# isarandi/metro-pose3d

Hardware: AMD Instinct MI355X
Metric: crops/sec (256x256, RN50 stride16) (higher is better)
Workload: dtype f16

## Files before the change

### include/metro_hip.h

```cpp
#ifndef METRO_HIP_H
#define METRO_HIP_H

#include <stddef.h>
#include <stdint.h>

#ifdef __cplusplus
extern "C" {
#endif

#define METRO_ABI_VERSION 8

typedef enum MetroStatus {
    METRO_OK = 0,
    METRO_ERR_INVALID_ARG = -1,
    METRO_ERR_UNSUPPORTED = -2,
    METRO_ERR_HIP = -3,
    METRO_ERR_STATE = -4,
    METRO_ERR_NONFINITE = -5
} MetroStatus;

typedef enum MetroPrecision { METRO_PREC_F16 = 0, METRO_PREC_F32 = 1, METRO_PREC_F64 = 2, METRO_PREC_F32M = 3 } MetroPrecision;

typedef enum MetroDType { METRO_F16 = 0, METRO_F32 = 1, METRO_F64 = 2 } MetroDType;

#define METRO_MAX_JOINTS 64

typedef struct MetroSpec {
    int32_t arch;
    int32_t stride;
    int32_t n_joints_head;
    int32_t depth;
    int32_t centered_stride;
    int32_t proc_side;
    float   box_size_mm;
    int32_t base_width;
    int32_t precision;
    int32_t n_joints_out;
    int32_t permutation[METRO_MAX_JOINTS];
} MetroSpec;

typedef struct MetroPlan MetroPlan;

typedef enum MetroParamKind {
    METRO_PARAM_CONV_W = 0,
    METRO_PARAM_BIAS = 1,
    METRO_PARAM_PRO_SCALE = 2,
    METRO_PARAM_PRO_SHIFT = 3
} MetroParamKind;

typedef struct MetroParamInfo {
    char    name[96];
    char    conv_var[160];
    char    bn_var[160];
    int32_t kind;
    int32_t dtype;
    int32_t c_out, kh, kw, c_in;
    int32_t kw_pad, c_in_pad;
    int64_t offset;
    int64_t bytes;
} MetroParamInfo;

#define METRO_FUSED_CONV1_IN_FRONT 1
#define METRO_FUSED_PROJECTION_SHORTCUT 2
#define METRO_FUSED_OUT_ON_CHIP 4
#define METRO_FUSED_REBUILT_SHORTCUT 8
#define METRO_FUSED_COMPACT_SHORTCUT 16

typedef struct MetroLayerInfo {
    char    name[96];
    int32_t kind;
    int32_t h_in, w_in, c_in, h_out, w_out, c_out, kh, kw, stride, dilation, pad_top, pad_left;
    int32_t has_prologue, relu, has_residual, res_stride, res_offset;
    int32_t out_dtype;
    int64_t out_offset;
    int64_t out_bytes_per_image;
    double  flops_per_image;
    int64_t out2_offset;
    int32_t out2_channels;
    int32_t fused_flags;
    int64_t algo_act_bytes_per_image;
    int64_t algo_param_bytes;
    int64_t out_sub_offset;
    int32_t out_sub_side, out_sub_off;
} MetroLayerInfo;

int  metro_plan_create(const MetroSpec* spec, int32_t max_batch, MetroPlan** out_plan);
int  metro_plan_destroy(MetroPlan* plan);
int64_t metro_plan_workspace_bytes(const MetroPlan* plan);
int64_t metro_plan_param_bytes(const MetroPlan* plan);
int32_t metro_plan_num_params(const MetroPlan* plan);
int  metro_plan_param_info(const MetroPlan* plan, int32_t index, MetroParamInfo* out);
int32_t metro_plan_num_layers(const MetroPlan* plan);
int  metro_plan_layer_info(const MetroPlan* plan, int32_t index, MetroLayerInfo* out);
double metro_plan_flops_per_image(const MetroPlan* plan);
int  metro_plan_layer_kernel(const MetroPlan* plan, int32_t index, int32_t n, char* buf, int32_t buf_len);
int  metro_kernel_notes(int32_t mode);
const char* metro_last_kernel_id(void);
int  metro_plan_bind_params(MetroPlan* plan, const void* d_param_blob);

int  metro_forward(MetroPlan* plan, const float* d_images_nhwc, int32_t n, float* d_poses_out,
                   void* d_workspace, void* stream);
int  metro_plan_set_graph_max_batch(MetroPlan* plan, int32_t max_batch_for_graphs);
int  metro_forward_status(const MetroPlan* plan, const void* d_workspace, int32_t n, void* stream, int32_t* n_nonfinite_out);
int64_t metro_plan_status_offset(const MetroPlan* plan);
int  metro_forward_upto(MetroPlan* plan, const float* d_images_nhwc, int32_t n,
                        float* d_poses_out, void* d_workspace, void* stream,
                        int32_t last_layer);

int  metro_forward_timed(MetroPlan* plan, const float* d_images_nhwc, int32_t n,
                         float* d_poses_out, void* d_workspace, void* stream,
                         float* ms_out );


typedef struct MetroConvDesc {
    int32_t n, h_in, w_in, c_in;
    int32_t in_pix_stride;
    int32_t h_out, w_out, c_out;
    int32_t kh, kw, stride, dilation;
    int32_t pad_top, pad_left;
    int32_t has_prologue;
    int32_t relu;
    int32_t has_residual;
    int32_t res_h, res_w;
    int32_t res_stride, res_offset;
    int32_t out_dtype;
    int32_t in_dtype;
} MetroConvDesc;

int  metro_conv_f16(const MetroConvDesc* d, const void* d_in, const void* d_w, const float* d_bias,
                    const void* d_pro_scale, const void* d_pro_shift, const void* d_residual,
                    void* d_out, void* stream);
int  metro_conv_f16_pair(const MetroConvDesc* d, const void* d_in, const void* d_w, const float* d_bias,
                         const void* d_pro_scale, const void* d_pro_shift, void* d_out, int32_t split,
                         void* d_out2, void* stream);
int  metro_conv_f16_next(const MetroConvDesc* d, const void* d_in, const void* d_w, const float* d_bias,
                         const void* d_residual, void* d_out, const void* d_w2, const float* d_bias2,
                         const void* d_scale2, const void* d_shift2, void* d_out2, int32_t c2, void* stream);
int  metro_conv_f16_conv1_conv2(const MetroConvDesc* d, const void* d_x, const void* d_w1, const float* d_bias1, const void* d_pro_scale,
                                const void* d_pro_shift, const void* d_w2, const float* d_bias2, void* d_out, void* stream);
int  metro_conv_f16_next_proj(const MetroConvDesc* d, const void* d_in, const void* d_w, const float* d_bias, const void* d_x,
                              const void* d_w_sc, const float* d_bias_sc, const void* d_pro_scale, const void* d_pro_shift, void* d_out,
                              const void* d_w2, const float* d_bias2, const void* d_scale2, const void* d_shift2, void* d_out2,
                              int32_t c2, void* stream);
int  metro_conv_f16_next_rebuild(const MetroConvDesc* d, const void* d_in, const void* d_w, const float* d_bias, const void* d_x,
                                 const void* d_w_sc, const float* d_bias_sc, const void* d_pro_scale, const void* d_pro_shift,
                                 const void* d_t2_prev, const void* d_w3_prev, const float* d_bias3_prev, void* d_out, void* d_out_sub,
                                 int32_t sub_off, const void* d_w2, const float* d_bias2, const void* d_scale2, const void* d_shift2,
                                 void* d_out2, int32_t c2, void* stream);
int  metro_conv_b1_form(int32_t classic);
int  metro_conv_f16_gemm4w(const MetroConvDesc* d, const void* d_in, const void* d_w, const float* d_bias,
                           const void* d_pro_scale, const void* d_pro_shift, const void* d_residual, void* d_out,
                           int32_t split, void* d_out2, void* stream);
int  metro_stem_pool_f16(const void* d_prepped, const void* d_w, const float* d_bias, void* d_out, int32_t n,
                         int32_t side, void* stream);
int  metro_stem_pool_f32in(const float* d_images, const void* d_w, const float* d_bias, void* d_out, int32_t n,
                           int32_t side, void* stream);
int  metro_stem_pool_u8in(const uint8_t* d_images, const void* d_w, const float* d_bias, void* d_out, int32_t n,
                          int32_t side, void* stream);
int  metro_conv_f64acc(const MetroConvDesc* d, const void* d_in, const double* d_w,
                       const double* d_bias, const double* d_pro_scale,
                       const double* d_pro_shift, const void* d_residual, void* d_out,
                       void* stream);

int  metro_conv_f32m(const MetroConvDesc* d, const void* d_in, const float* d_w, const float* d_bias, const float* d_pro_scale,
                     const float* d_pro_shift, const void* d_residual, void* d_out, void* stream);

int  metro_prep_input_f16(const float* d_images, int32_t n, int32_t side, void* d_out, void* stream);
int  metro_images_u8_to_f32(const uint8_t* d_in, int64_t count, float* d_out, void* stream);

int  metro_warp_crop_u8(const uint8_t* d_image, int32_t h, int32_t w, int32_t row_stride,
                        const float* d_homographies, int32_t n, int32_t side, float* d_out, void* stream);

#define METRO_MAX_FRAMES 64
#define METRO_WARP_HOMOGRAPHY 0
#define METRO_WARP_DISTORTED 1
typedef struct MetroFrame {
    const uint8_t* data;
    int32_t h, w, row_stride;
    int32_t reserved;
} MetroFrame;
typedef struct MetroCropWarp {
    int32_t frame;
    int32_t mode;
    double partial[9];
    float homography[9];
    float intrinsics[6];
    float distortion[5];
} MetroCropWarp;
int  metro_warp_crops_frames_u8(const MetroFrame* frames, int32_t n_frames, const MetroCropWarp* d_crops, int32_t n,
                                int32_t side, float* d_out, void* stream);
int  metro_warp_crops_frames_u8_to_u8(const MetroFrame* frames, int32_t n_frames, const MetroCropWarp* d_crops, int32_t n,
                                      int32_t side, uint8_t* d_out, void* stream);

#define METRO_PIX_RGB  0
#define METRO_PIX_BGR  1
#define METRO_PIX_NV12 2
#define METRO_PIX_I420 3
#define METRO_YUV_BT601 0
#define METRO_YUV_BT709 1
typedef struct MetroFramePlanes {
    const uint8_t* plane[3];
    int32_t h, w;
    int32_t stride[2];
    int32_t format, matrix;
} MetroFramePlanes;
int  metro_warp_crops_frames_planes(const MetroFramePlanes* frames, int32_t n_frames, const MetroCropWarp* d_crops,
                                    int32_t n, int32_t side, float* d_out, void* stream);
int  metro_warp_crops_frames_planes_to_u8(const MetroFramePlanes* frames, int32_t n_frames, const MetroCropWarp* d_crops,
                                          int32_t n, int32_t side, uint8_t* d_out, void* stream);

int  metro_maxpool3x3s2_zeropad(const void* d_in, void* d_out, int32_t n, int32_t h_in,
                                int32_t w_in, int32_t c, int32_t dtype, void* stream);

int64_t metro_softargmax_scratch_bytes(int32_t n, int32_t side, int32_t n_joints_head);
int  metro_softargmax(const void* d_logits, int32_t n, const MetroSpec* spec, int32_t precise,
                      void* d_partials, float* d_poses_out, void* stream);

int64_t metro_head_f16_scratch_bytes(int32_t n, int32_t side, int32_t n_joints_head);
int  metro_head_f16(const void* d_x, const void* d_w, const float* d_bias, const void* d_pro_scale, const void* d_pro_shift,
                    int32_t n, int32_t c_in, const MetroSpec* spec, void* d_partials, float* d_logits_out, float* d_poses_out,
                    void* stream);

int  metro_eval_metrics(const float* d_pred, const float* d_true, const uint8_t* d_valid, int32_t n,
                        int32_t n_joints, float threshold_mm, float* d_dist, float* d_dist_aligned,
                        double* d_sums, void* stream);

int  metro_softargmax01(const void* d_logits, int32_t n, const MetroSpec* spec, int32_t precise, void* d_scratch,
                        float* d_coords01_out, void* stream);
int  metro_backproject_bone_lengths(const float* d_coords01, const float* d_inv_intrinsics, const double* d_bone_lengths,
                                    int32_t per_pose_lengths, const int32_t* d_edges, int32_t n_edges, int32_t n,
                                    const MetroSpec* spec, int32_t root_relative, int32_t permute,
                                    float* d_coords3d_out, float* d_z_offset_out, void* stream);
int  metro_backproject_root_depth(const float* d_coords01, const float* d_inv_intrinsics, const float* d_root_z,
                                  int32_t n, const MetroSpec* spec, int32_t root_relative, int32_t permute,
                                  float* d_coords3d_out, void* stream);
int  metro_heatmap_to_25d(const float* d_coords01, int32_t n, const MetroSpec* spec, float* d_out, void* stream);
int  metro_to_orig_cam(const float* d_coords, const float* d_rot, const int32_t* d_mirror, float* d_out, int32_t n,
                       int32_t n_joints, void* stream);

int  metro_forward_coords01(MetroPlan* plan, const float* d_images_nhwc, int32_t n, float* d_poses_out,
                            float* d_coords01_out, void* d_workspace, void* stream);
int  metro_forward_u8(MetroPlan* plan, const uint8_t* d_images_nhwc, int32_t n, float* d_poses_out,
                      float* d_coords01_out, void* d_workspace, void* stream);
typedef struct MetroPlacement {
    int32_t keypoint_mode;
    int32_t reserved;
    float inv_intrinsics[9];
    float rot_to_orig_cam[9];
    float rot_to_world[9];
    float cam_loc[3];
    float homography[9];
    float intrinsics[6];
    float distortion[5];
} MetroPlacement;
#define METRO_SCALE_METRO 0
#define METRO_SCALE_BONE_LENGTHS 1
#define METRO_SCALE_TRUE_ROOT_DEPTH 2
#define METRO_COORDS_CROP 0
#define METRO_COORDS_CAMERA 1
#define METRO_COORDS_WORLD 2
int  metro_place_poses(const float* d_coords01, const float* d_poses, const MetroPlacement* d_records, int32_t n,
                       const MetroSpec* spec, int32_t scale_recovery, const double* d_bone_lengths, int32_t per_pose_lengths,
                       const float* d_root_depth, const int32_t* d_edges, int32_t n_edges, const int32_t* d_mirror,
                       int32_t coords, float* d_poses_out, float* d_keypoints_out, float* d_z_offset_out, void* stream);

typedef struct MetroViewBase {
    int32_t frame;
    int32_t mode;
    int32_t has_camera;
    int32_t reserved;
    double old_matrix[9];
    double orig_r[9];
    double virt_k[9];
    double virt_r[9];
    double partial[9];
    float homography[9];
    float inv_intrinsics[9];
    float rot_to_orig_cam[9];
    float rot_to_world[9];
    float cam_loc[3];
    float intrinsics[6];
    float distortion[5];
} MetroViewBase;
#define METRO_MAX_VIEWS 32
typedef struct MetroView {
    double cos_roll, sin_roll, zoom;
    int32_t flip;
    int32_t reserved;
} MetroView;
int  metro_expand_views(const MetroViewBase* d_bases, int32_t n, const MetroView* views, int32_t n_views, int32_t side,
                        MetroCropWarp* d_crops_out, MetroPlacement* d_placements_out, void* stream);
typedef struct MetroFrameCamera {
    float intrinsics[9];
    float r[9];
    float r_inv[9];
    float t[3];
    float distortion[5];
    int32_t has_distortion;
    double world_up[3];
    double old_matrix[9];
} MetroFrameCamera;
// ... 79 lines not shown
```

### metro_pose3d_amd/_lib.py

```python
from __future__ import annotations

import ctypes as C
import os

HERE = os.path.dirname(os.path.abspath(__file__))
LIB_PATH = os.environ.get('METRO_HIP_LIB') or os.path.join(HERE, 'libmetro_hip.so')

METRO_MAX_JOINTS = 64
ABI_VERSION = 8
METRO_PREC_F16, METRO_PREC_F32, METRO_PREC_F64, METRO_PREC_F32M = 0, 1, 2, 3
METRO_F16, METRO_F32, METRO_F64 = 0, 1, 2
PARAM_CONV_W, PARAM_BIAS, PARAM_PRO_SCALE, PARAM_PRO_SHIFT = 0, 1, 2, 3
LAYER_PREP, LAYER_CONV, LAYER_POOL, LAYER_SOFTARGMAX = 0, 1, 2, 3
FUSED_CONV1_IN_FRONT, FUSED_PROJECTION_SHORTCUT = 1, 2
FUSED_OUT_ON_CHIP, FUSED_REBUILT_SHORTCUT, FUSED_COMPACT_SHORTCUT = 4, 8, 16


class MetroSpec(C.Structure):
    _fields_ = [('arch', C.c_int32), ('stride', C.c_int32), ('n_joints_head', C.c_int32),
                ('depth', C.c_int32), ('centered_stride', C.c_int32), ('proc_side', C.c_int32),
                ('box_size_mm', C.c_float), ('base_width', C.c_int32), ('precision', C.c_int32),
                ('n_joints_out', C.c_int32), ('permutation', C.c_int32 * METRO_MAX_JOINTS)]


class MetroParamInfo(C.Structure):
    _fields_ = [('name', C.c_char * 96), ('conv_var', C.c_char * 160), ('bn_var', C.c_char * 160),
                ('kind', C.c_int32), ('dtype', C.c_int32),
                ('c_out', C.c_int32), ('kh', C.c_int32), ('kw', C.c_int32), ('c_in', C.c_int32),
                ('kw_pad', C.c_int32), ('c_in_pad', C.c_int32),
                ('offset', C.c_int64), ('bytes', C.c_int64)]


class MetroLayerInfo(C.Structure):
    _fields_ = [('name', C.c_char * 96), ('kind', C.c_int32),
                ('h_in', C.c_int32), ('w_in', C.c_int32), ('c_in', C.c_int32),
                ('h_out', C.c_int32), ('w_out', C.c_int32), ('c_out', C.c_int32),
                ('kh', C.c_int32), ('kw', C.c_int32), ('stride', C.c_int32),
                ('dilation', C.c_int32), ('pad_top', C.c_int32), ('pad_left', C.c_int32),
                ('has_prologue', C.c_int32), ('relu', C.c_int32), ('has_residual', C.c_int32),
                ('res_stride', C.c_int32), ('res_offset', C.c_int32), ('out_dtype', C.c_int32),
                ('out_offset', C.c_int64), ('out_bytes_per_image', C.c_int64),
                ('flops_per_image', C.c_double),
                ('out2_offset', C.c_int64), ('out2_channels', C.c_int32), ('fused_flags', C.c_int32),
                ('algo_act_bytes_per_image', C.c_int64), ('algo_param_bytes', C.c_int64),
                ('out_sub_offset', C.c_int64), ('out_sub_side', C.c_int32), ('out_sub_off', C.c_int32)]


class MetroConvDesc(C.Structure):
    _fields_ = [('n', C.c_int32), ('h_in', C.c_int32), ('w_in', C.c_int32), ('c_in', C.c_int32),
                ('in_pix_stride', C.c_int32),
                ('h_out', C.c_int32), ('w_out', C.c_int32), ('c_out', C.c_int32),
                ('kh', C.c_int32), ('kw', C.c_int32), ('stride', C.c_int32), ('dilation', C.c_int32),
                ('pad_top', C.c_int32), ('pad_left', C.c_int32),
                ('has_prologue', C.c_int32), ('relu', C.c_int32), ('has_residual', C.c_int32),
                ('res_h', C.c_int32), ('res_w', C.c_int32),
                ('res_stride', C.c_int32), ('res_offset', C.c_int32), ('out_dtype', C.c_int32),
                ('in_dtype', C.c_int32)]


METRO_MAX_FRAMES = 64
METRO_WARP_HOMOGRAPHY, METRO_WARP_DISTORTED = 0, 1


class MetroFrame(C.Structure):
    _fields_ = [('data', C.c_void_p), ('h', C.c_int32), ('w', C.c_int32), ('row_stride', C.c_int32),
                ('reserved', C.c_int32)]


METRO_PIX_RGB, METRO_PIX_BGR, METRO_PIX_NV12, METRO_PIX_I420 = 0, 1, 2, 3
METRO_YUV_BT601, METRO_YUV_BT709 = 0, 1


class MetroFramePlanes(C.Structure):
    _fields_ = [('plane', C.c_void_p * 3), ('h', C.c_int32), ('w', C.c_int32), ('stride', C.c_int32 * 2),
                ('format', C.c_int32), ('matrix', C.c_int32)]


class MetroCropWarp(C.Structure):
    _fields_ = [('frame', C.c_int32), ('mode', C.c_int32), ('partial', C.c_double * 9), ('homography', C.c_float * 9),
                ('intrinsics', C.c_float * 6), ('distortion', C.c_float * 5)]


METRO_SCALE_METRO, METRO_SCALE_BONE_LENGTHS, METRO_SCALE_TRUE_ROOT_DEPTH = 0, 1, 2
METRO_COORDS_CROP, METRO_COORDS_CAMERA, METRO_COORDS_WORLD = 0, 1, 2


class MetroPlacement(C.Structure):
    _fields_ = [('keypoint_mode', C.c_int32), ('reserved', C.c_int32), ('inv_intrinsics', C.c_float * 9),
                ('rot_to_orig_cam', C.c_float * 9), ('rot_to_world', C.c_float * 9), ('cam_loc', C.c_float * 3),
                ('homography', C.c_float * 9), ('intrinsics', C.c_float * 6), ('distortion', C.c_float * 5)]


METRO_MAX_VIEWS = 32
METRO_TRI_UNIFORM, METRO_TRI_COVARIANCE = 0, 1
METRO_MATCH_MAX_BOXES = 128
METRO_SMOOTH_FILTER, METRO_SMOOTH_RTS = 0, 1
METRO_SMOOTH_ISOTROPIC, METRO_SMOOTH_COVARIANCE = 0, 1
METRO_ASSOC_MAX = 128


class MetroViewBase(C.Structure):
    _fields_ = [('frame', C.c_int32), ('mode', C.c_int32), ('has_camera', C.c_int32), ('reserved', C.c_int32),
                ('old_matrix', C.c_double * 9), ('orig_r', C.c_double * 9), ('virt_k', C.c_double * 9),
                ('virt_r', C.c_double * 9), ('partial', C.c_double * 9), ('homography', C.c_float * 9),
                ('inv_intrinsics', C.c_float * 9), ('rot_to_orig_cam', C.c_float * 9), ('rot_to_world', C.c_float * 9),
                ('cam_loc', C.c_float * 3), ('intrinsics', C.c_float * 6), ('distortion', C.c_float * 5)]


class MetroFrameCamera(C.Structure):
    _fields_ = [('intrinsics', C.c_float * 9), ('r', C.c_float * 9), ('r_inv', C.c_float * 9), ('t', C.c_float * 3),
                ('distortion', C.c_float * 5), ('has_distortion', C.c_int32), ('world_up', C.c_double * 3),
                ('old_matrix', C.c_double * 9)]


class MetroView(C.Structure):
    _fields_ = [('cos_roll', C.c_double), ('sin_roll', C.c_double), ('zoom', C.c_double), ('flip', C.c_int32),
                ('reserved', C.c_int32)]


_P = C.c_void_p
SIGNATURES = {
    'metro_plan_create': (C.c_int, [C.POINTER(MetroSpec), C.c_int32, C.POINTER(_P)]),
    'metro_plan_destroy': (C.c_int, [_P]),
    'metro_plan_workspace_bytes': (C.c_int64, [_P]),
    'metro_plan_param_bytes': (C.c_int64, [_P]),
    'metro_plan_num_params': (C.c_int32, [_P]),
    'metro_plan_param_info': (C.c_int, [_P, C.c_int32, C.POINTER(MetroParamInfo)]),
    'metro_plan_num_layers': (C.c_int32, [_P]),
    'metro_plan_layer_info': (C.c_int, [_P, C.c_int32, C.POINTER(MetroLayerInfo)]),
    'metro_plan_flops_per_image': (C.c_double, [_P]),
    'metro_plan_bind_params': (C.c_int, [_P, _P]),
    'metro_plan_layer_kernel': (C.c_int, [_P, C.c_int32, C.c_int32, C.c_char_p, C.c_int32]),
    'metro_kernel_notes': (C.c_int, [C.c_int32]),
    'metro_last_kernel_id': (C.c_char_p, []),
    'metro_plan_set_graph_max_batch': (C.c_int, [_P, C.c_int32]),
    'metro_forward': (C.c_int, [_P, _P, C.c_int32, _P, _P, _P]),
    'metro_forward_coords01': (C.c_int, [_P, _P, C.c_int32, _P, _P, _P, _P]),
    'metro_forward_u8': (C.c_int, [_P, _P, C.c_int32, _P, _P, _P, _P]),
    'metro_forward_status': (C.c_int, [_P, _P, C.c_int32, _P, C.POINTER(C.c_int32)]),
    'metro_plan_status_offset': (C.c_int64, [_P]),
    'metro_forward_upto': (C.c_int, [_P, _P, C.c_int32, _P, _P, _P, C.c_int32]),
    'metro_forward_timed': (C.c_int, [_P, _P, C.c_int32, _P, _P, _P, C.POINTER(C.c_float)]),
    'metro_conv_f16': (C.c_int, [C.POINTER(MetroConvDesc), _P, _P, _P, _P, _P, _P, _P, _P]),
    'metro_conv_f32m': (C.c_int, [C.POINTER(MetroConvDesc), _P, _P, _P, _P, _P, _P, _P, _P]),
    'metro_conv_f64acc': (C.c_int, [C.POINTER(MetroConvDesc), _P, _P, _P, _P, _P, _P, _P, _P]),
    'metro_conv_f16_pair': (C.c_int, [C.POINTER(MetroConvDesc), _P, _P, _P, _P, _P, _P, C.c_int32, _P, _P]),
    'metro_conv_b1_form': (C.c_int, [C.c_int32]),
    'metro_conv_f16_gemm4w': (C.c_int, [C.POINTER(MetroConvDesc), _P, _P, _P, _P, _P, _P, _P, C.c_int32, _P, _P]),
    'metro_conv_f16_conv1_conv2': (C.c_int, [C.POINTER(MetroConvDesc), _P, _P, _P, _P, _P, _P, _P, _P, _P]),
    'metro_conv_f16_next_proj': (C.c_int, [C.POINTER(MetroConvDesc)] + [_P] * 14 + [C.c_int32, _P]),
    'metro_conv_f16_next_rebuild': (C.c_int, [C.POINTER(MetroConvDesc)] + [_P] * 13 + [C.c_int32] + [_P] * 5 + [C.c_int32, _P]),
    'metro_conv_f16_next': (C.c_int, [C.POINTER(MetroConvDesc), _P, _P, _P, _P, _P, _P, _P, _P, _P, _P, C.c_int32, _P]),
    'metro_stem_pool_f16': (C.c_int, [_P, _P, _P, _P, C.c_int32, C.c_int32, _P]),
    'metro_stem_pool_f32in': (C.c_int, [_P, _P, _P, _P, C.c_int32, C.c_int32, _P]),
    'metro_stem_pool_u8in': (C.c_int, [_P, _P, _P, _P, C.c_int32, C.c_int32, _P]),
    'metro_prep_input_f16': (C.c_int, [_P, C.c_int32, C.c_int32, _P, _P]),
    'metro_images_u8_to_f32': (C.c_int, [_P, C.c_int64, _P, _P]),
    'metro_warp_crop_u8': (C.c_int, [_P, C.c_int32, C.c_int32, C.c_int32, _P, C.c_int32, C.c_int32, _P, _P]),
    'metro_warp_crops_frames_u8': (C.c_int, [C.POINTER(MetroFrame), C.c_int32, _P, C.c_int32, C.c_int32, _P, _P]),
    'metro_warp_crops_frames_planes': (C.c_int, [C.POINTER(MetroFramePlanes), C.c_int32, _P, C.c_int32, C.c_int32, _P,
                                                 _P]),
    'metro_warp_crops_frames_u8_to_u8': (C.c_int, [C.POINTER(MetroFrame), C.c_int32, _P, C.c_int32, C.c_int32, _P, _P]),
    'metro_warp_crops_frames_planes_to_u8': (C.c_int, [C.POINTER(MetroFramePlanes), C.c_int32, _P, C.c_int32, C.c_int32, _P,
                                                       _P]),
    'metro_eval_metrics': (C.c_int, [_P, _P, _P, C.c_int32, C.c_int32, C.c_float, _P, _P, _P, _P]),
    'metro_maxpool3x3s2_zeropad': (C.c_int, [_P, _P, C.c_int32, C.c_int32, C.c_int32, C.c_int32,
                                             C.c_int32, _P]),
    'metro_softargmax_scratch_bytes': (C.c_int64, [C.c_int32, C.c_int32, C.c_int32]),
    'metro_softargmax01': (C.c_int, [_P, C.c_int32, C.POINTER(MetroSpec), C.c_int32, _P, _P, _P]),
    'metro_backproject_bone_lengths': (C.c_int, [_P, _P, _P, C.c_int32, _P, C.c_int32, C.c_int32, C.POINTER(MetroSpec),
                                                 C.c_int32, C.c_int32, _P, _P, _P]),
    'metro_backproject_root_depth': (C.c_int, [_P, _P, _P, C.c_int32, C.POINTER(MetroSpec), C.c_int32, C.c_int32, _P, _P]),
    'metro_to_orig_cam': (C.c_int, [_P, _P, _P, _P, C.c_int32, C.c_int32, _P]),
    'metro_place_poses': (C.c_int, [_P, _P, _P, C.c_int32, C.POINTER(MetroSpec), C.c_int32, _P, C.c_int32, _P, _P, C.c_int32,
                                    _P, C.c_int32, _P, _P, _P, _P]),
    'metro_expand_views': (C.c_int, [_P, C.c_int32, C.POINTER(MetroView), C.c_int32, C.c_int32, _P, _P, _P]),
    'metro_look_at_boxes': (C.c_int, [_P, _P, C.c_int32, C.c_int32, _P, C.c_int32, C.c_int32, _P, _P, _P]),
    'metro_merge_views': (C.c_int, [_P, _P, _P, _P, _P, C.c_int32, C.c_int32, C.c_int32, _P, _P, _P, _P, _P]),
    'metro_heatmap_to_25d': (C.c_int, [_P, C.c_int32, C.POINTER(MetroSpec), _P, _P]),
    'metro_head_f16_scratch_bytes': (C.c_int64, [C.c_int32, C.c_int32, C.c_int32]),
    'metro_head_f16': (C.c_int, [_P, _P, _P, _P, _P, C.c_int32, C.c_int32, C.POINTER(MetroSpec), _P, _P, _P, _P]),
    'metro_softargmax': (C.c_int, [_P, C.c_int32, C.POINTER(MetroSpec), C.c_int32, _P, _P, _P]),
    'metro_moments_scratch_bytes': (C.c_int64, [C.POINTER(MetroSpec), C.c_int32]),
    'metro_forward_moments': (C.c_int, [_P, _P, C.c_int32, C.c_int32, _P, _P, _P, _P, _P, _P, _P]),
    'metro_head_f16_moments': (C.c_int, [_P, _P, _P, _P, _P, C.c_int32, C.c_int32, C.POINTER(MetroSpec)] + [_P] * 8),
    'metro_softargmax01_moments': (C.c_int, [_P, C.c_int32, C.POINTER(MetroSpec), C.c_int32, _P, _P, _P, _P, _P, _P]),
    'metro_place_covariances': (C.c_int, [_P, _P, _P, C.c_int32, C.c_int32, C.POINTER(MetroSpec), _P, C.c_int32, _P, _P, _P]),
    'metro_triangulate_joints': (C.c_int, [_P, _P, _P, C.c_int32, _P, C.c_int32, _P, C.c_int32, C.POINTER(MetroSpec), _P, C.c_int32,
                                           C.c_double, _P, _P, _P, _P]),
    'metro_view_affinity': (C.c_int, [_P, _P, _P, C.POINTER(MetroSpec), _P, _P, C.c_int32, C.c_int32, C.c_int32, C.c_double, C.c_double,
                                      C.c_int32, _P, _P, _P]),
    'metro_triangulate_joints_cov': (C.c_int, [_P, _P, _P, C.c_int32, _P, C.c_int32, _P, C.c_int32, C.POINTER(MetroSpec), _P, C.c_int32,
                                               C.c_double, _P, _P, _P, _P, _P]),
    'metro_view_affinity_steps': (C.c_int, [_P, _P, _P, C.POINTER(MetroSpec), _P, _P, _P, C.c_int32, C.c_int32, C.c_int32, C.c_double,
                                            C.c_double, C.c_int32, _P, _P, _P]),
    'metro_person_steps': (C.c_int, [_P, C.c_int32, _P, _P, C.c_int32, C.c_int32, _P, C.c_int32, _P, C.c_int32, _P, _P, _P, _P, _P]),
    'metro_cluster_views': (C.c_int, [_P, C.c_int32, C.c_int32, C.c_float, _P, _P, _P, _P, _P]),
    'metro_smooth_tracks_workspace_bytes': (C.c_size_t, [C.c_int32, C.c_int32]),
    'metro_smooth_tracks': (C.c_int, [_P, _P, _P, C.c_int32, _P, C.c_int32, _P, C.c_int32, C.POINTER(MetroSpec), C.c_int32, C.c_int32,
                                      C.c_double, C.c_double, C.c_double, C.c_double, C.c_double, _P, _P, _P, _P, _P, _P, _P]),
    'metro_associate_tracks_workspace_bytes': (C.c_size_t, [C.c_int32, C.c_int32]),
    'metro_associate_tracks': (C.c_int, [_P, _P, _P, C.c_int32, _P, C.c_int32, _P, C.c_int32, C.POINTER(MetroSpec), C.c_int32,
                                         C.c_double, C.c_double, C.c_double, C.c_double, C.c_double, C.c_float, C.c_double, C.c_int32,
                                         C.c_double, _P, C.c_int32] + [_P] * 11),
    'metro_last_error': (C.c_char_p, []),
    'metro_abi_version': (C.c_int32, []),
}

EXPERIMENTAL_LIB_PATH = os.path.join(HERE, 'libmetro_experimental.so')
EXPERIMENTAL_SIGNATURES = {
    'metro_conv_f16_gemm8p': (C.c_int, [C.POINTER(MetroConvDesc), _P, _P, _P, _P, _P, _P, _P, C.c_int32, _P, _P]),
    'metro_conv_f16_gemm4d': (C.c_int, [C.POINTER(MetroConvDesc), _P, _P, _P, _P, _P, _P, _P, C.c_int32, _P, _P]),
    'metro_conv_f16_gemm4d_geo': (C.c_int, [C.POINTER(MetroConvDesc), _P, _P, _P, _P, _P, _P, _P, C.c_int32, _P, C.c_int32, _P]),
}

_lib = None
_xlib = None


class MetroError(RuntimeError):
    pass


class NonFiniteError(MetroError):
    """metro_forward_status: activations overflowed the arithmetic mode (fp16 storage tops out at 65 504)."""


def load() -> C.CDLL:
    global _lib
    if _lib is not None:
        return _lib
    if not os.path.exists(LIB_PATH):
        raise MetroError(
            f'{LIB_PATH} is missing: build it with `python -m metro_pose3d_amd.build` '
            '(hipcc --offload-arch=gfx950). There is no CPU fallback for this path.')
    import torch
    lib = C.CDLL(LIB_PATH)
    for name, (res, args) in SIGNATURES.items():
        fn = getattr(lib, name)
        fn.restype = res
        fn.argtypes = args
    if lib.metro_abi_version() != ABI_VERSION:
        raise MetroError(f'ABI version mismatch: library {lib.metro_abi_version()}, bindings {ABI_VERSION}')
    _lib = lib
    return lib


def load_experimental() -> C.CDLL:
    global _xlib
    if _xlib is not None:
        return _xlib
    load()
    if not os.path.exists(EXPERIMENTAL_LIB_PATH):
        raise MetroError(f'{EXPERIMENTAL_LIB_PATH} is missing: build it with `python -m metro_pose3d_amd.build`')
    lib = C.CDLL(EXPERIMENTAL_LIB_PATH)
    for name, (res, args) in EXPERIMENTAL_SIGNATURES.items():
        fn = getattr(lib, name)
        fn.restype = res
        fn.argtypes = args
    _xlib = lib
    return lib


def check(status: int, what: str = '') -> None:
    if status == 0:
        return
    msg = load().metro_last_error().decode(errors='replace')
    if status == -1:
        raise ValueError(f'{what}: {msg}')
    if status == -5:
        raise NonFiniteError(f'{what}: {msg}')
    raise MetroError(f'{what}: status {status}: {msg}')
```

### metro_pose3d_amd/csrc/conv_igemm_f16_dma.hip

```cpp
#include <cstdlib>
#include <type_traits>

#include "metro_common.h"
#include "gfx950_prims.h"

namespace metro {

template <int WAVES_M_, int WAVES_N_, int WM_, int WN_, int STAGES_, int BK_ = 64>
struct DmaCfg {
    static constexpr int WAVES_M = WAVES_M_, WAVES_N = WAVES_N_, WM = WM_, WN = WN_, STAGES = STAGES_;
    static constexpr int BK = BK_;
    static constexpr int CPR = BK / 8;
    static constexpr int RPI = 64 / CPR;
    static constexpr int NW = WAVES_M * WAVES_N;
    static constexpr int NT = 64 * NW;
    static constexpr int TM = WAVES_M * WM * 32;
    static constexpr int TN = WAVES_N * WN * 32;
    static constexpr int WI = TM / (RPI * NW);
    static constexpr int XI = TN / (RPI * NW);
    static constexpr int LPS = WI + XI;
    static constexpr int ROW_BYTES = BK * 2;
    static constexpr int STAGE_BYTES = (TM + TN) * ROW_BYTES;
    static constexpr int RING_BYTES = STAGES * STAGE_BYTES;
    static constexpr int OUT_ROW_BYTES = TM * 2 + 16;
    static constexpr int OUT_BYTES = TN * OUT_ROW_BYTES;
    static constexpr int MAIN_BYTES = RING_BYTES > OUT_BYTES ? RING_BYTES : OUT_BYTES;
    static constexpr int PRO_BYTES = 2 * 2048 * 2;
    static_assert(TM % (RPI * NW) == 0 && TN % (RPI * NW) == 0, "tile/loader mismatch");
    static_assert(BK == 64 || BK == 32, "BK must be 32 or 64");
    static_assert(STAGES >= 1 && STAGES <= 6, "ring depth 1..6");
};

struct Fuse2Args {
    const half_t* w2; const float* bias2; const half_t* scale2; const half_t* shift2; half_t* out2; int c2;
};

template <class Cfg, bool PROLOGUE, bool FASTK, bool FUSE2>
__device__ __forceinline__ void conv_dma_body(
    const ConvArgs& a, const half_t* __restrict__ in, const half_t* __restrict__ w,
    const float* __restrict__ bias, const half_t* __restrict__ pro_scale,
    const half_t* __restrict__ pro_shift, const half_t* __restrict__ residual,
    void* __restrict__ out, int out_f32, int tiles_m, void* __restrict__ out2, const Fuse2Args& f2) {
    extern __shared__ __attribute__((aligned(16))) char smem[];
    constexpr int BK = Cfg::BK, STAGES = Cfg::STAGES, NW = Cfg::NW;
    constexpr int CPR = Cfg::CPR, RPI = Cfg::RPI;
    constexpr int SLICES = BK / 16;
    constexpr int F2_W_OFF = Cfg::MAIN_BYTES + (PROLOGUE ? Cfg::PRO_BYTES : 0);
    constexpr int F2_W_BYTES = 64 * Cfg::TM * 2;
    constexpr int F2_P_OFF = F2_W_OFF + F2_W_BYTES;

    const int tid = threadIdx.x;
    const int lane = tid & 63;
    const int wave = __builtin_amdgcn_readfirstlane(tid >> 6);
    const int wave_m = wave / Cfg::WAVES_N;
    const int wave_n = wave % Cfg::WAVES_N;

    const int nblk = gridDim.x;
    int lid;
    {
        const int b = blockIdx.x;
        const int q = nblk >> 3, r = nblk & 7;
        const int xcd = b & 7, idx = b >> 3;
        lid = (xcd < r ? xcd * (q + 1) : r * (q + 1) + (xcd - r) * q) + idx;
    }
    const int tile_n = lid / tiles_m;
    const int tile_m = lid % tiles_m;
    const int m0 = tile_n * Cfg::TN;
    const int n0 = tile_m * Cfg::TM;

    const int taps = a.kh * a.kw;
    const int k_total = taps * a.c_in;
    const int kc_steps = (a.c_in + BK - 1) / BK;
    const int nk = taps * kc_steps;
    const int hw_out = a.h_out * a.w_out;
    const half_t* zero = reinterpret_cast<const half_t*>(g_zero_page);
    const unsigned smem_base = lds_offset_of(smem);

    half_t* pro_lds = reinterpret_cast<half_t*>(smem + Cfg::MAIN_BYTES);

    const int lrow = lane / CPR;
    const int lch = lane % CPR;
    const half_t* wsrc[Cfg::WI];
    int wkoff[Cfg::WI], winc[Cfg::WI];
    bool wvalid[Cfg::WI];
#pragma unroll
    for (int i = 0; i < Cfg::WI; ++i) {
        const int row = (i * NW + wave) * RPI + lrow;
        const int co = n0 + row;
        wvalid[i] = co < a.c_out;
        wkoff[i] = (lch ^ swz<BK>(row)) * 8;
        const half_t* base = w + (size_t)(wvalid[i] ? co : 0) * k_total;
        wsrc[i] = FASTK ? (wvalid[i] ? base + wkoff[i] : zero) : base;
        winc[i] = wvalid[i] ? BK : 0;
    }
    int xh[Cfg::XI], xw[Cfg::XI], xn[Cfg::XI], xkoff[Cfg::XI], xinc[Cfg::XI];
    const half_t* xptr[Cfg::XI];
    bool xvalid[Cfg::XI];
#pragma unroll
    for (int i = 0; i < Cfg::XI; ++i) {
        const int row = (i * NW + wave) * RPI + lrow;
        const int m = m0 + row;
        xvalid[i] = m < a.m_total;
        const int mm = xvalid[i] ? m : 0;
        const int img = mm / hw_out;
        const int rem = mm - img * hw_out;
        const int ho = rem / a.w_out;
        const int wo = rem - ho * a.w_out;
        xh[i] = ho * a.stride - a.pad_top;
        xw[i] = wo * a.stride - a.pad_left;
        xn[i] = img * a.h_in * a.w_in;
        xkoff[i] = (lch ^ swz<BK>(row)) * 8;
        xptr[i] = zero;
        xinc[i] = 0;
    }

    int is_tap = 0, is_c0 = 0, is_r = 0, is_s = 0;
    auto x_new_tap = [&]() {
#pragma unroll
        for (int i = 0; i < Cfg::XI; ++i) {
            const int hi = xh[i] + is_r * a.dil;
            const int wi = xw[i] + is_s * a.dil;
            const bool ok = xvalid[i] && (unsigned)hi < (unsigned)a.h_in && (unsigned)wi < (unsigned)a.w_in;
            xptr[i] = ok ? in + (size_t)(xn[i] + hi * a.w_in + wi) * a.in_pix_stride + xkoff[i] : zero;
            xinc[i] = ok ? BK : 0;
        }
    };
    if (FASTK) x_new_tap();
    unsigned is_wl = 0, is_xl = 0;
    int is_kbase = 0;
    auto issue_begin = [&](int buf) {
        is_wl = __builtin_amdgcn_readfirstlane(smem_base + buf * Cfg::STAGE_BYTES + wave * RPI * Cfg::ROW_BYTES);
        is_xl = is_wl + Cfg::TM * Cfg::ROW_BYTES;
        is_kbase = is_tap * a.c_in + is_c0;
    };
    auto issue_part = [&](int part) {
#pragma unroll
        for (int i = 0; i < Cfg::WI; ++i) {
            if ((i % SLICES) != part) continue;
            if (FASTK) {
                dma16(wsrc[i], is_wl + i * NW * RPI * Cfg::ROW_BYTES);
                wsrc[i] += winc[i];
            } else {
                const int c = is_c0 + wkoff[i];
                const half_t* src = (wvalid[i] && c < a.c_in) ? wsrc[i] + is_kbase + wkoff[i] : zero;
                dma16(src, is_wl + i * NW * RPI * Cfg::ROW_BYTES);
            }
        }
#pragma unroll
        for (int i = 0; i < Cfg::XI; ++i) {
            if (((i + Cfg::WI) % SLICES) != part) continue;
            if (FASTK) {
                dma16(xptr[i], is_xl + i * NW * RPI * Cfg::ROW_BYTES);
                xptr[i] += xinc[i];
            } else {
                const int hi = xh[i] + is_r * a.dil;
                const int wi = xw[i] + is_s * a.dil;
                const int c = is_c0 + xkoff[i];
                const bool ok = xvalid[i] && c < a.c_in && (unsigned)hi < (unsigned)a.h_in &&
                                (unsigned)wi < (unsigned)a.w_in;
                const half_t* src = ok ? in + (size_t)(xn[i] + hi * a.w_in + wi) * a.in_pix_stride + c : zero;
                dma16(src, is_xl + i * NW * RPI * Cfg::ROW_BYTES);
            }
        }
    };
    auto issue_end = [&]() {
        is_c0 += BK;
        if (is_c0 >= a.c_in) {
            is_c0 = 0;
            ++is_tap;
            if (++is_s == a.kw) { is_s = 0; ++is_r; }
            if (FASTK && is_tap < taps) x_new_tap();
        }
    };
    auto issue_step = [&](int buf) {
        issue_begin(buf);
#pragma unroll
        for (int p = 0; p < SLICES; ++p) issue_part(p);
        issue_end();
    };

    floatx16 acc[Cfg::WM][Cfg::WN];
#pragma unroll
    for (int i = 0; i < Cfg::WM; ++i)
#pragma unroll
        for (int j = 0; j < Cfg::WN; ++j)
#pragma unroll
            for (int e = 0; e < 16; ++e) acc[i][j][e] = 0.f;

    const int frag_row = lane & 31;
    const int frag_half = lane >> 5;

    auto compute_step = [&](int buf, int c0, auto with_issue) {
        const char* wl = smem + buf * Cfg::STAGE_BYTES;
        const char* xl = wl + Cfg::TM * Cfg::ROW_BYTES;
#pragma unroll
        for (int kk = 0; kk < BK / 16; ++kk) {
            half8_t af[Cfg::WM], bf[Cfg::WN];
            const int chunk = kk * 2 + frag_half;
#pragma unroll
            for (int i = 0; i < Cfg::WM; ++i) {
                const int row = (wave_m * Cfg::WM + i) * 32 + frag_row;
                af[i] = *reinterpret_cast<const half8_t*>(wl + row * Cfg::ROW_BYTES + ((chunk ^ swz<BK>(row)) << 4));
            }
#pragma unroll
            for (int j = 0; j < Cfg::WN; ++j) {
                const int row = (wave_n * Cfg::WN + j) * 32 + frag_row;
                bf[j] = *reinterpret_cast<const half8_t*>(xl + row * Cfg::ROW_BYTES + ((chunk ^ swz<BK>(row)) << 4));
            }
            if (PROLOGUE) {
                const half8_t sc = *reinterpret_cast<const half8_t*>(pro_lds + c0 + chunk * 8);
                const half8_t sh = *reinterpret_cast<const half8_t*>(pro_lds + 2048 + c0 + chunk * 8);
                const half8_t z = {};
#pragma unroll
                for (int j = 0; j < Cfg::WN; ++j) bf[j] = __builtin_elementwise_max(bf[j] * sc + sh, z);
            }
#ifdef METRO_SETPRIO
            __builtin_amdgcn_s_setprio(1);
#endif
#pragma unroll
            for (int i = 0; i < Cfg::WM; ++i)
#pragma unroll
                for (int j = 0; j < Cfg::WN; ++j)
                    acc[i][j] = __builtin_amdgcn_mfma_f32_32x32x16_f16(af[i], bf[j], acc[i][j], 0, 0, 0);
#ifdef METRO_SETPRIO
            __builtin_amdgcn_s_setprio(0);
#endif
            if constexpr (decltype(with_issue)::value) issue_part(kk);
        }
    };
    using Yes = std::integral_constant<bool, true>;
    using No = std::integral_constant<bool, false>;

    constexpr int CPRO = Cfg::TM / 8;
    constexpr int EPI_ITERS = Cfg::TN * CPRO / Cfg::NT;
    static_assert(Cfg::TN * CPRO % Cfg::NT == 0, "epilogue loop must divide evenly");
    const bool res_same = a.res_stride == 1 && a.res_offset == 0 && a.res_h == a.h_out && a.res_w == a.w_out;
    const bool has_res = residual != nullptr && !out_f32;
    uint4 rres[EPI_ITERS];
#pragma unroll
    for (int it = 0; it < EPI_ITERS; ++it) rres[it] = make_uint4(0, 0, 0, 0);
    auto prefetch_residual = [&]() {
#pragma unroll
        for (int it = 0; it < EPI_ITERS; ++it) {
            const int idx = tid + it * Cfg::NT;
            const int prow = idx / CPRO;
            const int ch = idx - prow * CPRO;
            const int m = m0 + prow;
            const int co = n0 + ch * 8;
            const bool ok = m < a.m_total && co + 8 <= a.c_out;
            size_t rp = ok ? (size_t)m : 0;
            if (!res_same && ok) {
                const int img = m / hw_out;
                const int rem = m - img * hw_out;
                const int ho = rem / a.w_out;
                const int wo = rem - ho * a.w_out;
                rp = (size_t)(img * a.res_h + ho * a.res_stride + a.res_offset) * a.res_w +
                     (wo * a.res_stride + a.res_offset);
            }
            rres[it] = *reinterpret_cast<const uint4*>(residual + rp * a.c_out + (ok ? co : 0));
        }
    };

    constexpr bool PRO_DMA = PROLOGUE && !FUSE2;
    if constexpr (PRO_DMA) {
#pragma unroll
        for (int i = 0; i < (8 + NW - 1) / NW; ++i) {
            const int id = wave * ((8 + NW - 1) / NW) + i;
            const int piece = id & 3;
            if (id < 8 && piece * 512 < a.c_in) {
                const int idx = piece * 512 + lane * 8;
                const half_t* src = idx < a.c_in ? ((id >> 2) ? pro_shift : pro_scale) + idx : zero;
                dma16(src, __builtin_amdgcn_readfirstlane(smem_base + Cfg::MAIN_BYTES + (id >> 2) * 4096 + piece * 1024));
            }
        }
    }
    if constexpr (STAGES > 1) {
#pragma unroll
        for (int s = 0; s < STAGES - 1; ++s)
            if (s < nk) issue_step(s);
    } else {
        issue_step(0);
    }
    if constexpr (FUSE2) {
        static_assert(BK == 64 && (F2_W_BYTES / 1024) % NW == 0, "FUSE2 layout");
#pragma unroll
        for (int i = 0; i < F2_W_BYTES / 1024 / NW; ++i) {
            const int vrow = (i * NW + wave) * 8 + (lane >> 3);
            const int kc = vrow >> 6, r = vrow & 63;
            const half_t* src = f2.w2 + (size_t)r * Cfg::TM + kc * 64 + (((lane & 7) ^ swz<64>(r)) * 8);
            dma16(src, __builtin_amdgcn_readfirstlane(smem_base + F2_W_OFF + (i * NW + wave) * 1024));
        }
        half_t* p2 = reinterpret_cast<half_t*>(smem + F2_P_OFF);
        for (int c = tid * 8; c < Cfg::TM; c += Cfg::NT * 8) {
            *reinterpret_cast<uint4*>(p2 + c) = *reinterpret_cast<const uint4*>(f2.scale2 + c);
            *reinterpret_cast<uint4*>(p2 + Cfg::TM + c) = *reinterpret_cast<const uint4*>(f2.shift2 + c);
        }
    }
    if (PROLOGUE && !PRO_DMA) {
        const int cpad = kc_steps * BK;
        for (int c = tid * 8; c < cpad; c += Cfg::NT * 8) {
            uint4 sv = make_uint4(0, 0, 0, 0), bv = make_uint4(0, 0, 0, 0);
            if (c < a.c_in) {
                sv = *reinterpret_cast<const uint4*>(pro_scale + c);
                bv = *reinterpret_cast<const uint4*>(pro_shift + c);
            }
            *reinterpret_cast<uint4*>(pro_lds + c) = sv;
            *reinterpret_cast<uint4*>(pro_lds + 2048 + c) = bv;
        }
    }

    if (PROLOGUE && !PRO_DMA) __syncthreads();
    if constexpr (STAGES == 1) {
        int cc0 = 0;
        for (int k = 0; k < nk; ++k) {
            if (k > 0) {
                wait_vm_and_barrier<0>();
                issue_step(0);
            }
            if (has_res && k == nk - 1) {
                prefetch_residual();
                wait_vm_and_barrier<EPI_ITERS>();
            } else {
                wait_vm_and_barrier<0>();
            }
            compute_step(0, cc0, No{});
            cc0 += BK;
            if (cc0 >= a.c_in) cc0 = 0;
        }
    } else {
        int cbuf = 0, ibuf = STAGES - 1, cc0 = 0;
        auto advance = [&]() {
            cbuf = cbuf + 1 == STAGES ? 0 : cbuf + 1;
            ibuf = ibuf + 1 == STAGES ? 0 : ibuf + 1;
            cc0 += BK;
            if (cc0 >= a.c_in) cc0 = 0;
        };
        const int n_main = nk - (STAGES - 1);
        for (int k = 0; k < n_main; ++k) {
            wait_vm_and_barrier<(STAGES - 2) * Cfg::LPS>();
            issue_begin(ibuf);
            compute_step(cbuf, cc0, Yes{});
            issue_end();
            advance();
        }
        if (has_res) prefetch_residual();
        for (int k = n_main < 0 ? 0 : n_main; k < nk; ++k) {
            int ahead = nk - 1 - k;
            if (ahead > STAGES - 2) ahead = STAGES - 2;
            if (has_res) {
                switch (ahead) {
                    case 4: wait_vm_and_barrier<(STAGES >= 6 ? 4 : 0) * Cfg::LPS + EPI_ITERS>(); break;
                    case 3: wait_vm_and_barrier<(STAGES >= 5 ? 3 : 0) * Cfg::LPS + EPI_ITERS>(); break;
                    case 2: wait_vm_and_barrier<(STAGES >= 4 ? 2 : 0) * Cfg::LPS + EPI_ITERS>(); break;
                    case 1: wait_vm_and_barrier<(STAGES >= 3 ? 1 : 0) * Cfg::LPS + EPI_ITERS>(); break;
                    default: wait_vm_and_barrier<EPI_ITERS>(); break;
                }
            } else {
                switch (ahead) {
                    case 4: wait_vm_and_barrier<(STAGES >= 6 ? 4 : 0) * Cfg::LPS>(); break;
                    case 3: wait_vm_and_barrier<(STAGES >= 5 ? 3 : 0) * Cfg::LPS>(); break;
                    case 2: wait_vm_and_barrier<(STAGES >= 4 ? 2 : 0) * Cfg::LPS>(); break;
                    case 1: wait_vm_and_barrier<(STAGES >= 3 ? 1 : 0) * Cfg::LPS>(); break;
                    default: wait_vm_and_barrier<0>(); break;
                }
            }
            compute_step(cbuf, cc0, No{});
            advance();
        }
    }

    const bool second = a.split > 0 && n0 >= a.split;
    const int o_c = a.split > 0 ? (second ? a.c_out2 : a.split) : a.c_out;
    const int o_n0 = second ? n0 - a.split : n0;
    const int o_relu = second ? a.relu2 : a.relu;
    void* o_ptr = second ? out2 : out;
    if (out_f32) {
#pragma unroll
        for (int j = 0; j < Cfg::WN; ++j) {
            const int m = m0 + (wave_n * Cfg::WN + j) * 32 + frag_row;
            if (m >= a.m_total) continue;
#pragma unroll
            for (int i = 0; i < Cfg::WM; ++i) {
#pragma unroll
                for (int q = 0; q < 4; ++q) {
                    const int co = n0 + (wave_m * Cfg::WM + i) * 32 + 8 * q + 4 * frag_half;
                    if (co >= a.c_out) continue;
                    const floatx4 bv = *reinterpret_cast<const floatx4*>(bias + co);
                    floatx4 v;
#pragma unroll
                    for (int e = 0; e < 4; ++e) v[e] = acc[i][j][4 * q + e] + bv[e];
                    if (a.relu) {
#pragma unroll
                        for (int e = 0; e < 4; ++e) v[e] = fmaxf(v[e], 0.f);
                    }
                    *reinterpret_cast<floatx4*>(reinterpret_cast<float*>(out) + (size_t)m * a.c_out + co) = v;
                }
            }
        }
        return;
    }

    __syncthreads();
#pragma unroll
    for (int i = 0; i < Cfg::WM; ++i) {
#pragma unroll
        for (int q = 0; q < 4; ++q) {
            const int col = (wave_m * Cfg::WM + i) * 32 + 8 * q + 4 * frag_half;
            const int co = n0 + col;
            floatx4 bv = {0.f, 0.f, 0.f, 0.f};
            if (co < a.c_out) bv = *reinterpret_cast<const floatx4*>(bias + co);
#pragma unroll
            for (int j = 0; j < Cfg::WN; ++j) {
                const int prow = (wave_n * Cfg::WN + j) * 32 + frag_row;
                half4_t hv;
#pragma unroll
                for (int e = 0; e < 4; ++e) {
                    float v = acc[i][j][4 * q + e] + bv[e];
                    if (o_relu) v = fmaxf(v, 0.f);
                    hv[e] = (half_t)v;
                }
                *reinterpret_cast<half4_t*>(smem + prow * Cfg::OUT_ROW_BYTES + col * 2) = hv;
            }
        }
    }
    constexpr int T2M = 2, T2N = Cfg::TN / 32;
    constexpr int F2_KSTEPS = FUSE2 ? Cfg::TM / 16 : 1;
    __syncthreads();
    half_t* outh = reinterpret_cast<half_t*>(o_ptr);
    constexpr int EPI_G = EPI_ITERS % 8 == 0 ? 8 : EPI_ITERS % 4 == 0 ? 4 : EPI_ITERS % 2 == 0 ? 2 : 1;
    const bool interior = m0 + Cfg::TN <= a.m_total && o_n0 + Cfg::TM <= o_c;
    if (interior) {
#pragma unroll
        for (int it0 = 0; it0 < EPI_ITERS; it0 += EPI_G) {
            uint4 vv[EPI_G];
#pragma unroll
            for (int u = 0; u < EPI_G; ++u) {
                const int idx = tid + (it0 + u) * Cfg::NT;
                const int prow = idx / CPRO;
                vv[u] = *reinterpret_cast<const uint4*>(smem + prow * Cfg::OUT_ROW_BYTES + (idx - prow * CPRO) * 16);
            }
            __builtin_amdgcn_sched_barrier(0);
#pragma unroll
            for (int u = 0; u < EPI_G; ++u) {
                const int idx = tid + (it0 + u) * Cfg::NT;
                const int prow = idx / CPRO;
                const int ch = idx - prow * CPRO;
                uint4 v = vv[u];
                if (residual != nullptr) {
                    half2_t* x = reinterpret_cast<half2_t*>(&v);
                    const half2_t* r = reinterpret_cast<const half2_t*>(&rres[it0 + u]);
#pragma unroll
                    for (int e = 0; e < 4; ++e) x[e] = x[e] + r[e];
                }
                store_out16<2>(outh + (size_t)(m0 + prow) * o_c + o_n0 + ch * 8, v);
                if constexpr (FUSE2) *reinterpret_cast<uint4*>(smem + prow * Cfg::OUT_ROW_BYTES + ch * 16) = v;
            }
        }
    } else
#pragma unroll
    for (int it = 0; it < EPI_ITERS; ++it) {
        const int idx = tid + it * Cfg::NT;
        const int prow = idx / CPRO;
        const int ch = idx - prow * CPRO;
        const int m = m0 + prow;
        const int co = o_n0 + ch * 8;
        if (m >= a.m_total || co >= o_c) continue;
        uint4 v = *reinterpret_cast<const uint4*>(smem + prow * Cfg::OUT_ROW_BYTES + ch * 16);
        if (co + 8 <= o_c) {
            if (residual != nullptr) {
                half2_t* x = reinterpret_cast<half2_t*>(&v);
                const half2_t* r = reinterpret_cast<const half2_t*>(&rres[it]);
#pragma unroll
                for (int e = 0; e < 4; ++e) x[e] = x[e] + r[e];
            }
            store_out16<2>(outh + (size_t)m * o_c + co, v);
            if constexpr (FUSE2) *reinterpret_cast<uint4*>(smem + prow * Cfg::OUT_ROW_BYTES + ch * 16) = v;
        } else {
            const half8_t x = *reinterpret_cast<const half8_t*>(&v);
#pragma unroll
            for (int e = 0; e < 8; ++e)
                if (co + e < o_c) outh[(size_t)m * o_c + co + e] = x[e];
        }
    }
    if constexpr (FUSE2) {
        __syncthreads();
        if (wave < T2M * T2N) {
            const int i2 = wave / T2N, j2 = wave % T2N;
            floatx16 acc2;
#pragma unroll
            for (int e = 0; e < 16; ++e) acc2[e] = 0.f;
            const half_t* p2 = reinterpret_cast<const half_t*>(smem + F2_P_OFF);
            const int prow2 = j2 * 32 + frag_row;
            const int arow = i2 * 32 + frag_row;
            const char* w2l = smem + F2_W_OFF + arow * 128;
#pragma unroll
            for (int ks = 0; ks < F2_KSTEPS; ++ks) {
                const int k0 = ks * 16 + frag_half * 8;
                const half8_t af = *reinterpret_cast<const half8_t*>(
                    w2l + (ks >> 2) * 8192 + ((((ks & 3) * 2 + frag_half) ^ swz<64>(arow)) << 4));
                half8_t bf = *reinterpret_cast<const half8_t*>(smem + prow2 * Cfg::OUT_ROW_BYTES + k0 * 2);
                const half8_t sc = *reinterpret_cast<const half8_t*>(p2 + k0);
                const half8_t sh = *reinterpret_cast<const half8_t*>(p2 + Cfg::TM + k0);
                const half8_t z = {};
                bf = __builtin_elementwise_max(bf * sc + sh, z);
                acc2 = __builtin_amdgcn_mfma_f32_32x32x16_f16(af, bf, acc2, 0, 0, 0);
            }
            const int m = m0 + prow2;
            if (m < a.m_total) {
#pragma unroll
                for (int q = 0; q < 4; ++q) {
                    const int co = i2 * 32 + 8 * q + 4 * frag_half;
                    const floatx4 bv = *reinterpret_cast<const floatx4*>(f2.bias2 + co);
                    half4_t hv;
#pragma unroll
                    for (int e = 0; e < 4; ++e) hv[e] = (half_t)fmaxf(acc2[4 * q + e] + bv[e], 0.f);
                    *reinterpret_cast<half4_t*>(f2.out2 + (size_t)m * f2.c2 + co) = hv;
                }
            }
        }
    }
}

template <class Cfg, bool PROLOGUE, bool FASTK>
__global__ __launch_bounds__(Cfg::NT) void conv_igemm_f16_dma_kernel(
    ConvArgs a, const half_t* __restrict__ in, const half_t* __restrict__ w,
    const float* __restrict__ bias, const half_t* __restrict__ pro_scale,
    const half_t* __restrict__ pro_shift, const half_t* __restrict__ residual,
    void* __restrict__ out, int out_f32, int tiles_m, void* __restrict__ out2) {
    conv_dma_body<Cfg, PROLOGUE, FASTK, false>(a, in, w, bias, pro_scale, pro_shift, residual, out, out_f32, tiles_m,
                                               out2, Fuse2Args{});
}

template <class Cfg>
__global__ __launch_bounds__(Cfg::NT) void conv_igemm_f16_fuse2_kernel(
    ConvArgs a, const half_t* __restrict__ in, const half_t* __restrict__ w, const float* __restrict__ bias,
    const half_t* __restrict__ residual, void* __restrict__ out, Fuse2Args f2) {
    conv_dma_body<Cfg, false, true, true>(a, in, w, bias, nullptr, nullptr, residual, out, 0, 1, nullptr, f2);
}

template <class Cfg, bool PROLOGUE, bool FASTK>
static int launch_dma_cfg2(const ConvArgs& a, const half_t* in, const half_t* w, const float* bias,
                           const half_t* ps, const half_t* pb, const half_t* res, void* out, int out_f32, void* out2,
                           hipStream_t stream) {
    static_assert(256 % Cfg::TM == 0, "a pair splits on a 256-row boundary (conv_form_supported): whole cout tiles");
    if (note_kernel("conv_igemm_f16_dma<%dx%d,bk%d,s%d%s%s>%s%s%s", Cfg::TM, Cfg::TN, Cfg::BK, Cfg::STAGES, PROLOGUE ? ",pro" : "",
                    FASTK ? "" : ",ktail", res ? "+res" : "", a.split > 0 ? "+pair" : "", out_f32 ? "+f32out" : ""))
        return METRO_OK;
    auto kern = conv_igemm_f16_dma_kernel<Cfg, PROLOGUE, FASTK>;
    constexpr int lds = Cfg::MAIN_BYTES + (PROLOGUE ? Cfg::PRO_BYTES : 0);
    static PerDeviceInt attr_done;
    if (const int st = ensure_dyn_lds(reinterpret_cast<const void*>(kern), lds, attr_done, "conv_igemm_f16_dma")) return st;
    const int tiles_m = (a.c_out + Cfg::TM - 1) / Cfg::TM;
    const int tiles_n = (a.m_total + Cfg::TN - 1) / Cfg::TN;
    hipLaunchKernelGGL(kern, dim3(tiles_m * tiles_n), dim3(Cfg::NT), lds, stream, a, in, w, bias, ps, pb,
                       res, out, out_f32, tiles_m, out2);
    return launch_status("conv_igemm_f16_dma");
}

template <class Cfg, bool PROLOGUE>
static int launch_dma_cfg(const ConvArgs& a, const half_t* in, const half_t* w, const float* bias,
                          const half_t* ps, const half_t* pb, const half_t* res, void* out, int out_f32, void* out2,
                          hipStream_t stream) {
    if (a.c_in % Cfg::BK == 0)
        return launch_dma_cfg2<Cfg, PROLOGUE, true>(a, in, w, bias, ps, pb, res, out, out_f32, out2, stream);
    return launch_dma_cfg2<Cfg, PROLOGUE, false>(a, in, w, bias, ps, pb, res, out, out_f32, out2, stream);
}

using Dma128x256s3 = DmaCfg<2, 4, 2, 2, 3>;
using Dma128x128s4 = DmaCfg<2, 4, 2, 1, 4>;
using Dma128x128s2 = DmaCfg<2, 4, 2, 1, 2>;
using Dma128x128s1 = DmaCfg<2, 4, 2, 1, 1>;
using Dma256x256s4k32 = DmaCfg<2, 4, 4, 2, 4, 32>;
using Dma128x256s3k32 = DmaCfg<2, 4, 2, 2, 3, 32>;
using Dma64x128s3 = DmaCfg<1, 4, 2, 1, 3>;
using Dma64x128s1 = DmaCfg<1, 4, 2, 1, 1>;
using Dma64x128s3k32 = DmaCfg<1, 4, 2, 1, 3, 32>;

using DmaFuse256x64 = DmaCfg<4, 2, 2, 1, 1>;

bool conv_f16_fuse2_supported(const MetroConvDesc& d, int c2) {
    static const int enabled = tuning_knob("METRO_FUSE2", 1);
    return enabled && d.c_out == DmaFuse256x64::TM && c2 == 64 && d.kh == 1 && d.kw == 1 && d.c_in == 64 &&
           d.in_pix_stride == 64 && d.stride == 1 && d.pad_top == 0 && d.pad_left == 0 && !d.has_prologue &&
           d.out_dtype == METRO_F16 && d.in_dtype == METRO_F16 && d.h_in == d.h_out && d.w_in == d.w_out;
}

static int launch_fuse2(const ConvArgs& a, const half_t* in, const half_t* w, const float* bias, const half_t* res,
                        void* out, const ConvFuse2& f, hipStream_t stream) {
    using Cfg = DmaFuse256x64;
    if (note_kernel("conv_igemm_f16_fuse2<256x64>%s", res ? "+res" : "")) return METRO_OK;
    auto kern = conv_igemm_f16_fuse2_kernel<Cfg>;
    constexpr int lds = Cfg::MAIN_BYTES + 64 * Cfg::TM * 2 + 2 * Cfg::TM * 2;
    static PerDeviceInt attr_done;
    if (const int st = ensure_dyn_lds(reinterpret_cast<const void*>(kern), lds, attr_done, "conv_igemm_f16_fuse2")) return st;
    const int tiles_n = (a.m_total + Cfg::TN - 1) / Cfg::TN;
    hipLaunchKernelGGL(kern, dim3(tiles_n), dim3(Cfg::NT), lds, stream, a, in, w, bias, res, out,
                       Fuse2Args{static_cast<const half_t*>(f.w2), f.bias2, static_cast<const half_t*>(f.scale2),
                                 static_cast<const half_t*>(f.shift2), static_cast<half_t*>(f.out2), f.c2});
    return launch_status("conv_igemm_f16_dma<fuse2>");
}

bool conv_f16_dma_supported(const MetroConvDesc& d) {
    return d.in_pix_stride % 4 == 0 && d.c_in % 8 == 0 && d.c_in <= 2048 && d.c_out % 4 == 0 &&
           (!d.has_residual || d.c_out % 8 == 0) && (d.in_pix_stride % 8 == 0 || !d.has_prologue);
}

bool conv_form_supported(const MetroConvDesc& d, const ConvFused& f) {
    const ConvSplit& s = f.pair;
    const ConvRebuild& rb = f.rb;
    switch (f.form) {
        case ConvForm::Plain:
            return true;
        case ConvForm::Pair:
            return d.kh == 1 && d.kw == 1 && d.stride == 1 && d.has_prologue && !d.has_residual && !d.relu && d.in_dtype == METRO_F16 &&
                   d.out_dtype == METRO_F16 && d.c_in % 64 == 0 && s.split > 0 && s.c_out2 > 0 && s.split + s.c_out2 == d.c_out &&
                   s.split % 256 == 0 && s.c_out2 % 8 == 0;
        case ConvForm::Next:
            return conv_f16_fuse2_supported(d, f.next.c2) || conv_pw64_supported(d, f);
        case ConvForm::NextProj:
            return conv_pw64_supported(d, f) && (rb.out_mode == 0 || rb.out_mode == 1);
        case ConvForm::NextRebuild:
            return conv_pw64_supported(d, f) &&
                   (rb.out_mode == 0 || (rb.out_mode == 2 && rb.out_sub != nullptr && (rb.sub_off == 0 || rb.sub_off == 1) && rb.h_sub > 0 &&
                                         rb.w_sub > 0));
    }
    return false;
}

int launch_conv_f16_dma(const MetroConvDesc& d, const void* in_, const void* w_, const float* bias,
                        const void* ps_, const void* pb_, const void* res_, void* out, hipStream_t stream, const ConvFused& f) {
    ConvArgs a = make_conv_args(d);
    void* out2 = nullptr;
    switch (f.form) {
        case ConvForm::NextProj:
        case ConvForm::NextRebuild:
            return launch_conv_pw64(d, in_, w_, bias, nullptr, nullptr, nullptr, out, stream, f);
        case ConvForm::Next:
            if (conv_pw64_supported(d, f)) return launch_conv_pw64(d, in_, w_, bias, ps_, pb_, res_, out, stream, f);
            return launch_fuse2(a, static_cast<const half_t*>(in_), static_cast<const half_t*>(w_), bias,
                                d.has_residual ? static_cast<const half_t*>(res_) : nullptr, out, f.next, stream);
        case ConvForm::Pair:
            if (conv_pw64_supported(d, f)) return launch_conv_pw64(d, in_, w_, bias, ps_, pb_, res_, out, stream, f);
            if (conv_gemm4w_supported(d, &f.pair)) return launch_conv_gemm4w(d, in_, w_, bias, ps_, pb_, res_, out, stream, &f.pair);
            a.split = f.pair.split; a.c_out2 = f.pair.c_out2; a.relu2 = f.pair.relu2;
            out2 = f.pair.out2;
            break;
        case ConvForm::Plain:
            if (conv_pws_supported(d)) return launch_conv_pws(d, in_, w_, bias, res_, out, stream);
            if (conv_pw64_supported(d, f)) return launch_conv_pw64(d, in_, w_, bias, ps_, pb_, res_, out, stream, f);
            if (conv_gemm4w_supported(d, nullptr)) return launch_conv_gemm4w(d, in_, w_, bias, ps_, pb_, res_, out, stream, nullptr);
            break;
    }
    const half_t* in = static_cast<const half_t*>(in_);
    const half_t* w = static_cast<const half_t*>(w_);
    const half_t* ps = static_cast<const half_t*>(ps_);
    const half_t* pb = static_cast<const half_t*>(pb_);
    const half_t* res = d.has_residual ? static_cast<const half_t*>(res_) : nullptr;
    const int out_f32 = d.out_dtype == METRO_F32;
    const bool pro = d.has_prologue != 0;
    const int tiles128 = (d.c_out + 127) / 128;
    static const int nk_s1 = tuning_knob("METRO_NK_S1", 2);
    static const int nk_s2 = tuning_knob("METRO_NK_S2", 8);
#define METRO_DMA(CFG)                                                                               \
    return pro ? launch_dma_cfg<CFG, true>(a, in, w, bias, ps, pb, res, out, out_f32, out2, stream)  \
               : launch_dma_cfg<CFG, false>(a, in, w, bias, ps, pb, res, out, out_f32, out2, stream)
    if (d.c_in <= 32 && !pro) {
        return launch_dma_cfg<Dma64x128s3k32, false>(a, in, w, bias, ps, pb, res, out, out_f32, out2, stream);
    }
    const int nk = d.kh * d.kw * ((d.c_in + 63) / 64);
    static const int head64 = tuning_knob("METRO_DMA_HEAD64", 1);
    const bool narrow = d.c_out <= 64 || (head64 && d.c_out < 256 && d.c_out % 128 != 0 && (d.c_out % 128) <= 64 &&
                                          d.c_out / 128 <= 1);
    if (narrow) {
        if (nk <= nk_s1) { METRO_DMA(Dma64x128s1); }
        METRO_DMA(Dma64x128s3);
    }
    if (nk <= nk_s1) { METRO_DMA(Dma128x128s1); }
    static const int k32 = tuning_knob("METRO_DMA_K32", 8);
    {
        const long b256 = (long)tiles128 * ((a.m_total + 255) / 256);
        if (k32 && nk <= k32 && b256 >= 512) { METRO_DMA(Dma128x256s3k32); }
    }
    if (nk <= nk_s2) { METRO_DMA(Dma128x128s2); }
    const long blocks256 = (long)tiles128 * ((a.m_total + 255) / 256);
    static const int big = tuning_knob("METRO_DMA_BIG", 2);
    if (big && d.c_out % 256 == 0 && blocks256 / 2 >= 256) { METRO_DMA(Dma256x256s4k32); }
    if (blocks256 >= 256) { METRO_DMA(Dma128x256s3); }
    static const int half_tiles = tuning_knob("METRO_DMA_HALF_TILES", 1);
    const long blocks128 = (long)tiles128 * ((a.m_total + 127) / 128);
    if (half_tiles && d.c_out % 64 == 0 && blocks128 >= 64 && blocks128 < 224 && a.split == 0) { METRO_DMA(Dma64x128s3); }
    METRO_DMA(Dma128x128s4);
#undef METRO_DMA
}

int launch_conv_f16(const MetroConvDesc& d, const void* in, const void* w, const float* bias, const void* ps,
                    const void* pb, const void* res, void* out, hipStream_t stream) {
    if (conv3x3_c64_supported(d)) return launch_conv3x3_c64(d, in, w, bias, out, stream);
    if (conv3x3_slab_supported(d)) return launch_conv3x3_slab(d, in, w, bias, out, stream);
    if (conv_f16_dma_supported(d)) return launch_conv_f16_dma(d, in, w, bias, ps, pb, res, out, stream);
    set_error("conv_f16: unsupported layer (c_in %d must be a multiple of 8 and <= 2048, in_pix_stride %d of 4 (8 with a "
              "prologue), c_out %d of 4 (8 with a residual))", d.c_in, d.in_pix_stride, d.c_out);
    return METRO_ERR_UNSUPPORTED;
}

}
```

### metro_pose3d_amd/csrc/entries.cpp

```cpp
#include <cmath>
#include <cstring>

#include "metro_common.h"

namespace metro {

static thread_local char g_err[512] = "";

void set_error(const char* fmt, ...) {
    va_list ap;
    va_start(ap, fmt);
    vsnprintf(g_err, sizeof(g_err), fmt, ap);
    va_end(ap);
}
const char* get_error() { return g_err; }

static thread_local KernelNotes g_notes = {0, ""};
KernelNotes& kernel_notes() { return g_notes; }
bool note_kernel(const char* fmt, ...) {
    if (g_notes.mode == 0) return false;
    const size_t cap = sizeof(g_notes.ids) - 5;
    const size_t used = strlen(g_notes.ids);
    if (used >= 4 && strcmp(g_notes.ids + used - 4, " ...") == 0) return g_notes.mode == 2;
    char one[512];
    va_list ap;
    va_start(ap, fmt);
    vsnprintf(one, sizeof(one), fmt, ap);
    va_end(ap);
    const size_t need = strlen(one) + (used ? 3 : 0);
    if (used + need > cap) { memcpy(g_notes.ids + used, " ...", 5); return g_notes.mode == 2; }
    if (used) memcpy(g_notes.ids + used, " & ", 3);
    memcpy(g_notes.ids + used + (used ? 3 : 0), one, strlen(one) + 1);
    return g_notes.mode == 2;
}

int validate_conv_desc(const MetroConvDesc* d) {
    METRO_CHECK_ARG(d != nullptr, "conv desc is NULL");
    METRO_CHECK_ARG(d->n > 0 && d->h_in > 0 && d->w_in > 0 && d->c_in > 0 && d->h_out > 0 &&
                        d->w_out > 0 && d->c_out > 0,
                    "conv desc: non-positive dimension");
    METRO_CHECK_ARG(d->kh > 0 && d->kw > 0 && d->stride > 0 && d->dilation > 0, "conv desc: bad kernel geometry");
    METRO_CHECK_ARG(d->in_pix_stride > 0, "conv desc: in_pix_stride must be positive");
    METRO_CHECK_ARG((long)d->n * d->h_out * d->w_out < (1L << 31), "conv desc: too many output pixels");
    METRO_CHECK_ARG((long)d->n * d->h_in * d->w_in < (1L << 31), "conv desc: too many input pixels");
    if (d->has_prologue) {
        METRO_CHECK_ARG(d->kh == 1 && d->kw == 1, "conv desc: prologue requires a 1x1 kernel");
        const long last_h = (long)(d->h_out - 1) * d->stride - d->pad_top;
        const long last_w = (long)(d->w_out - 1) * d->stride - d->pad_left;
        METRO_CHECK_ARG(d->pad_top <= 0 && d->pad_left <= 0 && last_h < d->h_in && last_w < d->w_in,
                        "conv desc: prologue requires every tap to be in bounds (no padding)");
    }
    if (d->has_residual) {
        METRO_CHECK_ARG(d->res_stride > 0 && d->res_offset >= 0, "conv desc: bad residual gather");
        METRO_CHECK_ARG((d->h_out - 1) * d->res_stride + d->res_offset < d->res_h &&
                            (d->w_out - 1) * d->res_stride + d->res_offset < d->res_w,
                        "conv desc: residual gather out of bounds");
    }
    return METRO_OK;
}

}

using namespace metro;

extern "C" {

int metro_kernel_notes(int32_t mode) {
    METRO_CHECK_ARG(mode >= 0 && mode <= 2, "metro_kernel_notes: mode must be 0 (off), 1 (record) or 2 (dry run)");
    KernelNotes& kn = kernel_notes();
    kn.mode = mode; kn.ids[0] = 0;
    return METRO_OK;
}
const char* metro_last_kernel_id(void) { return kernel_notes().ids; }

int metro_conv_f16(const MetroConvDesc* d, const void* d_in, const void* d_w, const float* d_bias,
                   const void* d_pro_scale, const void* d_pro_shift, const void* d_residual,
                   void* d_out, void* stream) {
    int st = validate_conv_desc(d);
    if (st) return st;
    METRO_CHECK_ARG(d->c_in % 8 == 0 && d->in_pix_stride % 4 == 0, "conv_f16: c_in must be a multiple of 8 (got %d) and in_pix_stride of 4", d->c_in);
    METRO_CHECK_ARG(d->c_in <= 2048, "conv_f16: c_in must be <= 2048 (got %d)", d->c_in);
    METRO_CHECK_ARG(d->c_out % 4 == 0, "conv_f16: c_out must be a multiple of 4 (got %d)", d->c_out);
    METRO_CHECK_ARG(d->out_dtype == METRO_F16 || d->out_dtype == METRO_F32, "conv_f16: out_dtype must be F16 or F32");
    METRO_CHECK_ARG(d->in_dtype == METRO_F16, "conv_f16: in_dtype must be F16");
    METRO_CHECK_ARG(!(d->has_residual && d->out_dtype == METRO_F32), "conv_f16: a residual needs F16 output (F32 output has no residual epilogue)");
    METRO_CHECK_ARG(d_in && d_w && d_bias && d_out, "conv_f16: NULL tensor pointer");
    METRO_CHECK_ARG(!d->has_prologue || (d_pro_scale && d_pro_shift), "conv_f16: prologue tensors missing");
    METRO_CHECK_ARG(!d->has_residual || d_residual, "conv_f16: residual tensor missing");
    return launch_conv_f16(*d, d_in, d_w, d_bias, d_pro_scale, d_pro_shift, d_residual, d_out,
                           static_cast<hipStream_t>(stream));
}

int metro_conv_f16_pair(const MetroConvDesc* d, const void* d_in, const void* d_w, const float* d_bias,
                        const void* d_pro_scale, const void* d_pro_shift, void* d_out, int32_t split,
                        void* d_out2, void* stream) {
    int st = validate_conv_desc(d);
    if (st) return st;
    METRO_CHECK_ARG(d_in && d_w && d_bias && d_out && d_out2 && d_pro_scale && d_pro_shift, "conv_f16_pair: NULL tensor pointer");
    ConvFused f;
    f.form = ConvForm::Pair;
    f.pair = {split, d->c_out - split, 1, d_out2};
    METRO_CHECK_ARG(conv_form_supported(*d, f), "conv_f16_pair: fp16 1x1 stride-1 convolution with prologue, without residual / ReLU on the "
                    "first output, c_in %% 64; split %d of c_out %d (split %% 256, rest %% 8)", split, d->c_out);
    return launch_conv_f16_dma(*d, d_in, d_w, d_bias, d_pro_scale, d_pro_shift, nullptr, d_out, static_cast<hipStream_t>(stream), f);
}

int metro_conv_f16_next(const MetroConvDesc* d, const void* d_in, const void* d_w, const float* d_bias,
                        const void* d_residual, void* d_out, const void* d_w2, const float* d_bias2,
                        const void* d_scale2, const void* d_shift2, void* d_out2, int32_t c2, void* stream) {
    int st = validate_conv_desc(d);
    if (st) return st;
    METRO_CHECK_ARG(d_in && d_w && d_bias && d_out && d_w2 && d_bias2 && d_scale2 && d_shift2 && d_out2,
                    "conv_f16_next: NULL tensor pointer");
    METRO_CHECK_ARG(!d->has_residual || d_residual, "conv_f16_next: residual tensor missing");
    ConvFused f;
    f.form = ConvForm::Next;
    f.next = {d_w2, d_bias2, d_scale2, d_shift2, d_out2, c2};
    METRO_CHECK_ARG(conv_form_supported(*d, f),
                    "conv_f16_next: built for 1x1 stride-1 64 -> 256 with c2 = 64 (block1) and 128 -> 512 with c2 = 128 (block2), fp16");
    return launch_conv_f16_dma(*d, d_in, d_w, d_bias, nullptr, nullptr, d_residual, d_out, static_cast<hipStream_t>(stream), f);
}

int metro_conv_f16_conv1_conv2(const MetroConvDesc* d, const void* d_x, const void* d_w1, const float* d_bias1, const void* d_pro_scale,
                               const void* d_pro_shift, const void* d_w2, const float* d_bias2, void* d_out, void* stream) {
    int st = validate_conv_desc(d);
    if (st) return st;
    METRO_CHECK_ARG(d_x && d_w1 && d_bias1 && d_pro_scale && d_pro_shift && d_w2 && d_bias2 && d_out, "conv_f16_conv1_conv2: NULL tensor pointer");
    METRO_CHECK_ARG(conv3x3_c64_supported(*d), "conv_f16_conv1_conv2: built for 3x3 stride-1 SAME 64 -> 64 on maps of <= 64 columns that tile into "
                    "128-pixel row pairs (block1 of the 256-pixel nets)");
    ConvPre1 p1;
    p1.w1 = d_w1; p1.bias1 = d_bias1; p1.pro_scale = d_pro_scale; p1.pro_shift = d_pro_shift;
    return launch_conv3x3_c64(*d, d_x, d_w2, d_bias2, d_out, static_cast<hipStream_t>(stream), &p1);
}

int metro_conv_f16_next_proj(const MetroConvDesc* d, const void* d_in, const void* d_w, const float* d_bias, const void* d_x,
                             const void* d_w_sc, const float* d_bias_sc, const void* d_pro_scale, const void* d_pro_shift, void* d_out,
                             const void* d_w2, const float* d_bias2, const void* d_scale2, const void* d_shift2, void* d_out2,
                             int32_t c2, void* stream) {
    int st = validate_conv_desc(d);
    if (st) return st;
    METRO_CHECK_ARG(d_in && d_w && d_bias && d_x && d_w_sc && d_bias_sc && d_pro_scale && d_pro_shift && d_w2 && d_bias2 &&
                        d_scale2 && d_shift2 && d_out2, "conv_f16_next_proj: NULL tensor pointer");
    ConvFused f;
    f.form = ConvForm::NextProj;
    f.next = {d_w2, d_bias2, d_scale2, d_shift2, d_out2, c2};
    f.psc = {d_x, d_w_sc, d_bias_sc, d_pro_scale, d_pro_shift};
    f.rb.out_mode = d_out == nullptr ? 1 : 0;
    METRO_CHECK_ARG(conv_form_supported(*d, f), "conv_f16_next_proj: built for 1x1 stride-1 64 -> 256 without prologue / residual, "
                    "c2 = 64 (block1/unit_1), fp16");
    return launch_conv_f16_dma(*d, d_in, d_w, d_bias, nullptr, nullptr, nullptr, d_out, static_cast<hipStream_t>(stream), f);
}

int metro_conv_f16_next_rebuild(const MetroConvDesc* d, const void* d_in, const void* d_w, const float* d_bias, const void* d_x,
                                const void* d_w_sc, const float* d_bias_sc, const void* d_pro_scale, const void* d_pro_shift,
                                const void* d_t2_prev, const void* d_w3_prev, const float* d_bias3_prev, void* d_out, void* d_out_sub,
                                int32_t sub_off, const void* d_w2, const float* d_bias2, const void* d_scale2, const void* d_shift2,
                                void* d_out2, int32_t c2, void* stream) {
    int st = validate_conv_desc(d);
    if (st) return st;
    METRO_CHECK_ARG(d_in && d_w && d_bias && d_x && d_w_sc && d_bias_sc && d_pro_scale && d_pro_shift && d_t2_prev && d_w3_prev && d_bias3_prev &&
                        d_w2 && d_bias2 && d_scale2 && d_shift2 && d_out2, "conv_f16_next_rebuild: NULL tensor pointer");
    METRO_CHECK_ARG((d_out != nullptr) != (d_out_sub != nullptr), "conv_f16_next_rebuild: exactly one of d_out (the whole sum) and d_out_sub (its "
                    "sub-sampled compact copy) must be given");
    METRO_CHECK_ARG(sub_off == 0 || sub_off == 1, "conv_f16_next_rebuild: sub_off %d must be 0 or 1", sub_off);
    ConvFused f;
    f.form = ConvForm::NextRebuild;
    f.next = {d_w2, d_bias2, d_scale2, d_shift2, d_out2, c2};
    f.psc = {d_x, d_w_sc, d_bias_sc, d_pro_scale, d_pro_shift};
    ConvRebuild& rb = f.rb;
    rb.t2_prev = d_t2_prev; rb.w3_prev = d_w3_prev; rb.bias3_prev = d_bias3_prev;
    if (d_out_sub != nullptr) {
        rb.out_mode = 2; rb.out_sub = d_out_sub; rb.sub_off = sub_off;
        rb.h_sub = (d->h_out - sub_off + 1) / 2; rb.w_sub = (d->w_out - sub_off + 1) / 2;
    }
    METRO_CHECK_ARG(conv_form_supported(*d, f), "conv_f16_next_rebuild: built for 1x1 stride-1 64 -> 256 without prologue / residual on maps "
                    "whose width is a power of two >= 16 and whose pixel count is a multiple of 64, c2 = 64 (block1/unit_2), fp16");
    return launch_conv_f16_dma(*d, d_in, d_w, d_bias, nullptr, nullptr, nullptr, d_out, static_cast<hipStream_t>(stream), f);
}

int metro_conv_b1_form(int32_t classic) {
    METRO_CHECK_ARG(classic == 0 || classic == 1, "metro_conv_b1_form: 0 (default dispatch) or 1 (classic single-role kernel)");
    conv_b1_set_form(classic);
    return METRO_OK;
}

int metro_conv_f16_gemm4w(const MetroConvDesc* d, const void* d_in, const void* d_w, const float* d_bias,
                          const void* d_pro_scale, const void* d_pro_shift, const void* d_residual, void* d_out,
                          int32_t split, void* d_out2, void* stream) {
    int st = validate_conv_desc(d);
    if (st) return st;
    METRO_CHECK_ARG(d_in && d_w && d_bias && d_out, "conv_f16_gemm4w: NULL tensor pointer");
    METRO_CHECK_ARG(!d->has_prologue || (d_pro_scale && d_pro_shift), "conv_f16_gemm4w: prologue tensors missing");
    METRO_CHECK_ARG(!d->has_residual || d_residual, "conv_f16_gemm4w: residual tensor missing");
    METRO_CHECK_ARG(split >= 0 && split < d->c_out && (split == 0 || d_out2), "conv_f16_gemm4w: bad split %d / missing second output", split);
    ConvSplit sp;
    sp.split = split; sp.c_out2 = d->c_out - split; sp.relu2 = 1; sp.out2 = d_out2;
    return launch_conv_gemm4w(*d, d_in, d_w, d_bias, d_pro_scale, d_pro_shift, d_residual, d_out,
                              static_cast<hipStream_t>(stream), split > 0 ? &sp : nullptr);
}

int metro_stem_pool_f16(const void* d_prepped, const void* d_w, const float* d_bias, void* d_out, int32_t n,
                        int32_t side, void* stream) {
    METRO_CHECK_ARG(d_prepped && d_w && d_bias && d_out, "stem_pool_f16: NULL tensor pointer");
    METRO_CHECK_ARG(n > 0, "stem_pool_f16: n = %d", n);
    METRO_CHECK_ARG(stem_pool_f16_supported(side, 64), "stem_pool_f16: side %d must be a multiple of 32 (and METRO_STEM_POOL != 0)", side);
    return launch_stem_pool_f16(d_prepped, d_w, d_bias, d_out, n, side, static_cast<hipStream_t>(stream));
}

int metro_stem_pool_f32in(const float* d_images, const void* d_w, const float* d_bias, void* d_out, int32_t n,
                          int32_t side, void* stream) {
    METRO_CHECK_ARG(d_images && d_w && d_bias && d_out, "stem_pool_f32in: NULL tensor pointer");
    METRO_CHECK_ARG(n > 0, "stem_pool_f32in: n = %d", n);
    METRO_CHECK_ARG(stem_pool_f32in_supported(side, 64), "stem_pool_f32in: side %d must be a multiple of 32 (and METRO_STEM_POOL / METRO_STEM_RAW != 0)", side);
    return launch_stem_pool_f32in(d_images, d_w, d_bias, d_out, n, side, static_cast<hipStream_t>(stream));
}

int metro_stem_pool_u8in(const uint8_t* d_images, const void* d_w, const float* d_bias, void* d_out, int32_t n,
                         int32_t side, void* stream) {
    METRO_CHECK_ARG(d_images && d_w && d_bias && d_out, "stem_pool_u8in: NULL tensor pointer");
    METRO_CHECK_ARG(n > 0, "stem_pool_u8in: n = %d", n);
    METRO_CHECK_ARG(stem_pool_f32in_supported(side, 64), "stem_pool_u8in: side %d must be a multiple of 32 (and METRO_STEM_POOL / METRO_STEM_RAW != 0)", side);
    return launch_stem_pool_u8in(d_images, d_w, d_bias, d_out, n, side, static_cast<hipStream_t>(stream));
}

int metro_images_u8_to_f32(const uint8_t* d_in, int64_t count, float* d_out, void* stream) {
    METRO_CHECK_ARG(d_in && d_out, "images_u8_to_f32: NULL pointer");
    METRO_CHECK_ARG(count > 0, "images_u8_to_f32: count = %lld", (long long)count);
    return launch_images_u8_to_f32(d_in, (long)count, d_out, static_cast<hipStream_t>(stream));
}

int metro_conv_f64acc(const MetroConvDesc* d, const void* d_in, const double* d_w, const double* d_bias,
                      const double* d_pro_scale, const double* d_pro_shift, const void* d_residual,
                      void* d_out, void* stream) {
    int st = validate_conv_desc(d);
    if (st) return st;
    METRO_CHECK_ARG((d->in_dtype == METRO_F32 || d->in_dtype == METRO_F64) && (d->out_dtype == METRO_F32 || d->out_dtype == METRO_F64) &&
                        !(d->in_dtype == METRO_F64 && d->out_dtype == METRO_F32),
                    "conv_f64acc: in/out dtypes must be F32/F32, F32/F64 or F64/F64");
    METRO_CHECK_ARG(d_in && d_w && d_bias && d_out, "conv_f64acc: NULL tensor pointer");
    METRO_CHECK_ARG(!d->has_prologue || (d_pro_scale && d_pro_shift), "conv_f64acc: prologue tensors missing");
    METRO_CHECK_ARG(!d->has_residual || d_residual, "conv_f64acc: residual tensor missing");
    return launch_conv_f64acc(*d, d_in, d_w, d_bias, d_pro_scale, d_pro_shift, d_residual, d_out,
                              static_cast<hipStream_t>(stream));
}

int metro_conv_f32m(const MetroConvDesc* d, const void* d_in, const float* d_w, const float* d_bias, const float* d_pro_scale,
                    const float* d_pro_shift, const void* d_residual, void* d_out, void* stream) {
    int st = validate_conv_desc(d);
    if (st) return st;
    METRO_CHECK_ARG(d->in_dtype == METRO_F32 && d->out_dtype == METRO_F32, "conv_f32m: in/out dtypes must be F32");
    METRO_CHECK_ARG(d_in && d_w && d_bias && d_out, "conv_f32m: NULL tensor pointer");
    METRO_CHECK_ARG(!d->has_prologue || (d_pro_scale && d_pro_shift), "conv_f32m: prologue tensors missing");
    METRO_CHECK_ARG(!d->has_residual || d_residual, "conv_f32m: residual tensor missing");
    return launch_conv_f32m(*d, d_in, d_w, d_bias, d_pro_scale, d_pro_shift, d_residual, d_out, static_cast<hipStream_t>(stream));
}

int metro_prep_input_f16(const float* d_images, int32_t n, int32_t side, void* d_out, void* stream) {
    METRO_CHECK_ARG(d_images && d_out && n > 0 && side > 0, "prep_input_f16: bad argument");
    return launch_prep_input_f16(d_images, n, side, d_out, static_cast<hipStream_t>(stream));
}

int metro_warp_crop_u8(const uint8_t* d_image, int32_t h, int32_t w, int32_t row_stride, const float* d_homographies,
                       int32_t n, int32_t side, float* d_out, void* stream) {
    METRO_CHECK_ARG(d_image && d_homographies && d_out, "warp_crop_u8: NULL pointer");
    METRO_CHECK_ARG(h > 0 && w > 0 && n > 0 && side > 0 && row_stride >= 3 * w, "warp_crop_u8: bad geometry (h %d w %d stride %d n %d side %d)", h, w, row_stride, n, side);
    METRO_CHECK_ARG(h <= 32767 && w <= 32767, "warp_crop_u8: frames larger than 32767 pixels a side are outside cv2.remap's short coordinates (h %d w %d)", h, w);
    return launch_warp_crop_u8(d_image, h, w, row_stride, d_homographies, d_out, n, side, static_cast<hipStream_t>(stream));
}

}

template <typename OutT>
static int warp_crops_frames_entry(const char* who, const MetroFrame* frames, int32_t n_frames, const MetroCropWarp* d_crops, int32_t n,
                                   int32_t side, OutT* d_out, void* stream) {
    METRO_CHECK_ARG(frames && d_crops && d_out, "%s: NULL pointer", who);
    METRO_CHECK_ARG(n_frames > 0 && n_frames <= METRO_MAX_FRAMES, "%s: %d frames (1 to %d per launch)", who,
                    n_frames, METRO_MAX_FRAMES);
    METRO_CHECK_ARG(n > 0 && side > 0, "%s: bad geometry (n %d side %d)", who, n, side);
    metro::FrameTable table = {};
    for (int i = 0; i < n_frames; ++i) {
        const MetroFrame& f = frames[i];
        METRO_CHECK_ARG(f.data, "%s: frame %d: NULL data pointer", who, i);
        METRO_CHECK_ARG(f.h <= 32767 && f.w <= 32767, "%s: frame %d: frames larger than 32767 pixels a side "
                        "are outside cv2.remap's short coordinates (h %d w %d)", who, i, f.h, f.w);
        METRO_CHECK_ARG(f.h > 0 && f.w > 0 && f.row_stride >= 3 * f.w,
                        "%s: frame %d: bad geometry (h %d w %d stride %d)", who, i, f.h, f.w, f.row_stride);
        table.f[i] = f;
    }
    return launch_warp_crops_frames_u8(table, n_frames, d_crops, n, side, d_out, static_cast<hipStream_t>(stream));
}

template <typename OutT>
static int warp_crops_frames_planes_entry(const char* who, const MetroFramePlanes* frames, int32_t n_frames, const MetroCropWarp* d_crops,
                                          int32_t n, int32_t side, OutT* d_out, void* stream) {
    METRO_CHECK_ARG(frames && d_crops && d_out, "%s: NULL pointer", who);
    METRO_CHECK_ARG(n_frames > 0 && n_frames <= METRO_MAX_FRAMES, "%s: %d frames (1 to %d per launch)", who,
                    n_frames, METRO_MAX_FRAMES);
    METRO_CHECK_ARG(n > 0 && side > 0, "%s: bad geometry (n %d side %d)", who, n, side);
    metro::FramePlanesTable table = {};
    for (int i = 0; i < n_frames; ++i) {
        const MetroFramePlanes& f = frames[i];
        METRO_CHECK_ARG(f.format >= METRO_PIX_RGB && f.format <= METRO_PIX_I420,
                        "%s: frame %d: unknown pixel format %d", who, i, f.format);
        METRO_CHECK_ARG(f.matrix == METRO_YUV_BT601 || f.matrix == METRO_YUV_BT709,
                        "%s: frame %d: unknown colour matrix %d", who, i, f.matrix);
        const bool yuv = f.format == METRO_PIX_NV12 || f.format == METRO_PIX_I420;
        const int n_planes = f.format == METRO_PIX_I420 ? 3 : f.format == METRO_PIX_NV12 ? 2 : 1;
        for (int k = 0; k < n_planes; ++k)
            METRO_CHECK_ARG(f.plane[k], "%s: frame %d: NULL plane %d", who, i, k);
        METRO_CHECK_ARG(f.h > 0 && f.w > 0 && f.h <= 32767 && f.w <= 32767, "%s: frame %d: h %d w %d "
                        "outside [1, 32767] (cv2.remap's short coordinates)", who, i, f.h, f.w);
        METRO_CHECK_ARG(!yuv || (f.h % 2 == 0 && f.w % 2 == 0),
                        "%s: frame %d: 4:2:0 frames need an even h and w (h %d w %d)", who, i, f.h, f.w);
        const int min_stride0 = yuv ? f.w : 3 * f.w;
        METRO_CHECK_ARG(f.stride[0] >= min_stride0, "%s: frame %d: stride[0] %d < %d", who, i, f.stride[0],
                        min_stride0);
        if (yuv) {
            const int min_stride1 = f.format == METRO_PIX_NV12 ? f.w : f.w / 2;
            METRO_CHECK_ARG(f.stride[1] >= min_stride1, "%s: frame %d: stride[1] %d < %d", who, i,
                            f.stride[1], min_stride1);
        }
        table.f[i] = f;
    }
    return launch_warp_crops_frames_planes(table, n_frames, d_crops, n, side, d_out, static_cast<hipStream_t>(stream));
}

extern "C" {

int metro_warp_crops_frames_u8(const MetroFrame* frames, int32_t n_frames, const MetroCropWarp* d_crops, int32_t n,
                               int32_t side, float* d_out, void* stream) {
// ... 446 lines not shown
```

### metro_pose3d_amd/csrc/executor.cpp

```cpp
#include <vector>

#include "plan.h"

using namespace metro;

namespace {

int launch_layer(const MetroPlan* p, const char* d_params, int li, const float* images, int n, float* poses, char* ws, hipStream_t stream, bool dump,
                 float* coords01 = nullptr, bool images_u8 = false, const MomentsOut& mo = MomentsOut{}) {
    const Layer& L = p->layers[li];
    auto slot_ptr = [&](int slot) -> void* {
        if (slot == S_IMAGES) return const_cast<float*>(images);
        if (slot < 0) return nullptr;
        return ws + p->slot_offset[slot];
    };
    auto prm = [&](int idx) -> const void* { return idx < 0 ? nullptr : d_params + p->params[idx].offset; };
    switch (L.kind) {
        case LK_PREP:
            if (images_u8)
                return launch_prep_input_u8_f16(reinterpret_cast<const unsigned char*>(images), n, p->spec.proc_side, slot_ptr(L.out_slot), stream);
            return launch_prep_input_f16(images, n, p->spec.proc_side, slot_ptr(L.out_slot), stream);
        case LK_POOL:
            return launch_maxpool(slot_ptr(L.in_slot), slot_ptr(L.out_slot), n, L.cd.h_in, L.cd.w_in, L.cd.c_in, p->act_dtype, stream);
        case LK_CONV: {
            MetroConvDesc cd = L.cd;
            cd.n = n;
            auto fprm = [&](int idx) { return static_cast<const float*>(prm(idx)); };
            void* in = slot_ptr(L.in_slot);
            void* out = slot_ptr(L.out_slot);
            const void* w = prm(L.main.w);
            const float* bias = fprm(L.main.bias);
            ConvFused f;
            switch (L.form) {
                case LayerForm::Head: {
                    float* logits_dump = dump ? static_cast<float*>(out) : nullptr;
                    return launch_head_f16(in, w, bias, prm(L.main.scale), prm(L.main.shift), n, L.cd.c_in, L.cd.c_out, p->spec.n_joints_head,
                                           p->spec.depth, L.cd.h_in, static_cast<float*>(slot_ptr(S_PART)), logits_dump, stream,
                                           static_cast<float*>(mo.scratch));
                }
                case LayerForm::StemPoolF32In:
                    if (images_u8)
                        return launch_stem_pool_u8in(reinterpret_cast<const unsigned char*>(images), w, bias, out, n, p->spec.proc_side, stream);
                    return launch_stem_pool_f32in(images, w, bias, out, n, p->spec.proc_side, stream);
                case LayerForm::StemPool:
                    return launch_stem_pool_f16(in, w, bias, out, n, p->spec.proc_side, stream);
                case LayerForm::Conv1Conv2: {
                    ConvPre1 p1;
                    p1.w1 = prm(L.conv1.w); p1.bias1 = fprm(L.conv1.bias);
                    p1.pro_scale = prm(L.conv1.scale); p1.pro_shift = prm(L.conv1.shift);
                    p1.t1_dump = dump ? slot_ptr(S_T1) : nullptr;
                    return launch_conv3x3_c64(cd, in, w, bias, out, stream, &p1);
                }
                case LayerForm::Plain:
                    if (p->fast)
                        return launch_conv_f16(cd, in, w, bias, prm(L.main.scale), prm(L.main.shift), slot_ptr(L.res_slot), out, stream);
                    if (p->spec.precision == METRO_PREC_F32M)
                        return launch_conv_f32m(cd, in, static_cast<const float*>(w), bias, fprm(L.main.scale), fprm(L.main.shift),
                                                slot_ptr(L.res_slot), out, stream);
                    return launch_conv_f64acc(cd, in, static_cast<const double*>(w), static_cast<const double*>(prm(L.main.bias)),
                                              static_cast<const double*>(prm(L.main.scale)), static_cast<const double*>(prm(L.main.shift)),
                                              slot_ptr(L.res_slot), out, stream);
                case LayerForm::Pair:
                    f.form = ConvForm::Pair;
                    f.pair = {L.cd.c_out - L.c2, L.c2, 1, slot_ptr(L.out2_slot)};
                    return launch_conv_f16_dma(cd, in, w, bias, prm(L.main.scale), prm(L.main.shift), nullptr, out, stream, f);
                case LayerForm::Next:
                case LayerForm::NextProj:
                case LayerForm::NextRebuild:
                    f.form = conv_form(L.form);
                    f.next = {prm(L.next.w), fprm(L.next.bias), prm(L.next.scale), prm(L.next.shift), slot_ptr(L.out2_slot), L.c2};
                    if (f.form != ConvForm::Next)
                        f.psc = {slot_ptr(L.psc_slot), prm(L.psc.w), fprm(L.psc.bias), prm(L.psc.scale), prm(L.psc.shift)};
                    if (f.form == ConvForm::NextRebuild) {
                        f.rb.t2_prev = slot_ptr(L.reb_slot); f.rb.w3_prev = prm(L.reb.w); f.rb.bias3_prev = fprm(L.reb.bias);
                    }
                    f.rb.out_mode = dump ? 0 : L.out_mode;
                    f.rb.classic = dump ? 1 : 0;
                    if (f.rb.out_mode == 2) { f.rb.out_sub = slot_ptr(L.sub_slot); f.rb.sub_off = L.sub_off; f.rb.h_sub = f.rb.w_sub = L.sub_side; }
                    return launch_conv_f16_dma(cd, in, w, bias, nullptr, nullptr, slot_ptr(L.res_slot), out, stream, f);
            }
            break;
        }
        case LK_SOFTARGMAX: {
            if (poses == nullptr) { set_error("metro_forward: poses_out is NULL"); return METRO_ERR_INVALID_ARG; }
            const SoftArgmaxArgs a = make_softargmax_args(p->spec, n);
            if (L.form == LayerForm::Head)
                return launch_softargmax_finalize(static_cast<const float*>(slot_ptr(S_PART)), a,
                                                  head_f16_records(n, L.head_c_in, a.depth * a.n_joints_head, a.side), poses, stream, coords01,
                                                  static_cast<int32_t*>(slot_ptr(S_STATUS)), mo);
            return launch_softargmax(slot_ptr(L.in_slot), a, p->spec.precision == METRO_PREC_F32M ? 1 : p->spec.precision, slot_ptr(S_PART), poses, stream,
                                     coords01, static_cast<int32_t*>(slot_ptr(S_STATUS)), mo);
        }
    }
    set_error("internal: layer %d has unknown kind %d", li, L.kind);
    return METRO_ERR_STATE;
}

int run_layers(MetroPlan* p, const float* images, int n, float* poses, void* ws_, hipStream_t stream,
               int last_layer, float* ms_out, float* coords01 = nullptr, bool images_u8 = false, const MomentsOut& mo = MomentsOut{}) {
    METRO_CHECK_ARG(p != nullptr, "plan is NULL");
    METRO_CHECK_ARG(n > 0 && n <= p->max_batch, "batch %d outside [1, %d]", n, p->max_batch);
    METRO_CHECK_ARG(images != nullptr && ws_ != nullptr, "NULL images/workspace pointer");
    if (p->d_params == nullptr) { set_error("metro_forward: parameters not bound (metro_plan_bind_params)"); return METRO_ERR_STATE; }
    char* ws = static_cast<char*>(ws_);
    const int nl = (int)p->layers.size();
    if (last_layer < 0 || last_layer >= nl) last_layer = nl - 1;

    std::vector<hipEvent_t> ev;
    if (ms_out) {
        ev.resize(2 * (last_layer + 1));
        for (auto& e : ev) METRO_HIP_CHECK(hipEventCreate(&e));
    }
    int st = METRO_OK;
    for (int li = 0; li <= last_layer && st == METRO_OK; ++li) {
        if (ms_out) METRO_HIP_CHECK(hipEventRecord(ev[2 * li], stream));
        st = launch_layer(p, p->d_params, li, images, n, poses, ws, stream, li == last_layer && li + 1 < nl, coords01, images_u8, mo);
        if (ms_out) METRO_HIP_CHECK(hipEventRecord(ev[2 * li + 1], stream));
    }
    if (ms_out) {
        if (st == METRO_OK) {
            METRO_HIP_CHECK(hipEventSynchronize(ev.back()));
            for (int li = 0; li <= last_layer; ++li) {
                float ms = 0.f;
                METRO_HIP_CHECK(hipEventElapsedTime(&ms, ev[2 * li], ev[2 * li + 1]));
                ms_out[li] += ms;
            }
        }
        for (auto& e : ev) (void)hipEventDestroy(e);
    }
    return st;
}

}

extern "C" {

int metro_plan_layer_kernel(const MetroPlan* plan, int32_t index, int32_t n, char* buf, int32_t buf_len) {
    METRO_CHECK_ARG(plan && buf && buf_len > 1 && index >= 0 && index < (int)plan->layers.size(), "metro_plan_layer_kernel: bad argument");
    METRO_CHECK_ARG(n > 0 && n <= plan->max_batch, "metro_plan_layer_kernel: batch %d outside [1, %d]", n, plan->max_batch);
    KernelNotes& kn = kernel_notes();
    const KernelNotes saved = kn;
    kn.mode = 2; kn.ids[0] = 0;
    static const char fake = 0;
    float dummy_poses = 0.f;
    const int st = launch_layer(plan, &fake, index, reinterpret_cast<const float*>(&fake), n, &dummy_poses,
                                const_cast<char*>(&fake), nullptr, false);
    snprintf(buf, (size_t)buf_len, "%s", kn.ids);
    kn = saved;
    return st;
}

int metro_plan_bind_params(MetroPlan* plan, const void* d_param_blob) {
    METRO_CHECK_ARG(plan && d_param_blob, "metro_plan_bind_params: NULL argument");
    METRO_CHECK_ARG(((uintptr_t)d_param_blob & 255) == 0, "parameter blob must be 256-byte aligned");
    plan->d_params = static_cast<const char*>(d_param_blob);
    for (GraphEntry& g : plan->graphs)
        if (g.exec) (void)hipGraphExecDestroy(g.exec);
    plan->graphs.clear();
    return METRO_OK;
}

int metro_plan_set_graph_max_batch(MetroPlan* plan, int32_t max_batch_for_graphs) {
    METRO_CHECK_ARG(plan != nullptr && max_batch_for_graphs >= 0, "metro_plan_set_graph_max_batch: bad argument");
    plan->graph_max_batch = max_batch_for_graphs;
    return METRO_OK;
}

static int forward_impl(MetroPlan* plan, const float* d_images_nhwc, int32_t n, float* d_poses_out, float* d_coords01,
                        void* d_workspace, void* stream_) {
    hipStream_t stream = static_cast<hipStream_t>(stream_);
    if (plan == nullptr || n > plan->graph_max_batch || n < 1)
        return run_layers(plan, d_images_nhwc, n, d_poses_out, d_workspace, stream, -1, nullptr, d_coords01);
    GraphEntry* hit = nullptr;
    for (GraphEntry& g : plan->graphs)
        if (g.n == n && g.images == d_images_nhwc && g.poses == d_poses_out && g.coords01 == d_coords01 && g.ws == d_workspace)
            hit = &g;
    if (hit == nullptr) {
        if (plan->graphs.size() >= 16) {
            if (plan->graphs.front().exec) (void)hipGraphExecDestroy(plan->graphs.front().exec);
            plan->graphs.erase(plan->graphs.begin());
        }
        plan->graphs.push_back(GraphEntry{n, d_images_nhwc, d_poses_out, d_coords01, d_workspace, stream, nullptr, 0});
        hit = &plan->graphs.back();
    }
    if (hit->exec == nullptr) {
        if (hit->eager_runs == 0) {
            hit->eager_runs = 1;
            return run_layers(plan, d_images_nhwc, n, d_poses_out, d_workspace, stream, -1, nullptr, d_coords01);
        }
        hipGraph_t graph = nullptr;
        if (plan->cap_stream == nullptr) METRO_HIP_CHECK(hipStreamCreateWithFlags(&plan->cap_stream, hipStreamNonBlocking));
        METRO_HIP_CHECK(hipStreamBeginCapture(plan->cap_stream, hipStreamCaptureModeThreadLocal));
        const int st = run_layers(plan, d_images_nhwc, n, d_poses_out, d_workspace, plan->cap_stream, -1, nullptr, d_coords01);
        const hipError_t e = hipStreamEndCapture(plan->cap_stream, &graph);
        if (st != METRO_OK) { if (graph) (void)hipGraphDestroy(graph); return st; }
        if (e != hipSuccess) { set_error("hipStreamEndCapture: %s", hipGetErrorString(e)); return METRO_ERR_HIP; }
        const hipError_t ei = hipGraphInstantiate(&hit->exec, graph, nullptr, nullptr, 0);
        (void)hipGraphDestroy(graph);
        if (ei != hipSuccess) { hit->exec = nullptr; set_error("hipGraphInstantiate: %s", hipGetErrorString(ei)); return METRO_ERR_HIP; }
    }
    METRO_HIP_CHECK(hipGraphLaunch(hit->exec, stream));
    return METRO_OK;
}

int metro_forward(MetroPlan* plan, const float* d_images_nhwc, int32_t n, float* d_poses_out,
                  void* d_workspace, void* stream) {
    return forward_impl(plan, d_images_nhwc, n, d_poses_out, nullptr, d_workspace, stream);
}

int metro_forward_coords01(MetroPlan* plan, const float* d_images_nhwc, int32_t n, float* d_poses_out,
                           float* d_coords01_out, void* d_workspace, void* stream) {
    METRO_CHECK_ARG(d_coords01_out != nullptr && d_poses_out != nullptr, "metro_forward_coords01: NULL poses / coords01 pointer");
    return forward_impl(plan, d_images_nhwc, n, d_poses_out, d_coords01_out, d_workspace, stream);
}

int metro_forward_u8(MetroPlan* plan, const uint8_t* d_images_nhwc, int32_t n, float* d_poses_out, float* d_coords01_out,
                     void* d_workspace, void* stream) {
    METRO_CHECK_ARG(plan != nullptr, "metro_forward_u8: plan is NULL");
    METRO_CHECK_ARG(plan->spec.precision == METRO_PREC_F16,
                    "metro_forward_u8: uint8 crops run on f16 plans only; for this precision expand them with metro_images_u8_to_f32 "
                    "and call metro_forward");
    METRO_CHECK_ARG(d_poses_out != nullptr, "metro_forward_u8: NULL poses pointer");
    METRO_CHECK_ARG(((uintptr_t)d_images_nhwc & 15) == 0, "metro_forward_u8: uint8 crops must start at a 16-byte aligned address (got %p)",
                    (const void*)d_images_nhwc);
    return run_layers(plan, reinterpret_cast<const float*>(d_images_nhwc), n, d_poses_out, d_workspace, static_cast<hipStream_t>(stream), -1,
                      nullptr, d_coords01_out, true);
}

int64_t metro_moments_scratch_bytes(const MetroSpec* spec, int32_t n) {
    if (spec == nullptr || n <= 0 || spec->stride <= 0 || spec->proc_side / spec->stride < 2 || spec->n_joints_head <= 0) return -1;
    return moments_scratch_bytes(n, spec->proc_side / spec->stride, spec->n_joints_head);
}

int metro_forward_moments(MetroPlan* plan, const void* d_images_nhwc, int32_t images_u8, int32_t n, float* d_poses_out,
                          float* d_coords01_out, float* d_cov01_out, float* d_peak_out, void* d_moments_scratch,
                          void* d_workspace, void* stream) {
    METRO_CHECK_ARG(plan != nullptr, "metro_forward_moments: plan is NULL");
    METRO_CHECK_ARG(d_poses_out != nullptr, "metro_forward_moments: NULL poses pointer");
    METRO_CHECK_ARG(images_u8 == 0 || images_u8 == 1, "metro_forward_moments: images_u8 must be 0 or 1 (got %d)", images_u8);
    METRO_CHECK_ARG(!images_u8 || plan->spec.precision == METRO_PREC_F16,
                    "metro_forward_moments: uint8 crops run on f16 plans only; for this precision expand them with "
                    "metro_images_u8_to_f32");
    METRO_CHECK_ARG(!images_u8 || ((uintptr_t)d_images_nhwc & 15) == 0,
                    "metro_forward_moments: uint8 crops must start at a 16-byte aligned address (got %p)", d_images_nhwc);
    METRO_CHECK_ARG((d_cov01_out != nullptr) == (d_peak_out != nullptr) && (d_cov01_out != nullptr) == (d_moments_scratch != nullptr),
                    "metro_forward_moments: cov01_out, peak_out and the moments scratch go together (all three or none)");
    METRO_CHECK_ARG(((uintptr_t)d_moments_scratch & 15) == 0, "metro_forward_moments: the moments scratch must be 16-byte aligned");
    MomentsOut mo;
    mo.scratch = d_moments_scratch; mo.cov01 = d_cov01_out; mo.peak = d_peak_out;
    return run_layers(plan, static_cast<const float*>(d_images_nhwc), n, d_poses_out, d_workspace, static_cast<hipStream_t>(stream), -1,
                      nullptr, d_coords01_out, images_u8 != 0, mo);
}

int metro_forward_status(const MetroPlan* plan, const void* d_workspace, int32_t n, void* stream_, int32_t* n_nonfinite_out) {
    METRO_CHECK_ARG(plan && d_workspace && n_nonfinite_out, "metro_forward_status: NULL argument");
    METRO_CHECK_ARG(n > 0 && n <= plan->max_batch, "metro_forward_status: batch %d outside [1, %d]", n, plan->max_batch);
    hipStream_t stream = static_cast<hipStream_t>(stream_);
    std::vector<int32_t> host((size_t)n);
    METRO_HIP_CHECK(hipMemcpyAsync(host.data(), static_cast<const char*>(d_workspace) + plan->slot_offset[S_STATUS], (size_t)n * 4,
                                   hipMemcpyDeviceToHost, stream));
    METRO_HIP_CHECK(hipStreamSynchronize(stream));
    int32_t bad = 0;
    for (int32_t v : host) bad += v != 0;
    *n_nonfinite_out = bad;
    if (bad) {
        set_error("%d of %d crops reached the soft-argmax with non-finite statistics%s", bad, n,
                  plan->spec.precision == METRO_PREC_F16 ? " (fp16 storage overflows at 65504: run this model with precision f32m or f64)" : "");
        return METRO_ERR_NONFINITE;
    }
    return METRO_OK;
}


int metro_forward_upto(MetroPlan* plan, const float* d_images_nhwc, int32_t n, float* d_poses_out,
                       void* d_workspace, void* stream, int32_t last_layer) {
    return run_layers(plan, d_images_nhwc, n, d_poses_out, d_workspace, static_cast<hipStream_t>(stream), last_layer, nullptr);
}

int metro_forward_timed(MetroPlan* plan, const float* d_images_nhwc, int32_t n, float* d_poses_out,
                        void* d_workspace, void* stream, float* ms_out) {
    METRO_CHECK_ARG(ms_out != nullptr, "metro_forward_timed: ms_out is NULL");
    return run_layers(plan, d_images_nhwc, n, d_poses_out, d_workspace, static_cast<hipStream_t>(stream), -1, ms_out);
}

}
```

### metro_pose3d_amd/csrc/metro_common.h

```cpp
#pragma once
#include <hip/hip_runtime.h>
#include <cstdarg>
#include <cstdint>
#include <cstdio>
#include <cstdlib>

#include "../../include/metro_hip.h"

namespace metro {

void set_error(const char* fmt, ...);
const char* get_error();

#define METRO_CHECK_ARG(cond, ...)                  \
    do {                                            \
        if (!(cond)) {                              \
            ::metro::set_error(__VA_ARGS__);        \
            return METRO_ERR_INVALID_ARG;           \
        }                                           \
    } while (0)

#define METRO_HIP_CHECK(expr)                                                              \
    do {                                                                                   \
        hipError_t _e = (expr);                                                            \
// ... 74 lines not shown
    }
}

constexpr int METRO_MAX_DEVICES = 64;
struct PerDeviceInt { int v[METRO_MAX_DEVICES]; };

inline int current_device_slot(int* slot) {
    int dev = 0;
    const hipError_t e = hipGetDevice(&dev);
    if (e != hipSuccess || dev < 0 || dev >= METRO_MAX_DEVICES) {
        set_error("hipGetDevice: %s (device %d; at most %d devices per process)", hipGetErrorString(e), dev, METRO_MAX_DEVICES);
        return METRO_ERR_HIP;
    }
    *slot = dev;
    return METRO_OK;
}

inline int ensure_dyn_lds(const void* kern, int bytes, PerDeviceInt& done, const char* what) {
    int slot = 0;
    const int st = current_device_slot(&slot);
    if (st) return st;
    if (done.v[slot]) return METRO_OK;
    const hipError_t e = hipFuncSetAttribute(kern, hipFuncAttributeMaxDynamicSharedMemorySize, bytes);
    if (e != hipSuccess) {
        set_error("hipFuncSetAttribute(%s, %d B of LDS, device %d): %s", what, bytes, slot, hipGetErrorString(e));
        return METRO_ERR_HIP;
    }
    done.v[slot] = 1;
    return METRO_OK;
}

inline int ensure_dyn_lds_and_grid_cap(const void* kern, int threads, int bytes, PerDeviceInt& cap, const char* what,
                                       int max_blocks_per_cu, int* grid_cap) {
    int slot = 0;
    int st = current_device_slot(&slot);
    if (st) return st;
    if (cap.v[slot] == 0) {
        const hipError_t e = hipFuncSetAttribute(kern, hipFuncAttributeMaxDynamicSharedMemorySize, bytes);
        if (e != hipSuccess) {
            set_error("hipFuncSetAttribute(%s, %d B of LDS, device %d): %s", what, bytes, slot, hipGetErrorString(e));
            return METRO_ERR_HIP;
        }
        int cus = 0, occ = 0;
        METRO_HIP_CHECK(hipDeviceGetAttribute(&cus, hipDeviceAttributeMultiprocessorCount, slot));
        if (const int lim = tuning_knob("METRO_CU_LIMIT", 0); lim > 0 && lim < cus) cus = lim;
        METRO_HIP_CHECK(hipOccupancyMaxActiveBlocksPerMultiprocessor(&occ, kern, threads, bytes));
        if (occ < 1) occ = 1;
        if (max_blocks_per_cu > 0 && occ > max_blocks_per_cu) occ = max_blocks_per_cu;
        cap.v[slot] = cus * occ;
    }
    *grid_cap = cap.v[slot];
    return METRO_OK;
}

inline int launch_status(const char* what) {
    if (kernel_notes().mode == 2) {
        set_error("internal: %s was launched during a dry run (note_kernel must come first)", what);
        return METRO_ERR_STATE;
    }
    hipError_t e = hipGetLastError();
    if (e != hipSuccess) {
        set_error("launch of %s failed: %s", what, hipGetErrorString(e));
        return METRO_ERR_HIP;
    }
    return METRO_OK;
}

struct ConvSplit {
    int split = 0;
    int c_out2 = 0;
    int relu2 = 0;
    void* out2 = nullptr;
};

struct ConvFuse2 {
    const void* w2 = nullptr;
    const float* bias2 = nullptr;
    const void* scale2 = nullptr;
    const void* shift2 = nullptr;
    void* out2 = nullptr;
    int c2 = 0;
};

struct ConvPre1 {
    const void* w1 = nullptr;
    const float* bias1 = nullptr;
    const void* pro_scale = nullptr;
    const void* pro_shift = nullptr;
    void* t1_dump = nullptr;
};

struct ConvProjSc {
    const void* x = nullptr;
    const void* w_sc = nullptr;
    const float* bias_sc = nullptr;
    const void* pro_scale = nullptr;
    const void* pro_shift = nullptr;
};

struct ConvRebuild {
    const void* t2_prev = nullptr;
    const void* w3_prev = nullptr;
    const float* bias3_prev = nullptr;
    int out_mode = 0;
    void* out_sub = nullptr;
    int sub_off = 0, h_sub = 0, w_sub = 0;
    int classic = 0;
};

enum class ConvForm { Plain, Pair, Next, NextProj, NextRebuild };

struct ConvFused {
    ConvForm form = ConvForm::Plain;
    ConvSplit pair;
    ConvFuse2 next;
    ConvProjSc psc;
    ConvRebuild rb;
};

struct ConvArgs {
    int split, c_out2, relu2;
    int n, h_in, w_in, c_in, in_pix_stride;
    int h_out, w_out, c_out;
    int kh, kw, stride, dil, pad_top, pad_left;
    int res_h, res_w, res_stride, res_offset;
    int m_total;
    int relu;
};

inline ConvArgs make_conv_args(const MetroConvDesc& d) {
    ConvArgs a;
    a.split = 0; a.c_out2 = 0; a.relu2 = 0;
    a.n = d.n; a.h_in = d.h_in; a.w_in = d.w_in; a.c_in = d.c_in; a.in_pix_stride = d.in_pix_stride;
    a.h_out = d.h_out; a.w_out = d.w_out; a.c_out = d.c_out;
    a.kh = d.kh; a.kw = d.kw; a.stride = d.stride; a.dil = d.dilation;
    a.pad_top = d.pad_top; a.pad_left = d.pad_left;
    a.res_h = d.res_h; a.res_w = d.res_w; a.res_stride = d.res_stride; a.res_offset = d.res_offset;
    a.m_total = d.n * d.h_out * d.w_out;
    a.relu = d.relu;
    return a;
}

int validate_conv_desc(const MetroConvDesc* d);

int launch_conv_f16(const MetroConvDesc& d, const void* in, const void* w, const float* bias,
                    const void* pro_scale, const void* pro_shift, const void* residual, void* out,
                    hipStream_t stream);
bool conv_f16_dma_supported(const MetroConvDesc& d);
int launch_conv_f16_dma(const MetroConvDesc& d, const void* in, const void* w, const float* bias,
                        const void* pro_scale, const void* pro_shift, const void* residual, void* out,
                        hipStream_t stream, const ConvFused& f = ConvFused{});
bool conv_form_supported(const MetroConvDesc& d, const ConvFused& f);
bool conv_f16_fuse2_supported(const MetroConvDesc& d, int c2);
bool conv_gemm4w_shape_ok(const MetroConvDesc& d, const ConvSplit* split);
bool conv_gemm4w_supported(const MetroConvDesc& d, const ConvSplit* split);
int launch_conv_gemm4w(const MetroConvDesc& d, const void* in, const void* w, const float* bias, const void* pro_scale,
                       const void* pro_shift, const void* residual, void* out, hipStream_t stream, const ConvSplit* split);
bool conv_pw64_supported(const MetroConvDesc& d, const ConvFused& f);
int launch_conv_pw64(const MetroConvDesc& d, const void* in, const void* w, const float* bias, const void* pro_scale,
                     const void* pro_shift, const void* residual, void* out, hipStream_t stream, const ConvFused& f);
bool conv_b1_chain_preferred();
void conv_b1_set_form(int classic);
bool classic_forms_forced();
bool conv_pws_supported(const MetroConvDesc& d);
int launch_conv_pws(const MetroConvDesc& d, const void* in, const void* w, const float* bias, const void* res, void* out, hipStream_t stream);
int launch_conv_b1_chain(const MetroConvDesc& d, const void* in, const void* w, const float* bias, void* out, hipStream_t stream,
                         const ConvFused& f);
bool stem_pool_f16_supported(int side, int base_width);
int launch_stem_pool_f16(const void* prepped, const void* w, const float* bias, void* out, int n, int side,
                         hipStream_t stream);
bool stem_pool_f32in_supported(int side, int base_width);
int launch_stem_pool_f32in(const float* images, const void* w, const float* bias, void* out, int n, int side,
                           hipStream_t stream);
int launch_stem_pool_u8in(const unsigned char* images, const void* w, const float* bias, void* out, int n, int side,
                          hipStream_t stream);
bool conv3x3_c64_supported(const MetroConvDesc& d);
int launch_conv3x3_c64(const MetroConvDesc& d, const void* in, const void* w, const float* bias, void* out, hipStream_t stream,
                       const ConvPre1* pre1 = nullptr);
bool conv3x3_slab_supported(const MetroConvDesc& d);
int launch_conv3x3_slab(const MetroConvDesc& d, const void* in, const void* w, const float* bias, void* out,
                        hipStream_t stream);
int launch_conv_f64acc(const MetroConvDesc& d, const void* in, const double* w, const double* bias,
                       const double* pro_scale, const double* pro_shift, const void* residual,
                       void* out, hipStream_t stream);
int launch_conv_f32m(const MetroConvDesc& d, const void* in, const float* w, const float* bias, const float* pro_scale,
                     const float* pro_shift, const void* residual, void* out, hipStream_t stream);
int launch_prep_input_f16(const float* images, int n, int side, void* out, hipStream_t stream);
int launch_prep_input_u8_f16(const unsigned char* images, int n, int side, void* out, hipStream_t stream);
int launch_images_u8_to_f32(const unsigned char* in, long count, float* out, hipStream_t stream);
struct FrameTable { MetroFrame f[METRO_MAX_FRAMES]; };
template <typename OutT>
int launch_warp_crops_frames_u8(const FrameTable& frames, int n_frames, const MetroCropWarp* crops, int n, int side,
                                OutT* out, hipStream_t stream);
struct FramePlanesTable { MetroFramePlanes f[METRO_MAX_FRAMES]; };
template <typename OutT>
int launch_warp_crops_frames_planes(const FramePlanesTable& frames, int n_frames, const MetroCropWarp* crops, int n,
                                    int side, OutT* out, hipStream_t stream);
template <typename OutT>
int launch_warp_crop_u8(const unsigned char* img, int h, int w, int row_stride, const float* homs, OutT* out,
                        int n, int side, hipStream_t stream);
int launch_eval_metrics(const float* pred, const float* truth, const unsigned char* valid, int n, int nj,
                        float threshold, float* dist, float* dist_pa, double* sums, hipStream_t stream);
int launch_maxpool(const void* in, void* out, int n, int h_in, int w_in, int c, int dtype,
                   hipStream_t stream);

struct SoftArgmaxArgs {
    int n, side, depth, n_joints_head, n_joints_out;
    int lrc, half_off;
    float box_size_mm;
    int proc_side;
    int perm[METRO_MAX_JOINTS];
};
struct MomentsOut {
    void* scratch = nullptr;
    float* cov01 = nullptr;
    float* peak = nullptr;
};
int64_t moments_scratch_bytes(int n, int side, int n_joints_head);
int softargmax_slabs(int n, int side);
int64_t softargmax_scratch_bytes(int n, int side, int n_joints_head);
int launch_softargmax(const void* logits, const SoftArgmaxArgs& a, int precise, void* partials,
                      float* poses_out, hipStream_t stream, float* coords01_out = nullptr, int32_t* status = nullptr,
                      const MomentsOut& mo = MomentsOut{});
int launch_softargmax_finalize(const float* partials, const SoftArgmaxArgs& a, int slabs, float* poses_out,
                               hipStream_t stream, float* coords01_out = nullptr, int32_t* status = nullptr,
                               const MomentsOut& mo = MomentsOut{});
bool head_f16_supported(int c_in, int c_head, int n_joints, int depth, int side);
int head_f16_slabs(int side);
int head_f16_records(int n, int c_in, int c_head, int side);
int launch_head_f16(const void* x, const void* w, const float* bias, const void* pro_scale, const void* pro_shift,
                    int n, int c_in, int c_head, int n_joints, int depth, int side, float* partials, float* logits_out,
                    hipStream_t stream, float* moments = nullptr);
int launch_backproject(const float* coords01, const float* inv_k, const double* targets, int per_pose_targets,
                       const float* root_z, const int* edges, int n, int nj, int ne, const MetroSpec& spec,
                       int root_relative, int permute, float* out, float* z_out, hipStream_t stream);
int launch_heatmap_to_25d(const float* coords01, float* out, int n, const MetroSpec& spec, hipStream_t stream);
int launch_to_orig_cam(const float* x, const float* rot, const int* mirror, float* out, int n, int nj, hipStream_t stream);
int launch_place_poses(const float* coords01, const float* poses, const MetroPlacement* rec, int n, const MetroSpec& spec,
                       int scale, const double* targets, int per_pose_targets, const float* root_z, const int* edges, int ne,
                       const int* mirror, int coords, float* out, float* keypoints, float* z_out, hipStream_t stream);
SoftArgmaxArgs make_softargmax_args(const MetroSpec& spec, int n);
int launch_expand_views(const MetroViewBase* bases, int n, const MetroView* views, int n_views, int side, MetroCropWarp* crops,
                        MetroPlacement* places, hipStream_t stream);
int launch_merge_views(const float* poses, const float* keypoints, const float* z, const MetroPlacement* rec, const int* mirror,
                       int n, int n_views, int nj, float* poses_out, float* keypoints_out, float* z_out, float* spread_out,
                       hipStream_t stream);
int launch_place_covariances(const float* cov01, const float* peak, const MetroPlacement* rec, int n, int n_views,
                             const MetroSpec& spec, const int* mirror, int coords, float* cov_out, float* peak_out,
                             hipStream_t stream);
int launch_triangulate_joints(const float* coords01, const float* cov01, const MetroPlacement* rec, int m, const int* rows,
                              int n_rows, const int* starts, int n_persons, const MetroSpec& spec, const int* mirror, int weights,
                              double min_det, float* points, int* n_rays, float* residual, float* cov, hipStream_t stream);
int launch_view_affinity(const float* coords01, const float* cov01, const MetroPlacement* rec, const MetroSpec& spec,
                         const int* mirror, const int* frame_index, const int* step_index, int n, int n_views, int weights,
                         double min_sin2, double clip_mm, int min_pairs, float* cost, int* n_pairs, hipStream_t stream);
int launch_cluster_views(const float* cost, int n, int n_views, float max_cost, int* person_index, int* n_persons, int* rows,
                         int* starts, hipStream_t stream);
int launch_person_steps(const int* rows, int n_rows, const int* starts, const int* n_persons, int n, int n_views, const int* box_step,
                        int n_boxes, const double* step_times, int n_steps, int* person_step, double* person_times, int* step_rows,
                        int* step_starts, hipStream_t stream);
size_t smooth_tracks_workspace_bytes(int n_rows, int n_out);
int launch_smooth_tracks(const float* poses, const float* cov, const double* times, int n, const int* rows, int n_rows,
                         const int* starts, int n_tracks, int n_out, int mode, int measurement, double q, double r_floor,
                         double cov_scale, double v0, double gate, double* state, void* workspace, float* poses_out,
                         float* velocity_out, float* cov_out, unsigned char* used_out, hipStream_t stream);
size_t associate_tracks_workspace_bytes(int n_tracks, int n_out);
int launch_associate_tracks(const float* poses, const float* cov, const double* times, int n, const int* step_rows, int n_step_rows,
                            const int* step_starts, int n_steps, int n_out, int measurement, double q, double r_floor,
                            double cov_scale, double v0, double gate, float max_cost_mm, double clip_mm, int min_joints,
                            double max_age_s, double* state, int n_tracks, int* ids, int* next_id, void* workspace, int* track_index,
                            int* track_id, float* cost_out, int* rows_out, int* starts_out, int* n_new, int* n_dropped,
                            hipStream_t stream);
int launch_look_at_boxes(const double* boxes, const int32_t* frame_index, int n, int n_frames, const MetroFrameCamera* cameras,
                         int n_cameras, int side, MetroViewBase* out, int32_t* status, hipStream_t stream);

}
```

### metro_pose3d_amd/csrc/plan.h

```cpp
#pragma once
#include <cstring>
#include <vector>

#include "metro_common.h"

namespace metro {

enum LayerKind { LK_PREP = 0, LK_CONV = 1, LK_POOL = 2, LK_SOFTARGMAX = 3 };
enum Slot { S_IMAGES = -2, S_NONE = -1, S_PREP = 0, S_STEM, S_X0, S_X1, S_T1, S_T2, S_T2B, S_SC, S_LOGITS, S_PART, S_STATUS, S_COUNT };

inline int dtype_bytes(int dtype) { return dtype == METRO_F16 ? 2 : dtype == METRO_F32 ? 4 : 8; }

struct ConvParams { int w = -1, bias = -1, scale = -1, shift = -1; };

enum class LayerForm { Plain, Pair, Next, NextProj, NextRebuild, Conv1Conv2, StemPool, StemPoolF32In, Head };
inline ConvForm conv_form(LayerForm f) { return static_cast<ConvForm>(f); }
static_assert((int)LayerForm::Plain == (int)ConvForm::Plain && (int)LayerForm::Pair == (int)ConvForm::Pair &&
              (int)LayerForm::Next == (int)ConvForm::Next && (int)LayerForm::NextProj == (int)ConvForm::NextProj &&
              (int)LayerForm::NextRebuild == (int)ConvForm::NextRebuild, "LayerForm starts with ConvForm's values");

struct Layer {
    Layer() { memset(&info, 0, sizeof(info)); }
    MetroLayerInfo info;
    int kind = LK_CONV;
    LayerForm form = LayerForm::Plain;
    MetroConvDesc cd{};
    int in_slot = S_NONE, out_slot = S_NONE, res_slot = S_NONE;
    ConvParams main;
    ConvParams conv1;
    ConvParams next;
    ConvParams psc;
    ConvParams reb;
    int c2 = 0, out2_slot = S_NONE;
    int psc_slot = S_NONE, reb_slot = S_NONE;
    int out_mode = 0, sub_slot = S_NONE, sub_off = 0, sub_side = 0;
    int head_c_in = 0;
};

struct GraphEntry {
    int n;
    const void* images;
    const void* poses;
    const void* coords01;
    const void* ws;
    hipStream_t stream;
    hipGraphExec_t exec;
    int eager_runs;
};

}

struct MetroPlan {
    std::vector<metro::GraphEntry> graphs;
    hipStream_t cap_stream = nullptr;
    int graph_max_batch = 0;
    MetroSpec spec;
    int max_batch;
    bool fast;
    int act_dtype;
    int act_bytes;
    std::vector<MetroParamInfo> params;
    std::vector<metro::Layer> layers;
    int64_t slot_bytes_per_image[metro::S_COUNT] = {}, slot_offset[metro::S_COUNT] = {};
    int64_t workspace_bytes = 0, param_bytes = 0;
    const char* d_params = nullptr;
    double flops_per_image = 0.0;
};
```

### metro_pose3d_amd/csrc/planner.cpp

```cpp
#include <algorithm>
#include <cmath>
#include <string>

#include "plan.h"

using namespace metro;

namespace {

int64_t align_up(int64_t v, int64_t a) { return (v + a - 1) / a * a; }

int tf_same_pad_beg(int in, int k_eff, int s) {
    const int out = (in + s - 1) / s;
    return std::max((out - 1) * s + k_eff - in, 0) / 2;
}

int stem_side(int proc_side) { return (proc_side + 6 - 7) / 2 + 1; }
int pool_side(int s2) { return (s2 + 2 - 3) / 2 + 1; }

struct UnitGeom {
    int block, unit, n_units;
    int c_in, width, c_out;
    int side_in, side_out, stride, rate;
    bool centered, project;
// ... 157 lines not shown
    int wdt() const { return p->fast ? METRO_F16 : p->spec.precision == METRO_PREC_F32M ? METRO_F32 : METRO_F64; }
    int bdt() const { return p->fast || p->spec.precision == METRO_PREC_F32M ? METRO_F32 : METRO_F64; }

    ConvParams conv_params(const std::string& lname, const std::string& scope, const std::string& bn_fold,
                           const std::string& prologue_bn, int c_out, int k, int c_in) {
        const std::string conv_var = root + "/" + scope, bn_var = bn_fold.empty() ? "" : root + "/" + bn_fold;
        ConvParams g;
        g.w = add_param(lname + "/W", METRO_PARAM_CONV_W, conv_var, bn_var, wdt(), {c_out, k, k, c_in, k, c_in});
        g.bias = add_param(lname + "/bias", METRO_PARAM_BIAS, conv_var, bn_var, bdt(), {c_out});
        if (!prologue_bn.empty()) {
            g.scale = add_param(lname + "/pro_scale", METRO_PARAM_PRO_SCALE, "", root + "/" + prologue_bn, wdt(), {c_in});
            g.shift = add_param(lname + "/pro_shift", METRO_PARAM_PRO_SHIFT, "", root + "/" + prologue_bn, wdt(), {c_in});
        }
        return g;
    }

    void need(int slot, int64_t bytes) { if (slot >= 0) p->slot_bytes_per_image[slot] = std::max(p->slot_bytes_per_image[slot], bytes); }
    void fill_info(Layer& L, const std::string& lname, double flops) {
        MetroLayerInfo& I = L.info;
        const MetroConvDesc& cd = L.cd;
        snprintf(I.name, sizeof(I.name), "%s", lname.c_str());
        I.kind = L.kind; I.h_in = cd.h_in; I.w_in = cd.w_in; I.c_in = cd.c_in; I.h_out = cd.h_out; I.w_out = cd.w_out; I.c_out = cd.c_out;
        I.kh = cd.kh; I.kw = cd.kw; I.stride = cd.stride; I.dilation = cd.dilation; I.pad_top = cd.pad_top; I.pad_left = cd.pad_left;
        I.has_prologue = cd.has_prologue; I.relu = cd.relu; I.has_residual = cd.has_residual;
        I.res_stride = cd.res_stride; I.res_offset = cd.res_offset; I.out_dtype = cd.out_dtype;
        I.flops_per_image = flops; p->flops_per_image += flops;
    }
    void add_fused_flops(Layer& L, int side, int c_out, int c_in) {
        const double flops = 2.0 * side * side * (double)c_out * c_in;
        L.info.flops_per_image += flops; p->flops_per_image += flops;
    }

    MetroConvDesc conv_desc(const ConvSpec& c) const {
        MetroConvDesc cd{};
        cd.h_in = cd.w_in = c.side_in; cd.c_in = c.c_in; cd.in_pix_stride = c.c_in;
        cd.h_out = cd.w_out = c.side_out; cd.c_out = c.c_out;
        cd.kh = cd.kw = c.k; cd.stride = c.stride; cd.dilation = c.rate; cd.pad_top = cd.pad_left = c.pad_beg;
        cd.has_prologue = !c.prologue_bn.empty(); cd.relu = c.relu; cd.has_residual = c.res_slot != S_NONE;
        cd.res_h = cd.res_w = c.res_side; cd.res_stride = c.res_stride; cd.res_offset = c.res_offset;
        cd.out_dtype = c.out_dtype < 0 ? p->act_dtype : c.out_dtype; cd.in_dtype = c.in_dtype < 0 ? p->act_dtype : c.in_dtype;
        return cd;
    }

    Layer conv(const ConvSpec& c) {
        Layer L;
        const MetroConvDesc& cd = L.cd = conv_desc(c);
        L.main = conv_params(c.name, c.scope, c.bn_fold, c.prologue_bn, c.c_out, c.k, c.c_in);
        L.in_slot = c.in_slot; L.out_slot = c.out_slot; L.res_slot = c.res_slot;
        need(c.out_slot, (int64_t)c.side_out * c.side_out * c.c_out * dtype_bytes(cd.out_dtype));
        fill_info(L, c.name, (double)2.0 * c.side_out * c.side_out * c.c_out * c.k * c.k * c.c_in);
        return L;
    }

    int shortcut_conv1_pair(const UnitGeom& g, int in_slot, Layer* out) {
        Layer& L = *out;
        const int side = g.side_in;
        L.form = LayerForm::Pair;
        L.cd = conv_desc({g.name + "/shortcut+conv1", "", "", g.scope + "/preact", in_slot, S_SC, side, g.c_in, side, g.c_out + g.width});
        const std::string sc = root + "/" + g.scope + "/shortcut", c1 = root + "/" + g.scope + "/conv1", pre = root + "/" + g.scope + "/preact";
        const ParamShape w_sc = {g.c_out, 1, 1, g.c_in, 1, g.c_in}, w_c1 = {g.width, 1, 1, g.c_in, 1, g.c_in};
        L.main.w = add_param(g.name + "/shortcut/W", METRO_PARAM_CONV_W, sc, "", METRO_F16, w_sc);
        L.conv1.w = add_param(g.name + "/conv1/W", METRO_PARAM_CONV_W, c1, c1 + "/BatchNorm", METRO_F16, w_c1);
        L.main.bias = add_param(g.name + "/shortcut/bias", METRO_PARAM_BIAS, sc, "", METRO_F32, {g.c_out});
        L.conv1.bias = add_param(g.name + "/conv1/bias", METRO_PARAM_BIAS, c1, c1 + "/BatchNorm", METRO_F32, {g.width});
        if (p->params[L.conv1.w].offset != p->params[L.main.w].offset + p->params[L.main.w].bytes ||
            p->params[L.conv1.bias].offset != p->params[L.main.bias].offset + p->params[L.main.bias].bytes) {
            set_error("internal: fused pair parameters of %s are not contiguous in the blob", g.name.c_str());
            return METRO_ERR_STATE;
        }
        L.main.scale = add_param(g.name + "/shortcut/pro_scale", METRO_PARAM_PRO_SCALE, "", pre, METRO_F16, {g.c_in});
        L.main.shift = add_param(g.name + "/shortcut/pro_shift", METRO_PARAM_PRO_SHIFT, "", pre, METRO_F16, {g.c_in});
        L.in_slot = in_slot; L.out_slot = S_SC; L.c2 = g.width; L.out2_slot = S_T1;
        need(S_SC, (int64_t)side * side * g.c_out * 2); need(S_T1, (int64_t)side * side * g.width * 2);
        fill_info(L, g.name + "/shortcut+conv1", 2.0 * side * side * (double)(g.c_out + g.width) * g.c_in);
        L.info.c_out = g.c_out;
        return METRO_OK;
    }

    void fuse_conv1_in_front(Layer& L, const UnitGeom& g, int x_slot) {
        L.conv1 = conv_params(g.name + "/conv1", g.scope + "/conv1", g.scope + "/conv1/BatchNorm", g.scope + "/preact", g.width, 1, g.c_in);
        L.form = LayerForm::Conv1Conv2; L.in_slot = x_slot;
        snprintf(L.info.name, sizeof(L.info.name), "%s/conv1+conv2", g.name.c_str());
        L.info.fused_flags |= METRO_FUSED_CONV1_IN_FRONT;
        add_fused_flops(L, g.side_in, g.width, g.c_in);
    }

    void fuse_projection_shortcut(Layer& L, const UnitGeom& g, int x_slot) {
        L.psc = conv_params(g.name + "/shortcut", g.scope + "/shortcut", "", g.scope + "/preact", g.c_out, 1, g.c_in);
        L.form = LayerForm::NextProj; L.psc_slot = x_slot;
        L.info.fused_flags |= METRO_FUSED_PROJECTION_SHORTCUT;
        add_fused_flops(L, g.side_in, g.c_out, g.c_in);
    }

    void fuse_next_conv1(Layer& L, const UnitGeom& nx) {
        L.next = conv_params(nx.name + "/conv1", nx.scope + "/conv1", nx.scope + "/conv1/BatchNorm", nx.scope + "/preact", nx.width, 1, nx.c_in);
        L.c2 = nx.width; L.out2_slot = S_T1;
        if (L.form == LayerForm::Plain) L.form = LayerForm::Next;
        need(S_T1, (int64_t)nx.side_in * nx.side_in * nx.width * 2);
        const std::string name = std::string(L.info.name) + "+" + nx.name.substr(nx.name.find('/') + 1) + "/conv1";
        snprintf(L.info.name, sizeof(L.info.name), "%s", name.c_str());
        add_fused_flops(L, nx.side_in, nx.width, nx.c_in);
    }

    int prev3 = -1;
    int emit_unit(const UnitGeom& g, const UnitFusion& f, const UnitGeom* next_unit, int* x_slot) {
        const std::string &un = g.name, &sc = g.scope;
        const int x = *x_slot;
        const int out = f.shortcut == ShortcutFrom::RebuiltInConv3 ? x : x == S_X0 ? S_X1 : S_X0;
        if (f.conv1 == Conv1At::Pair) {
            Layer L;
            if (const int st = shortcut_conv1_pair(g, x, &L)) return st;
            p->layers.push_back(L);
        } else if (f.conv1 == Conv1At::OwnLaunch) {
            if (f.shortcut == ShortcutFrom::OwnLaunch) {
                ConvSpec c{un + "/shortcut", sc + "/shortcut", "", sc + "/preact", x, S_SC, g.side_in, g.c_in, g.side_out, g.c_out};
                c.stride = g.stride; c.pad_beg = -g.shift;
                p->layers.push_back(conv(c));
            }
            ConvSpec c{un + "/conv1", sc + "/conv1", sc + "/conv1/BatchNorm", sc + "/preact", x, S_T1, g.side_in, g.c_in, g.side_in, g.width};
            c.relu = true;
            p->layers.push_back(conv(c));
        }
        const int t2 = f.sum == SumTo::OnChip ? S_T2B : S_T2;
        ConvSpec c2{un + "/conv2", sc + "/conv2", sc + "/conv2/BatchNorm", "", S_T1, t2, g.side_in, g.width, g.side_out, g.width};
        c2.k = 3; c2.stride = g.stride; c2.rate = g.rate; c2.pad_beg = g.pad_beg; c2.relu = true;
        Layer L2 = conv(c2);
        if (f.conv1 == Conv1At::FrontOfConv2) fuse_conv1_in_front(L2, g, x);
        p->layers.push_back(L2);
        ConvSpec c3{un + "/conv3", sc + "/conv3", "", "", t2, f.sum == SumTo::SubSampled ? S_SC : out, g.side_out, g.width, g.side_out, g.c_out};
        if (f.shortcut == ShortcutFrom::OwnLaunch || f.shortcut == ShortcutFrom::Pair) {
            c3.res_slot = S_SC; c3.res_side = g.side_out;
        } else if (f.shortcut == ShortcutFrom::Identity || f.shortcut == ShortcutFrom::Compact) {
            c3.res_slot = x; c3.res_side = g.side_in; c3.res_stride = g.stride; c3.res_offset = g.shift;
        }
        Layer L3 = conv(c3);
        if (f.shortcut == ShortcutFrom::Compact) {
            L3.cd.res_h = L3.cd.res_w = g.side_out; L3.cd.res_stride = 1; L3.cd.res_offset = 0;
            L3.info.fused_flags |= METRO_FUSED_COMPACT_SHORTCUT;
        } else if (f.shortcut == ShortcutFrom::InConv3) {
            fuse_projection_shortcut(L3, g, x);
        } else if (f.shortcut == ShortcutFrom::RebuiltInConv3) {
            const Layer& L1 = p->layers[prev3];
            L3.info.has_residual = 1;
            L3.info.fused_flags |= METRO_FUSED_REBUILT_SHORTCUT; L3.form = LayerForm::NextRebuild;
            L3.reb.w = L1.main.w; L3.reb.bias = L1.main.bias; L3.reb_slot = L1.in_slot;
            L3.psc = L1.psc; L3.psc_slot = L1.psc_slot;
        }
        if (f.sum != SumTo::Stored) L3.info.fused_flags |= METRO_FUSED_OUT_ON_CHIP;
        L3.out_mode = f.sum == SumTo::Stored ? 0 : f.sum == SumTo::OnChip ? 1 : 2;
        if (f.sum == SumTo::SubSampled) { L3.sub_slot = out; L3.sub_off = f.sub_off; L3.sub_side = f.sub_side; }
        if (f.carries_next_conv1) fuse_next_conv1(L3, *next_unit);
        p->layers.push_back(L3);
        prev3 = (int)p->layers.size() - 1;
        *x_slot = out;
        return METRO_OK;
    }
};

void layout_workspace(MetroPlan* p, bool head_fused);

int build_plan(MetroPlan* p) {
    const MetroSpec& sp = p->spec;
    Builder B{p, std::string("MainPart/resnet_v2_") + std::to_string(sp.arch)};
    const bool fast = p->fast;
    const int adt = p->act_dtype, aes = p->act_bytes, side = sp.proc_side, bw = sp.base_width;

    const int s2 = stem_side(side), s4 = pool_side(s2);
    bool fused_stem_pool = false;
    const bool raw_stem = fast && stem_pool_f32in_supported(side, bw);
    if (fast && !raw_stem) {
        Layer L;
        L.kind = LK_PREP;
        L.cd.h_in = L.cd.w_in = side; L.cd.c_in = 3;
        L.cd.h_out = side + 6; L.cd.w_out = side + 8; L.cd.c_out = 4; L.cd.out_dtype = METRO_F16;
        L.in_slot = S_IMAGES; L.out_slot = S_PREP;
        B.need(S_PREP, (int64_t)(side + 6) * (side + 8) * 4 * 2);
        B.fill_info(L, "prep_input", 0.0);
        p->layers.push_back(L);
    }
    if (fast) {
        Layer S;
        MetroConvDesc& cd = S.cd;
        cd.h_in = side + 6; cd.w_in = side + 8; cd.c_in = 32; cd.in_pix_stride = 4;
        cd.h_out = cd.w_out = s2; cd.c_out = bw;
        cd.kh = 7; cd.kw = 1; cd.stride = 2; cd.dilation = 1; cd.pad_top = cd.pad_left = 0;
        cd.out_dtype = adt; cd.in_dtype = METRO_F16;
        const std::string cv = B.root + "/conv1";
        S.main.w = B.add_param("conv1/W", METRO_PARAM_CONV_W, cv, "", METRO_F16, {bw, 7, 7, 3, 8, 4});
        S.main.bias = B.add_param("conv1/bias", METRO_PARAM_BIAS, cv, "", METRO_F32, {bw});
        S.in_slot = S_PREP; S.out_slot = S_STEM;
        if (stem_pool_f16_supported(side, bw)) {
            fused_stem_pool = true;
            S.form = raw_stem ? LayerForm::StemPoolF32In : LayerForm::StemPool;
            if (raw_stem) S.in_slot = S_IMAGES;
            S.out_slot = S_X0;
            B.need(S_X0, (int64_t)s4 * s4 * bw * aes);
            B.fill_info(S, "conv1+pool1", 2.0 * s2 * s2 * bw * 7 * 7 * 3);
            S.info.h_out = S.info.w_out = s4;
            S.cd.h_out = S.cd.w_out = s4;
        } else {
            B.need(S_STEM, (int64_t)s2 * s2 * bw * aes);
            B.fill_info(S, "conv1", 2.0 * s2 * s2 * bw * 7 * 7 * 3);
        }
        p->layers.push_back(S);
    } else {
        ConvSpec c{"conv1", "conv1", "", "", S_IMAGES, S_STEM, side, 3, s2, bw};
        c.k = 7; c.stride = 2; c.pad_beg = 3; c.in_dtype = METRO_F32;
        p->layers.push_back(B.conv(c));
    }
    if (!fused_stem_pool) {
        Layer L;
        L.kind = LK_POOL;
        L.cd.h_in = L.cd.w_in = s2; L.cd.c_in = bw; L.cd.h_out = L.cd.w_out = s4; L.cd.c_out = bw;
        L.cd.kh = L.cd.kw = 3; L.cd.stride = 2; L.cd.dilation = 1; L.cd.pad_top = L.cd.pad_left = 1;
        L.cd.out_dtype = adt;
        L.in_slot = S_STEM; L.out_slot = S_X0;
        B.need(S_X0, (int64_t)s4 * s4 * bw * aes);
        B.fill_info(L, "pool1", 0.0);
        p->layers.push_back(L);
    }

    std::vector<UnitGeom> units;
    std::vector<UnitFusion> fusions;
    int st = unit_geometry(sp, &units);
    if (st == METRO_OK) st = choose_fusion(units, fast, &fusions);
    int cur = S_X0;
    for (size_t i = 0; i < units.size() && st == METRO_OK; ++i)
        st = B.emit_unit(units[i], fusions[i], i + 1 < units.size() ? &units[i + 1] : nullptr, &cur);
    if (st != METRO_OK) return st;
    const int cur_side = units.back().side_out, cur_c = units.back().c_out;

    const int c_head = sp.depth * sp.n_joints_head;
    ConvSpec lg{"logits", "logits", "", "postnorm", cur, S_LOGITS, cur_side, cur_c, cur_side, c_head};
    lg.out_dtype = sp.precision == METRO_PREC_F64 ? METRO_F64 : METRO_F32;
    Layer logits = B.conv(lg);
    const bool head_fused = fast && head_f16_supported(cur_c, c_head, sp.n_joints_head, sp.depth, cur_side);
    if (head_fused) logits.form = LayerForm::Head;
    p->layers.push_back(logits);

    Layer L;
    L.kind = LK_SOFTARGMAX;
    L.cd.h_in = L.cd.w_in = cur_side; L.cd.c_in = c_head; L.cd.h_out = 1; L.cd.w_out = sp.n_joints_out;
    L.cd.c_out = 3; L.cd.out_dtype = METRO_F32;
    L.in_slot = S_LOGITS;
    L.form = head_fused ? LayerForm::Head : LayerForm::Plain;
    L.head_c_in = cur_c;
    B.fill_info(L, "softargmax", 0.0);
    p->layers.push_back(L);

    layout_workspace(p, head_fused);
    return METRO_OK;
}

void layout_workspace(MetroPlan* p, bool head_fused) {
    const MetroSpec& sp = p->spec;
    const bool fast = p->fast;
    int64_t off = 0, aes = p->act_bytes;
    for (int s = 0; s < S_COUNT; ++s) {
        p->slot_offset[s] = off;
        int64_t bytes = p->slot_bytes_per_image[s] * p->max_batch;
        if (s == S_PART) {
            const int hs = sp.proc_side / sp.stride;
            bytes = softargmax_scratch_bytes(p->max_batch, hs, sp.n_joints_head);
            if (head_fused)
                bytes = std::max(bytes, (int64_t)p->max_batch * head_f16_slabs(hs) * sp.n_joints_head * 5 * 4);
        }
        if (s == S_STATUS) bytes = (int64_t)p->max_batch * 4;
        off = align_up(off + bytes, 256);
    }
    p->workspace_bytes = off;
    for (Layer& L : p->layers) {
        L.info.out_offset = L.out_slot >= 0 ? p->slot_offset[L.out_slot] : -1;
        L.info.out_sub_offset = L.out_mode == 2 ? p->slot_offset[L.sub_slot] : -1;
        L.info.out_sub_side = L.out_mode == 2 ? L.sub_side : 0;
        L.info.out_sub_off = L.out_mode == 2 ? L.sub_off : 0;
        const int64_t es = dtype_bytes(L.cd.out_dtype);
        L.info.out_bytes_per_image = (int64_t)L.cd.h_out * L.cd.w_out * (L.form == LayerForm::Pair ? L.cd.c_out - L.c2 : L.cd.c_out) * es;
        const bool two = L.out2_slot != S_NONE;
        L.info.out2_offset = two ? p->slot_offset[L.out2_slot] : -1;
        L.info.out2_channels = two ? L.c2 : 0;
        if (L.form == LayerForm::Conv1Conv2) {
            L.info.out2_offset = p->slot_offset[S_T1];
            L.info.out2_channels = p->params[L.conv1.w].c_out;
        }
        const int64_t in_es = L.in_slot == S_IMAGES ? 4 : (L.kind == LK_SOFTARGMAX ? (sp.precision == METRO_PREC_F64 ? 8 : 4)
                                                           : (L.kind == LK_CONV && !fast ? aes : (L.kind == LK_CONV ? 2 : aes)));
        int64_t act = 0;
        if (L.in_slot == S_IMAGES) act += (int64_t)sp.proc_side * sp.proc_side * 3 * 4;
        else if (L.kind == LK_CONV && L.cd.in_pix_stride != L.cd.c_in) act += (int64_t)L.cd.h_in * L.cd.w_in * L.cd.in_pix_stride * in_es;
        else act += (int64_t)L.cd.h_in * L.cd.w_in * L.cd.c_in * in_es;
        if (L.kind == LK_SOFTARGMAX) act += (int64_t)sp.n_joints_out * 3 * 4;
        else if (L.out_mode == 0) act += L.info.out_bytes_per_image;
        else if (L.out_mode == 2) act += (int64_t)L.sub_side * L.sub_side * L.cd.c_out * es;
        if (L.reb.w >= 0) act += (int64_t)L.cd.h_out * L.cd.w_out * p->params[L.reb.w].c_in * es;
        if (two) act += (int64_t)L.cd.h_out * L.cd.w_out * L.info.out2_channels * es;
        if (L.kind == LK_CONV && L.cd.has_residual) act += (int64_t)L.cd.h_out * L.cd.w_out * L.cd.c_out * es;
        if (L.psc.w >= 0) act += (int64_t)L.cd.h_out * L.cd.w_out * p->params[L.psc.w].c_in * es;
        if (L.form == LayerForm::Head) {
            const int64_t part = (int64_t)head_f16_slabs(sp.proc_side / sp.stride) * sp.n_joints_head * 5 * 4;
            if (L.kind == LK_CONV) act = (int64_t)L.cd.h_in * L.cd.w_in * L.cd.c_in * 2 + part;
            else act = part + (int64_t)sp.n_joints_out * 3 * 4;
        }
        L.info.algo_act_bytes_per_image = act;
        int64_t pb = 0;
        for (const ConvParams& g : {L.main, L.conv1, L.next, L.psc, L.reb})
            for (int idx : {g.w, g.bias, g.scale, g.shift})
// ... 74 lines not shown
```

### metro_pose3d_amd/engine.py

```python
from __future__ import annotations

import ctypes as C
from typing import Dict, List, Optional

import numpy as np
import torch

from metro_pose3d_amd import _lib
from metro_pose3d_amd._lib import check
from metro_pose3d_amd.spec import ModelSpec

BN_EPS = 1e-5

_NP_DTYPE = {_lib.METRO_F16: np.float16, _lib.METRO_F32: np.float32, _lib.METRO_F64: np.float64}
_PRECISIONS = {'f16': _lib.METRO_PREC_F16, 'f32': _lib.METRO_PREC_F32, 'f64': _lib.METRO_PREC_F64, 'f32m': _lib.METRO_PREC_F32M}


def _bn_scale_shift(params: Dict[str, np.ndarray], bn: str):
    g = params[bn + '/gamma'].astype(np.float64)
    b = params[bn + '/beta'].astype(np.float64)
    m = params[bn + '/moving_mean'].astype(np.float64)
    v = params[bn + '/moving_variance'].astype(np.float64)
    scale = g / np.sqrt(v + BN_EPS)
    return scale, b - m * scale


def pack_param(info: _lib.MetroParamInfo, params: Dict[str, np.ndarray]) -> np.ndarray:
    conv = info.conv_var.decode()
    bn = info.bn_var.decode()
    dt = _NP_DTYPE[info.dtype]
    if info.kind == _lib.PARAM_CONV_W:
        w = params[conv + '/weights'].astype(np.float64)
        if w.shape != (info.kh, info.kw, info.c_in, info.c_out):
            raise ValueError(f'{conv}/weights has shape {w.shape}, plan expects '
                             f'{(info.kh, info.kw, info.c_in, info.c_out)}')
        if bn:
            w = w * _bn_scale_shift(params, bn)[0]
        packed = np.zeros((info.c_out, info.kh, info.kw_pad, info.c_in_pad), dtype=np.float64)
        packed[:, :, :info.kw, :info.c_in] = w.transpose(3, 0, 1, 2)
        return packed.astype(dt)
    if info.kind == _lib.PARAM_BIAS:
        v = _bn_scale_shift(params, bn)[1] if bn else params[conv + '/biases'].astype(np.float64)
    elif info.kind == _lib.PARAM_PRO_SCALE:
        v = _bn_scale_shift(params, bn)[0]
    elif info.kind == _lib.PARAM_PRO_SHIFT:
        v = _bn_scale_shift(params, bn)[1]
    else:
        raise ValueError(f'unknown parameter kind {info.kind}')
    if v.shape != (info.c_out,):
        raise ValueError(f'{info.name.decode()}: length {v.shape} != {info.c_out}')
    return v.astype(dt)


class Engine:

    def __init__(self, spec: ModelSpec, params: Optional[Dict[str, np.ndarray]],
                 precision: str = 'f16', max_batch: int = 64, device: Optional[torch.device] = None):
        if precision not in _PRECISIONS:
            raise ValueError(f"precision must be 'f16', 'f32', 'f32m' or 'f64', got {precision!r}")
        self.lib = _lib.load()
        self.spec = spec
        self.precision = precision
        self.max_batch = int(max_batch)
        self._plan = C.c_void_p()
        cspec = spec.to_c(_PRECISIONS[precision])
        check(self.lib.metro_plan_create(C.byref(cspec), self.max_batch, C.byref(self._plan)),
              'metro_plan_create')
        self.cspec = cspec
        import os
        gmax = int(os.environ.get('METRO_HIPGRAPH_MAX_BATCH', '0'))
        check(self.lib.metro_plan_set_graph_max_batch(self._plan, gmax), 'metro_plan_set_graph_max_batch')
        self.device = None
        self._blob = None
        self._ws = None
        self._u8_f32 = None
        self._moments = None
        if params is not None:
            if device is None:
                if not torch.cuda.is_available():
                    raise _lib.MetroError('no HIP device visible: the MeTRo hot path has no CPU fallback')
                device = torch.device('cuda', torch.cuda.current_device())
            self.bind(params, device)

    def param_infos(self) -> List[_lib.MetroParamInfo]:
        out = []
        for i in range(self.lib.metro_plan_num_params(self._plan)):
            pi = _lib.MetroParamInfo()
            check(self.lib.metro_plan_param_info(self._plan, i, C.byref(pi)), 'metro_plan_param_info')
            out.append(pi)
        return out

    def layer_infos(self) -> List[_lib.MetroLayerInfo]:
        out = []
        for i in range(self.lib.metro_plan_num_layers(self._plan)):
            li = _lib.MetroLayerInfo()
            check(self.lib.metro_plan_layer_info(self._plan, i, C.byref(li)), 'metro_plan_layer_info')
            out.append(li)
        return out

    def layer_kernels(self, n: int) -> List[str]:
        out = []
        buf = C.create_string_buffer(1024)
        for i in range(self.lib.metro_plan_num_layers(self._plan)):
            check(self.lib.metro_plan_layer_kernel(self._plan, i, int(n), buf, len(buf)), 'metro_plan_layer_kernel')
            out.append(buf.value.decode())
        return out

    @property
    def flops_per_image(self) -> float:
        return float(self.lib.metro_plan_flops_per_image(self._plan))

    @property
    def workspace_bytes(self) -> int:
        return int(self.lib.metro_plan_workspace_bytes(self._plan))

    @property
    def param_bytes(self) -> int:
        return int(self.lib.metro_plan_param_bytes(self._plan))

    def pack_params(self, params: Dict[str, np.ndarray]) -> np.ndarray:
        blob = np.zeros(self.param_bytes, dtype=np.uint8)
        for pi in self.param_infos():
            t = pack_param(pi, params)
            raw = np.ascontiguousarray(t).view(np.uint8).reshape(-1)
            if raw.size != pi.bytes:
                raise ValueError(f'{pi.name.decode()}: packed {raw.size} bytes, plan expects {pi.bytes}')
            blob[pi.offset:pi.offset + pi.bytes] = raw
        return blob

    def bind(self, params: Dict[str, np.ndarray], device: torch.device) -> None:
        self.device = torch.device(device)
        blob = self.pack_params(params)
        with torch.cuda.device(self.device):
            self._blob = torch.from_numpy(blob).to(self.device)
            self._ws = torch.empty(self.workspace_bytes, dtype=torch.uint8, device=self.device)
            if self._blob.data_ptr() % 256 or self._ws.data_ptr() % 256:
                raise _lib.MetroError('torch returned a device buffer that is not 256-byte aligned')
            check(self.lib.metro_plan_bind_params(self._plan, C.c_void_p(self._blob.data_ptr())),
                  'metro_plan_bind_params')

    def _check_images(self, images: torch.Tensor) -> torch.Tensor:
        s = self.spec.proc_side
        if self._blob is None:
            raise _lib.MetroError('Engine has no parameters bound')
        if not isinstance(images, torch.Tensor):
            raise ValueError('images must be a torch.Tensor on the GPU')
        if images.dim() != 4 or tuple(images.shape[1:]) != (s, s, 3):
            raise ValueError(f'images must be [N,{s},{s},3] NHWC, got {tuple(images.shape)}')
        if images.dtype not in (torch.float32, torch.uint8):
            raise ValueError(f'images must be float32 in [0,1] or uint8 (byte b = b / 255), got {images.dtype}')
        if images.device != self.device:
            raise ValueError(f'images are on {images.device}, the plan is on {self.device}')
        if images.shape[0] < 1 or images.shape[0] > self.max_batch:
            raise ValueError(f'batch {images.shape[0]} outside [1, {self.max_batch}]')
        images = images.contiguous()
        if images.dtype == torch.uint8 and images.data_ptr() % 16:
            images = images.clone()
        return images

    def _as_float32(self, images: torch.Tensor) -> torch.Tensor:
        n, s = images.shape[0], self.spec.proc_side
        if self._u8_f32 is None:
            self._u8_f32 = torch.empty((self.max_batch, s, s, 3), dtype=torch.float32, device=self.device)
        out = self._u8_f32[:n]
        stream = torch.cuda.current_stream(self.device).cuda_stream
        check(self.lib.metro_images_u8_to_f32(C.c_void_p(images.data_ptr()), images.numel(), C.c_void_p(out.data_ptr()),
                                              C.c_void_p(stream)), 'metro_images_u8_to_f32')
        return out

    def forward(self, images: torch.Tensor, out: Optional[torch.Tensor] = None,
                coords01: Optional[torch.Tensor] = None, cov01: Optional[torch.Tensor] = None,
                peak: Optional[torch.Tensor] = None) -> torch.Tensor:
        images = self._check_images(images)
        n = images.shape[0]
        if (cov01 is None) != (peak is None):
            raise ValueError('cov01 and peak go together: pass both or neither')
        if cov01 is not None:
            self._check_out('cov01', cov01, (n, self.spec.skeleton.n_head, 6))
            self._check_out('peak', peak, (n, self.spec.skeleton.n_head))
        if out is None:
            out = torch.empty((n, self.spec.skeleton.n_out, 3), dtype=torch.float32, device=self.device)
        stream = torch.cuda.current_stream(self.device).cuda_stream
        if coords01 is not None:
            self._check_coords01(coords01, n)
        if cov01 is not None:
            u8 = images.dtype == torch.uint8 and self.precision == 'f16'
            if images.dtype == torch.uint8 and not u8:
                images = self._as_float32(images)
            if self._moments is None:
                nb = int(self.lib.metro_moments_scratch_bytes(C.byref(self.cspec), self.max_batch))
                self._moments = torch.empty(nb, dtype=torch.uint8, device=self.device)
            check(self.lib.metro_forward_moments(self._plan, C.c_void_p(images.data_ptr()), int(u8), n, C.c_void_p(out.data_ptr()),
                                                 C.c_void_p(coords01.data_ptr() if coords01 is not None else 0),
                                                 C.c_void_p(cov01.data_ptr()), C.c_void_p(peak.data_ptr()),
                                                 C.c_void_p(self._moments.data_ptr()), C.c_void_p(self._ws.data_ptr()),
                                                 C.c_void_p(stream)), 'metro_forward_moments')
            return out
        if images.dtype == torch.uint8:
            if self.precision == 'f16':
                check(self.lib.metro_forward_u8(self._plan, C.c_void_p(images.data_ptr()), n, C.c_void_p(out.data_ptr()),
                                                C.c_void_p(coords01.data_ptr() if coords01 is not None else 0),
                                                C.c_void_p(self._ws.data_ptr()), C.c_void_p(stream)), 'metro_forward_u8')
                return out
            images = self._as_float32(images)
        if coords01 is None:
            check(self.lib.metro_forward(self._plan, C.c_void_p(images.data_ptr()), n,
                                         C.c_void_p(out.data_ptr()), C.c_void_p(self._ws.data_ptr()),
                                         C.c_void_p(stream)), 'metro_forward')
            return out
        check(self.lib.metro_forward_coords01(self._plan, C.c_void_p(images.data_ptr()), n, C.c_void_p(out.data_ptr()),
                                              C.c_void_p(coords01.data_ptr()), C.c_void_p(self._ws.data_ptr()),
                                              C.c_void_p(stream)), 'metro_forward_coords01')
        return out

    def _check_coords01(self, coords01, n: int) -> None:
        shape = (n, self.spec.skeleton.n_head, 3)
        if (not isinstance(coords01, torch.Tensor) or coords01.dtype != torch.float32 or tuple(coords01.shape) != shape
                or coords01.device != self.device or not coords01.is_contiguous()):
            raise ValueError(f'coords01 must be a contiguous float32 {list(shape)} tensor on {self.device}, got '
                             f'{getattr(coords01, "dtype", type(coords01))} {tuple(getattr(coords01, "shape", ()))}')

    def _check_out(self, name: str, t, shape) -> None:
        if (not isinstance(t, torch.Tensor) or t.dtype != torch.float32 or tuple(t.shape) != tuple(shape)
                or t.device != self.device or not t.is_contiguous()):
            raise ValueError(f'{name} must be a contiguous float32 {list(shape)} tensor on {self.device}, got '
                             f'{getattr(t, "dtype", type(t))} {tuple(getattr(t, "shape", ()))}')

    def check_finite(self, n: int) -> None:
        stream = torch.cuda.current_stream(self.device).cuda_stream
        bad = C.c_int32(0)
        check(self.lib.metro_forward_status(self._plan, C.c_void_p(self._ws.data_ptr()), int(n), C.c_void_p(stream), C.byref(bad)),
              f'{self.spec.arch_name} stride {self.spec.stride} in precision {self.precision!r}')

    def status_words(self, n: int) -> torch.Tensor:
        off = int(self.lib.metro_plan_status_offset(self._plan))
        return self._ws[off:off + 4 * int(n)].view(torch.int32)

    def forward_upto(self, images: torch.Tensor, layer: int, second: bool = False) -> torch.Tensor:
        images = self._check_images(images)
        if images.dtype == torch.uint8:
            images = self._as_float32(images)
        n = images.shape[0]
        li = self.layer_infos()[layer]
        poses = torch.empty((n, self.spec.skeleton.n_out, 3), dtype=torch.float32, device=self.device)
        stream = torch.cuda.current_stream(self.device).cuda_stream
        check(self.lib.metro_forward_upto(self._plan, C.c_void_p(images.data_ptr()), n,
                                          C.c_void_p(poses.data_ptr()), C.c_void_p(self._ws.data_ptr()),
                                          C.c_void_p(stream), layer), 'metro_forward_upto')
        if li.kind == _lib.LAYER_SOFTARGMAX:
            return poses
        dt = {_lib.METRO_F16: torch.float16, _lib.METRO_F32: torch.float32,
              _lib.METRO_F64: torch.float64}[li.out_dtype]
        if second:
            if li.out2_offset < 0:
                raise ValueError(f'{li.name.decode()}: layer has no second output')
            nb2 = li.h_out * li.w_out * li.out2_channels * 2 * n
            return self._ws[li.out2_offset:li.out2_offset + nb2].view(torch.float16).view(
                n, li.h_out, li.w_out, li.out2_channels).clone()
        nbytes = li.out_bytes_per_image * n
# ... 32 lines not shown
```

Before: 47980.

## Fuse bottleneck conv2 and conv3 with residual add into one kernel

Adds a FUSE3 path to the DMA implicit-GEMM conv kernel. For stride-2 bottleneck units it computes conv2, keeps the bias+ReLU result tile in LDS, then runs the 1x1 conv3 over four output slabs from LDS-staged weights and adds the residual before storing. The executor groups these layer pairs into one launch when a preference check passes, and the planner marks eligible pairs. The aim is to drop the global write and reread of the conv2 activation and one launch per unit. The cost is a more complex LDS schedule, higher LDS and register pressure, and fewer possible tilings.

```diff
diff --git a/include/metro_hip.h b/include/metro_hip.h
--- a/include/metro_hip.h
+++ b/include/metro_hip.h
@@ -94,6 +94,10 @@
 int  metro_plan_layer_info(const MetroPlan* plan, int32_t index, MetroLayerInfo* out);
 double metro_plan_flops_per_image(const MetroPlan* plan);
 int  metro_plan_layer_kernel(const MetroPlan* plan, int32_t index, int32_t n, char* buf, int32_t buf_len);
+int32_t metro_plan_num_launches(const MetroPlan* plan, int32_t n);
+int  metro_plan_launch_info(const MetroPlan* plan, int32_t n, int32_t index, int32_t* first_layer, int32_t* n_layers, char* buf,
+                            int32_t buf_len);
+int  metro_plan_set_launch_groups(MetroPlan* plan, int32_t on);
 int  metro_kernel_notes(int32_t mode);
 const char* metro_last_kernel_id(void);
 int  metro_plan_bind_params(MetroPlan* plan, const void* d_param_blob);
@@ -147,6 +151,11 @@
                                  const void* d_t2_prev, const void* d_w3_prev, const float* d_bias3_prev, void* d_out, void* d_out_sub,
                                  int32_t sub_off, const void* d_w2, const float* d_bias2, const void* d_scale2, const void* d_shift2,
                                  void* d_out2, int32_t c2, void* stream);
+int  metro_conv_f16_conv2_conv3_supported(const MetroConvDesc* d, int32_t c_out3, int32_t res_stride, int32_t res_offset, int32_t res_h,
+                                          int32_t res_w);
+int  metro_conv_f16_conv2_conv3(const MetroConvDesc* d, const void* d_in, const void* d_w2, const float* d_bias2, const void* d_w3,
+                                const float* d_bias3, int32_t c_out3, const void* d_residual, int32_t res_stride, int32_t res_offset,
+                                int32_t res_h, int32_t res_w, void* d_out, void* stream);
 int  metro_conv_b1_form(int32_t classic);
 int  metro_conv_f16_gemm4w(const MetroConvDesc* d, const void* d_in, const void* d_w, const float* d_bias,
                            const void* d_pro_scale, const void* d_pro_shift, const void* d_residual, void* d_out,
diff --git a/metro_pose3d_amd/_lib.py b/metro_pose3d_amd/_lib.py
--- a/metro_pose3d_amd/_lib.py
+++ b/metro_pose3d_amd/_lib.py
@@ -134,6 +134,9 @@
     'metro_kernel_notes': (C.c_int, [C.c_int32]),
     'metro_last_kernel_id': (C.c_char_p, []),
     'metro_plan_set_graph_max_batch': (C.c_int, [_P, C.c_int32]),
+    'metro_plan_num_launches': (C.c_int32, [_P, C.c_int32]),
+    'metro_plan_launch_info': (C.c_int, [_P, C.c_int32, C.c_int32, C.POINTER(C.c_int32), C.POINTER(C.c_int32), C.c_char_p, C.c_int32]),
+    'metro_plan_set_launch_groups': (C.c_int, [_P, C.c_int32]),
     'metro_forward': (C.c_int, [_P, _P, C.c_int32, _P, _P, _P]),
     'metro_forward_coords01': (C.c_int, [_P, _P, C.c_int32, _P, _P, _P, _P]),
     'metro_forward_u8': (C.c_int, [_P, _P, C.c_int32, _P, _P, _P, _P]),
@@ -145,6 +148,8 @@
     'metro_conv_f32m': (C.c_int, [C.POINTER(MetroConvDesc), _P, _P, _P, _P, _P, _P, _P, _P]),
     'metro_conv_f64acc': (C.c_int, [C.POINTER(MetroConvDesc), _P, _P, _P, _P, _P, _P, _P, _P]),
     'metro_conv_f16_pair': (C.c_int, [C.POINTER(MetroConvDesc), _P, _P, _P, _P, _P, _P, C.c_int32, _P, _P]),
+    'metro_conv_f16_conv2_conv3_supported': (C.c_int, [C.POINTER(MetroConvDesc)] + [C.c_int32] * 5),
+    'metro_conv_f16_conv2_conv3': (C.c_int, [C.POINTER(MetroConvDesc), _P, _P, _P, _P, _P, C.c_int32, _P] + [C.c_int32] * 4 + [_P, _P]),
     'metro_conv_b1_form': (C.c_int, [C.c_int32]),
     'metro_conv_f16_gemm4w': (C.c_int, [C.POINTER(MetroConvDesc), _P, _P, _P, _P, _P, _P, _P, C.c_int32, _P, _P]),
     'metro_conv_f16_conv1_conv2': (C.c_int, [C.POINTER(MetroConvDesc), _P, _P, _P, _P, _P, _P, _P, _P, _P]),
diff --git a/metro_pose3d_amd/csrc/conv_igemm_f16_dma.hip b/metro_pose3d_amd/csrc/conv_igemm_f16_dma.hip
--- a/metro_pose3d_amd/csrc/conv_igemm_f16_dma.hip
+++ b/metro_pose3d_amd/csrc/conv_igemm_f16_dma.hip
@@ -35,12 +35,38 @@
     const half_t* w2; const float* bias2; const half_t* scale2; const half_t* shift2; half_t* out2; int c2;
 };
 
-template <class Cfg, bool PROLOGUE, bool FASTK, bool FUSE2>
+struct Fuse3Args {
+    const half_t* w3; const float* bias3; const half_t* residual; half_t* out; int c3;
+    int res_stride, res_offset, res_h, res_w;
+};
+template <class Cfg>
+struct Fuse3Lay {
+    static constexpr int KC = Cfg::TM / 64;
+    static constexpr bool COMPACT = KC == 1;
+    static constexpr int CH_BYTES = Cfg::TM * 128;
+    static constexpr int NCH = 4 * KC;
+    static constexpr int PFC = COMPACT ? 3 : 2;
+    static constexpr int T2_OFF = COMPACT ? Cfg::STAGE_BYTES : Cfg::RING_BYTES;
+    static constexpr int OUT_OFF = T2_OFF + Cfg::OUT_BYTES;
+    static constexpr int PF_OFF = COMPACT ? 0 : OUT_OFF + Cfg::OUT_BYTES;
+    static constexpr int BIAS_OFF = COMPACT ? Cfg::RING_BYTES : PF_OFF + PFC * CH_BYTES;
+    static constexpr int LDS_BYTES = BIAS_OFF + (COMPACT ? 2048 : 3072);
+    static constexpr int chunk_off(int c) {
+        return COMPACT ? (c < PFC ? c * CH_BYTES : OUT_OFF + Cfg::OUT_BYTES) : c < PFC ? PF_OFF + c * CH_BYTES : ((c - PFC) % 4) * CH_BYTES;
+    }
+    static_assert(Cfg::BK == 64 && Cfg::STAGES == 3 && (KC == 1 || KC == 2), "FUSE3: the 3-stage BK 64 ring, widths 64 and 128");
+    static_assert(PF_OFF % 128 == 0 && OUT_OFF % 128 == 0 && BIAS_OFF % 128 == 0 && LDS_BYTES <= 160 * 1024, "FUSE3 LDS layout");
+    static_assert(COMPACT ? PFC * CH_BYTES <= Cfg::STAGE_BYTES && chunk_off(3) + CH_BYTES <= Cfg::RING_BYTES && 2 * LDS_BYTES <= 160 * 1024
+                          : 4 * CH_BYTES <= Cfg::RING_BYTES, "FUSE3 chunk schedule");
+};
+
+template <class Cfg, bool PROLOGUE, bool FASTK, bool FUSE2, bool FUSE3 = false>
 __device__ __forceinline__ void conv_dma_body(
     const ConvArgs& a, const half_t* __restrict__ in, const half_t* __restrict__ w,
     const float* __restrict__ bias, const half_t* __restrict__ pro_scale,
     const half_t* __restrict__ pro_shift, const half_t* __restrict__ residual,
-    void* __restrict__ out, int out_f32, int tiles_m, void* __restrict__ out2, const Fuse2Args& f2) {
+    void* __restrict__ out, int out_f32, int tiles_m, void* __restrict__ out2, const Fuse2Args& f2,
+    const Fuse3Args& f3 = Fuse3Args{}) {
     extern __shared__ __attribute__((aligned(16))) char smem[];
     constexpr int BK = Cfg::BK, STAGES = Cfg::STAGES, NW = Cfg::NW;
     constexpr int CPR = Cfg::CPR, RPI = Cfg::RPI;
@@ -261,6 +287,45 @@
         }
     };
 
+    using F3 = Fuse3Lay<std::conditional_t<FUSE3, Cfg, DmaCfg<1, 4, 2, 1, 3>>>;
+    constexpr int F3_RES = FUSE3 ? 4 * EPI_ITERS : 1;
+    uint4 r3[F3_RES];
+    [[maybe_unused]] auto f3_issue_chunk = [&](int c, int dst_off) {
+        const int slab = c / F3::KC, kc = c % F3::KC;
+#pragma unroll
+        for (int i = 0; i < Cfg::WI; ++i) {
+            const int row = (i * NW + wave) * RPI + lrow;
+            const half_t* src = f3.w3 + (size_t)(slab * Cfg::TM + row) * Cfg::TM + kc * 64 + ((lch ^ swz<64>(row)) * 8);
+            dma16(src, __builtin_amdgcn_readfirstlane(smem_base + dst_off + (i * NW + wave) * RPI * 128));
+        }
+    };
+    [[maybe_unused]] auto f3_prefetch = [&]() {
+#pragma unroll
+        for (int c = 0; c < F3::PFC; ++c) f3_issue_chunk(c, F3::chunk_off(c));
+        const bool same = f3.res_stride == 1 && f3.res_offset == 0 && f3.res_h == a.h_out && f3.res_w == a.w_out;
+#pragma unroll
+        for (int it = 0; it < EPI_ITERS; ++it) {
+            const int idx = tid + it * Cfg::NT;
+            const int prow = idx / CPRO;
+            const int ch = idx - prow * CPRO;
+            const int m = m0 + prow;
+            const bool ok = m < a.m_total;
+            size_t rp = ok ? (size_t)m : 0;
+            if (!same && ok) {
+                const int img = m / hw_out;
+                const int rem = m - img * hw_out;
+                const int ho = rem / a.w_out;
+                const int wo = rem - ho * a.w_out;
+                rp = (size_t)(img * f3.res_h + ho * f3.res_stride + f3.res_offset) * f3.res_w + (wo * f3.res_stride + f3.res_offset);
+            }
+            const half_t* rb = f3.residual + rp * f3.c3 + ch * 8;
+#pragma unroll
+            for (int sl = 0; sl < 4; ++sl) {
+                if constexpr (FUSE3) r3[sl * EPI_ITERS + it] = *reinterpret_cast<const uint4*>(rb + sl * Cfg::TM);
+            }
+        }
+    };
+
     constexpr bool PRO_DMA = PROLOGUE && !FUSE2;
     if constexpr (PRO_DMA) {
 #pragma unroll
@@ -272,6 +337,14 @@
                 const half_t* src = idx < a.c_in ? ((id >> 2) ? pro_shift : pro_scale) + idx : zero;
                 dma16(src, __builtin_amdgcn_readfirstlane(smem_base + Cfg::MAIN_BYTES + (id >> 2) * 4096 + piece * 1024));
             }
+        }
+    }
+    if constexpr (FUSE3) {
+        static_assert(NW >= 3 && Cfg::TM * 4 <= 1024 && Cfg::TM * 16 <= 2048, "FUSE3 bias pieces");
+        if (wave < 3 && (wave < 2 || Cfg::TM * 16 > 1024)) {
+            const int n = wave == 0 ? Cfg::TM : 4 * Cfg::TM, idx = (wave == 2 ? 256 : 0) + lane * 4;
+            const float* src = idx < n ? (wave == 0 ? bias : f3.bias3) + idx : reinterpret_cast<const float*>(zero);
+            dma16(src, __builtin_amdgcn_readfirstlane(smem_base + F3::BIAS_OFF + wave * 1024));
         }
     }
     if constexpr (STAGES > 1) {
@@ -343,8 +416,23 @@
             issue_end();
             advance();
         }
+        if constexpr (FUSE3) {
+            constexpr int F3_X = F3::PFC * Cfg::WI + F3_RES;
+            if constexpr (F3::COMPACT) {
+                wait_vm_and_barrier<Cfg::LPS>();
+                f3_prefetch();
+            } else {
+                f3_prefetch();
+                wait_vm_and_barrier<Cfg::LPS + F3_X>();
+            }
+            compute_step(cbuf, cc0, No{});
+            advance();
+            wait_vm_and_barrier<F3_X>();
+            compute_step(cbuf, cc0, No{});
+            advance();
+        }
         if (has_res) prefetch_residual();
-        for (int k = n_main < 0 ? 0 : n_main; k < nk; ++k) {
+        for (int k = FUSE3 ? nk : n_main < 0 ? 0 : n_main; k < nk; ++k) {
             int ahead = nk - 1 - k;
             if (ahead > STAGES - 2) ahead = STAGES - 2;
             if (has_res) {
@@ -367,6 +455,147 @@
             compute_step(cbuf, cc0, No{});
             advance();
         }
+    }
+
+    if constexpr (FUSE3) {
+        if constexpr (F3::COMPACT) {
+            wait_lgkm_and_barrier();
+            f3_issue_chunk(3, F3::chunk_off(3));
+        }
+        char* t2l = smem + F3::T2_OFF;
+        char* ol = smem + F3::OUT_OFF;
+        const float* bias2_l = reinterpret_cast<const float*>(smem + F3::BIAS_OFF);
+        const float* bias3_l = bias2_l + 256;
+#pragma unroll
+        for (int i = 0; i < Cfg::WM; ++i) {
+#pragma unroll
+            for (int q = 0; q < 4; ++q) {
+                const int col = (wave_m * Cfg::WM + i) * 32 + 8 * q + 4 * frag_half;
+                const floatx4 bv = *reinterpret_cast<const floatx4*>(bias2_l + col);
+#pragma unroll
+                for (int j = 0; j < Cfg::WN; ++j) {
+                    const int prow = (wave_n * Cfg::WN + j) * 32 + frag_row;
+                    half4_t hv;
+#pragma unroll
+                    for (int e = 0; e < 4; ++e) {
+                        float v = acc[i][j][4 * q + e] + bv[e];
+                        if (a.relu) v = fmaxf(v, 0.f);
+                        hv[e] = (half_t)v;
+                    }
+                    *reinterpret_cast<half4_t*>(t2l + prow * Cfg::OUT_ROW_BYTES + col * 2) = hv;
+                }
+            }
+        }
+        wait_vm_and_barrier<F3_RES + (F3::COMPACT ? Cfg::WI : 0)>();
+        if constexpr (!F3::COMPACT) {
+#pragma unroll
+            for (int c = F3::PFC; c < F3::PFC + 4; ++c) f3_issue_chunk(c, F3::chunk_off(c));
+        }
+        const bool interior = m0 + Cfg::TN <= a.m_total;
+        half_t* o3 = f3.out;
+#pragma unroll
+        for (int sl = 0; sl < 4; ++sl) {
+            if (sl > 0) {
+                if constexpr (F3::COMPACT) {
+                    if (sl < 3) wait_lgkm_and_barrier();
+                    else if (interior) wait_vm_and_barrier<3 * EPI_ITERS>();
+                    else wait_vm_and_barrier<0>();
+                } else {
+                    if (sl < 3) wait_vm_and_barrier<2 * Cfg::WI>();
+                    else if (interior) wait_vm_and_barrier<2 * EPI_ITERS>();
+                    else wait_vm_and_barrier<0>();
+                }
+            }
+            floatx16 acc3[Cfg::WM][Cfg::WN];
+#pragma unroll
+            for (int i = 0; i < Cfg::WM; ++i)
+#pragma unroll
+                for (int j = 0; j < Cfg::WN; ++j)
+#pragma unroll
+                    for (int e = 0; e < 16; ++e) acc3[i][j][e] = 0.f;
+#pragma unroll
+            for (int kc = 0; kc < F3::KC; ++kc) {
+                const char* wl = smem + F3::chunk_off(sl * F3::KC + kc);
+#pragma unroll
+                for (int kk = 0; kk < 4; ++kk) {
+                    half8_t af[Cfg::WM], bf[Cfg::WN];
+                    const int chunk = kk * 2 + frag_half;
+#pragma unroll
+                    for (int i = 0; i < Cfg::WM; ++i) {
+                        const int row = (wave_m * Cfg::WM + i) * 32 + frag_row;
+                        af[i] = *reinterpret_cast<const half8_t*>(wl + row * 128 + ((chunk ^ swz<64>(row)) << 4));
+                    }
+#pragma unroll
+                    for (int j = 0; j < Cfg::WN; ++j) {
+                        const int prow = (wave_n * Cfg::WN + j) * 32 + frag_row;
+                        bf[j] = *reinterpret_cast<const half8_t*>(t2l + prow * Cfg::OUT_ROW_BYTES + (kc * 64 + kk * 16 + frag_half * 8) * 2);
+                    }
+#pragma unroll
+                    for (int i = 0; i < Cfg::WM; ++i)
+#pragma unroll
+                        for (int j = 0; j < Cfg::WN; ++j)
+                            acc3[i][j] = __builtin_amdgcn_mfma_f32_32x32x16_f16(af[i], bf[j], acc3[i][j], 0, 0, 0);
+                }
+            }
+#pragma unroll
+            for (int i = 0; i < Cfg::WM; ++i) {
+#pragma unroll
+                for (int q = 0; q < 4; ++q) {
+                    const int col = (wave_m * Cfg::WM + i) * 32 + 8 * q + 4 * frag_half;
+                    const floatx4 bv = *reinterpret_cast<const floatx4*>(bias3_l + sl * Cfg::TM + col);
+#pragma unroll
+                    for (int j = 0; j < Cfg::WN; ++j) {
+                        const int prow = (wave_n * Cfg::WN + j) * 32 + frag_row;
+                        half4_t hv;
+#pragma unroll
+                        for (int e = 0; e < 4; ++e) hv[e] = (half_t)(acc3[i][j][4 * q + e] + bv[e]);
+                        *reinterpret_cast<half4_t*>(ol + prow * Cfg::OUT_ROW_BYTES + col * 2) = hv;
+                    }
+                }
+            }
+            wait_lgkm_and_barrier();
+            if constexpr (!F3::COMPACT) {
+                if (sl == 1) { f3_issue_chunk(6, F3::chunk_off(6)); f3_issue_chunk(7, F3::chunk_off(7)); }
+            }
+            if (interior) {
+                uint4 vv[EPI_ITERS];
+#pragma unroll
+                for (int it = 0; it < EPI_ITERS; ++it) {
+                    const int idx = tid + it * Cfg::NT;
+                    const int prow = idx / CPRO;
+                    vv[it] = *reinterpret_cast<const uint4*>(ol + prow * Cfg::OUT_ROW_BYTES + (idx - prow * CPRO) * 16);
+                }
+                __builtin_amdgcn_sched_barrier(0);
+#pragma unroll
+                for (int it = 0; it < EPI_ITERS; ++it) {
+                    const int idx = tid + it * Cfg::NT;
+                    const int prow = idx / CPRO;
+                    const int ch = idx - prow * CPRO;
+                    uint4 v = vv[it];
+                    half2_t* x = reinterpret_cast<half2_t*>(&v);
+                    const half2_t* r = reinterpret_cast<const half2_t*>(&r3[sl * EPI_ITERS + it]);
+#pragma unroll
+                    for (int e = 0; e < 4; ++e) x[e] = x[e] + r[e];
+                    store_out16<2>(o3 + (size_t)(m0 + prow) * f3.c3 + sl * Cfg::TM + ch * 8, v);
+                }
+            } else {
+#pragma unroll
+                for (int it = 0; it < EPI_ITERS; ++it) {
+                    const int idx = tid + it * Cfg::NT;
+                    const int prow = idx / CPRO;
+                    const int ch = idx - prow * CPRO;
+                    const int m = m0 + prow;
+                    if (m >= a.m_total) continue;
+                    uint4 v = *reinterpret_cast<const uint4*>(ol + prow * Cfg::OUT_ROW_BYTES + ch * 16);
+                    half2_t* x = reinterpret_cast<half2_t*>(&v);
+                    const half2_t* r = reinterpret_cast<const half2_t*>(&r3[sl * EPI_ITERS + it]);
+#pragma unroll
+                    for (int e = 0; e < 4; ++e) x[e] = x[e] + r[e];
+                    store_out16<2>(o3 + (size_t)m * f3.c3 + sl * Cfg::TM + ch * 8, v);
+                }
+            }
+        }
+        return;
     }
 
     const bool second = a.split > 0 && n0 >= a.split;
@@ -536,6 +765,12 @@
     ConvArgs a, const half_t* __restrict__ in, const half_t* __restrict__ w, const float* __restrict__ bias,
     const half_t* __restrict__ residual, void* __restrict__ out, Fuse2Args f2) {
     conv_dma_body<Cfg, false, true, true>(a, in, w, bias, nullptr, nullptr, residual, out, 0, 1, nullptr, f2);
+}
+
+template <class Cfg>
+__global__ __launch_bounds__(Cfg::NT) void conv_igemm_f16_c2c3_kernel(
+    ConvArgs a, const half_t* __restrict__ in, const half_t* __restrict__ w, const float* __restrict__ bias, Fuse3Args f3) {
+    conv_dma_body<Cfg, false, true, false, true>(a, in, w, bias, nullptr, nullptr, nullptr, nullptr, 0, 1, nullptr, Fuse2Args{}, f3);
 }
 
 template <class Cfg, bool PROLOGUE, bool FASTK>
@@ -598,6 +833,52 @@
                        Fuse2Args{static_cast<const half_t*>(f.w2), f.bias2, static_cast<const half_t*>(f.scale2),
                                  static_cast<const half_t*>(f.shift2), static_cast<half_t*>(f.out2), f.c2});
     return launch_status("conv_igemm_f16_dma<fuse2>");
+}
+
+using Dma128x64s3 = DmaCfg<2, 2, 2, 1, 3>;
+
+bool conv2_conv3_supported(const MetroConvDesc& d, int c3, int res_stride, int res_offset, int res_h, int res_w) {
+    static const int enabled = tuning_knob("METRO_C2C3", 1);
+    static const int w64 = tuning_knob("METRO_C2C3_W64", 1), w128 = tuning_knob("METRO_C2C3_W128", 1);
+    if (!enabled || !(d.kh == 3 && d.kw == 3 && d.stride == 2 && d.dilation == 1 && d.c_in == d.c_out && d.in_pix_stride == d.c_in &&
+                      ((d.c_out == 64 && w64) || (d.c_out == 128 && w128)) && c3 == 4 * d.c_out && d.relu && !d.has_prologue && !d.has_residual &&
+                      d.in_dtype == METRO_F16 && d.out_dtype == METRO_F16))
+        return false;
+    const bool same = res_stride == 1 && res_offset == 0 && res_h == d.h_out && res_w == d.w_out;
+    const bool sub = res_stride == 2 && (res_offset == 0 || res_offset == 1) && res_offset + 2 * (d.h_out - 1) < res_h &&
+                     res_offset + 2 * (d.w_out - 1) < res_w;
+    return same || sub;
+}
+
+bool conv2_conv3_preferred(const MetroConvDesc& d) {
+    const long m = (long)d.n * d.h_out * d.w_out;
+    return d.c_out == 64 ? (m + Dma64x128s3::TN - 1) / Dma64x128s3::TN <= 2 * 256 : (m + Dma128x64s3::TN - 1) / Dma128x64s3::TN <= 256;
+}
+
+template <class Cfg>
+static int launch_c2c3_cfg(const ConvArgs& a, const half_t* in, const half_t* w, const float* bias, const Fuse3Args& f3, bool same,
+                           hipStream_t stream) {
+    if (note_kernel("conv_igemm_f16_c2c3<%dx%d,bk%d,s%d>%s", Cfg::TM, Cfg::TN, Cfg::BK, Cfg::STAGES, same ? "+res" : "+ressub"))
+        return METRO_OK;
+    auto kern = conv_igemm_f16_c2c3_kernel<Cfg>;
+    constexpr int lds = Fuse3Lay<Cfg>::LDS_BYTES;
+    static PerDeviceInt attr_done;
+    if (const int st = ensure_dyn_lds(reinterpret_cast<const void*>(kern), lds, attr_done, "conv_igemm_f16_c2c3")) return st;
+    const int tiles_n = (a.m_total + Cfg::TN - 1) / Cfg::TN;
+    hipLaunchKernelGGL(kern, dim3(tiles_n), dim3(Cfg::NT), lds, stream, a, in, w, bias, f3);
+    return launch_status("conv_igemm_f16_c2c3");
+}
+
+int launch_conv2_conv3(const MetroConvDesc& d, const void* in, const void* w2, const float* bias2, const void* w3, const float* bias3,
+                       int c3, const void* residual, int res_stride, int res_offset, int res_h, int res_w, void* out,
+                       hipStream_t stream) {
+    const ConvArgs a = make_conv_args(d);
+    const Fuse3Args f3{static_cast<const half_t*>(w3), bias3, static_cast<const half_t*>(residual), static_cast<half_t*>(out), c3,
+                       res_stride, res_offset, res_h, res_w};
+    const bool same = res_stride == 1 && res_offset == 0 && res_h == d.h_out && res_w == d.w_out;
+    if (d.c_out == 64)
+        return launch_c2c3_cfg<Dma64x128s3>(a, static_cast<const half_t*>(in), static_cast<const half_t*>(w2), bias2, f3, same, stream);
+    return launch_c2c3_cfg<Dma128x64s3>(a, static_cast<const half_t*>(in), static_cast<const half_t*>(w2), bias2, f3, same, stream);
 }
 
 bool conv_f16_dma_supported(const MetroConvDesc& d) {
diff --git a/metro_pose3d_amd/csrc/entries.cpp b/metro_pose3d_amd/csrc/entries.cpp
--- a/metro_pose3d_amd/csrc/entries.cpp
+++ b/metro_pose3d_amd/csrc/entries.cpp
@@ -176,6 +176,25 @@
     METRO_CHECK_ARG(conv_form_supported(*d, f), "conv_f16_next_rebuild: built for 1x1 stride-1 64 -> 256 without prologue / residual on maps "
                     "whose width is a power of two >= 16 and whose pixel count is a multiple of 64, c2 = 64 (block1/unit_2), fp16");
     return launch_conv_f16_dma(*d, d_in, d_w, d_bias, nullptr, nullptr, nullptr, d_out, static_cast<hipStream_t>(stream), f);
+}
+
+int metro_conv_f16_conv2_conv3_supported(const MetroConvDesc* d, int32_t c_out3, int32_t res_stride, int32_t res_offset, int32_t res_h,
+                                         int32_t res_w) {
+    return d != nullptr && conv2_conv3_supported(*d, c_out3, res_stride, res_offset, res_h, res_w) ? 1 : 0;
+}
+
+int metro_conv_f16_conv2_conv3(const MetroConvDesc* d, const void* d_in, const void* d_w2, const float* d_bias2, const void* d_w3,
+                               const float* d_bias3, int32_t c_out3, const void* d_residual, int32_t res_stride, int32_t res_offset,
+                               int32_t res_h, int32_t res_w, void* d_out, void* stream) {
+    int st = validate_conv_desc(d);
+    if (st) return st;
+    METRO_CHECK_ARG(d_in && d_w2 && d_bias2 && d_w3 && d_bias3 && d_residual && d_out, "conv_f16_conv2_conv3: NULL tensor pointer");
+    METRO_CHECK_ARG(conv2_conv3_supported(*d, c_out3, res_stride, res_offset, res_h, res_w),
+                    "conv_f16_conv2_conv3: built for a 3x3 stride-2 fp16 conv2 of width 64 or 128 with ReLU (no prologue, no residual) and a "
+                    "conv3 of 4 x width channels whose shortcut is compact (res_stride 1 on the output map) or gathered (res_stride 2, "
+                    "res_offset 0 | 1, in bounds)");
+    return launch_conv2_conv3(*d, d_in, d_w2, d_bias2, d_w3, d_bias3, c_out3, d_residual, res_stride, res_offset, res_h, res_w, d_out,
+                              static_cast<hipStream_t>(stream));
 }
 
 int metro_conv_b1_form(int32_t classic) {
diff --git a/metro_pose3d_amd/csrc/executor.cpp b/metro_pose3d_amd/csrc/executor.cpp
--- a/metro_pose3d_amd/csrc/executor.cpp
+++ b/metro_pose3d_amd/csrc/executor.cpp
@@ -96,6 +96,26 @@
     return METRO_ERR_STATE;
 }
 
+int launch_len(const MetroPlan* p, int li, int last_layer, int n) {
+    const Layer& L = p->layers[li];
+    if (!p->launch_groups || L.group_len < 2 || li + L.group_len - 1 > last_layer) return 1;
+    MetroConvDesc cd = L.cd;
+    cd.n = n;
+    return conv2_conv3_preferred(cd) ? L.group_len : 1;
+}
+
+int launch_group(const MetroPlan* p, const char* d_params, int li, int n, char* ws, hipStream_t stream) {
+    const Layer& L2 = p->layers[li];
+    const Layer& L3 = p->layers[li + 1];
+    auto slot_ptr = [&](int slot) -> void* { return slot < 0 ? nullptr : ws + p->slot_offset[slot]; };
+    auto prm = [&](int idx) -> const void* { return idx < 0 ? nullptr : d_params + p->params[idx].offset; };
+    MetroConvDesc cd = L2.cd;
+    cd.n = n;
+    return launch_conv2_conv3(cd, slot_ptr(L2.in_slot), prm(L2.main.w), static_cast<const float*>(prm(L2.main.bias)), prm(L3.main.w),
+                              static_cast<const float*>(prm(L3.main.bias)), L3.cd.c_out, slot_ptr(L3.res_slot), L3.cd.res_stride,
+                              L3.cd.res_offset, L3.cd.res_h, L3.cd.res_w, slot_ptr(L3.out_slot), stream);
+}
+
 int run_layers(MetroPlan* p, const float* images, int n, float* poses, void* ws_, hipStream_t stream,
                int last_layer, float* ms_out, float* coords01 = nullptr, bool images_u8 = false, const MomentsOut& mo = MomentsOut{}) {
     METRO_CHECK_ARG(p != nullptr, "plan is NULL");
@@ -112,15 +132,20 @@
         for (auto& e : ev) METRO_HIP_CHECK(hipEventCreate(&e));
     }
     int st = METRO_OK;
-    for (int li = 0; li <= last_layer && st == METRO_OK; ++li) {
-        if (ms_out) METRO_HIP_CHECK(hipEventRecord(ev[2 * li], stream));
-        st = launch_layer(p, p->d_params, li, images, n, poses, ws, stream, li == last_layer && li + 1 < nl, coords01, images_u8, mo);
-        if (ms_out) METRO_HIP_CHECK(hipEventRecord(ev[2 * li + 1], stream));
+    std::vector<char> timed(ms_out ? last_layer + 1 : 0, 0);
+    for (int li = 0; li <= last_layer && st == METRO_OK;) {
+        const int len = launch_len(p, li, last_layer, n), lt = li + len - 1;
+        if (ms_out) METRO_HIP_CHECK(hipEventRecord(ev[2 * lt], stream));
+        if (len > 1) st = launch_group(p, p->d_params, li, n, ws, stream);
+        else st = launch_layer(p, p->d_params, li, images, n, poses, ws, stream, li == last_layer && li + 1 < nl, coords01, images_u8, mo);
+        if (ms_out) { METRO_HIP_CHECK(hipEventRecord(ev[2 * lt + 1], stream)); timed[lt] = 1; }
+        li += len;
     }
     if (ms_out) {
         if (st == METRO_OK) {
             METRO_HIP_CHECK(hipEventSynchronize(ev.back()));
             for (int li = 0; li <= last_layer; ++li) {
+                if (!timed[li]) continue;
                 float ms = 0.f;
                 METRO_HIP_CHECK(hipEventElapsedTime(&ms, ev[2 * li], ev[2 * li + 1]));
                 ms_out[li] += ms;
@@ -148,6 +173,45 @@
     snprintf(buf, (size_t)buf_len, "%s", kn.ids);
     kn = saved;
     return st;
+}
+
+int32_t metro_plan_num_launches(const MetroPlan* plan, int32_t n) {
+    if (plan == nullptr || n <= 0 || n > plan->max_batch) return -1;
+    const int last = (int)plan->layers.size() - 1;
+    int32_t count = 0;
+    for (int li = 0; li <= last; li += launch_len(plan, li, last, n)) ++count;
+    return count;
+}
+
+int metro_plan_launch_info(const MetroPlan* plan, int32_t n, int32_t index, int32_t* first_layer, int32_t* n_layers, char* buf, int32_t buf_len) {
+    METRO_CHECK_ARG(plan && first_layer && n_layers && buf && buf_len > 1, "metro_plan_launch_info: bad argument");
+    METRO_CHECK_ARG(n > 0 && n <= plan->max_batch, "metro_plan_launch_info: batch %d outside [1, %d]", n, plan->max_batch);
+    const int last = (int)plan->layers.size() - 1;
+    int li = 0, k = 0;
+    while (li <= last && k < index) { li += launch_len(plan, li, last, n); ++k; }
+    METRO_CHECK_ARG(index >= 0 && li <= last, "metro_plan_launch_info: launch %d outside the forward's launches", index);
+    const int len = launch_len(plan, li, last, n);
+    *first_layer = li; *n_layers = len;
+    if (len == 1) return metro_plan_layer_kernel(plan, li, n, buf, buf_len);
+    KernelNotes& kn = kernel_notes();
+    const KernelNotes saved = kn;
+    kn.mode = 2; kn.ids[0] = 0;
+    static const char fake = 0;
+    const int st = launch_group(plan, &fake, li, n, const_cast<char*>(&fake), nullptr);
+    snprintf(buf, (size_t)buf_len, "%s", kn.ids);
+    kn = saved;
+    return st;
+}
+
+int metro_plan_set_launch_groups(MetroPlan* plan, int32_t on) {
+    METRO_CHECK_ARG(plan != nullptr && (on == 0 || on == 1), "metro_plan_set_launch_groups: bad argument");
+    if ((on != 0) != plan->launch_groups) {
+        for (GraphEntry& g : plan->graphs)
+            if (g.exec) (void)hipGraphExecDestroy(g.exec);
+        plan->graphs.clear();
+    }
+    plan->launch_groups = on != 0;
+    return METRO_OK;
 }
 
 int metro_plan_bind_params(MetroPlan* plan, const void* d_param_blob) {
diff --git a/metro_pose3d_amd/csrc/metro_common.h b/metro_pose3d_amd/csrc/metro_common.h
--- a/metro_pose3d_amd/csrc/metro_common.h
+++ b/metro_pose3d_amd/csrc/metro_common.h
@@ -250,6 +250,11 @@
                         hipStream_t stream, const ConvFused& f = ConvFused{});
 bool conv_form_supported(const MetroConvDesc& d, const ConvFused& f);
 bool conv_f16_fuse2_supported(const MetroConvDesc& d, int c2);
+bool conv2_conv3_supported(const MetroConvDesc& d, int c3, int res_stride, int res_offset, int res_h, int res_w);
+bool conv2_conv3_preferred(const MetroConvDesc& d);
+int launch_conv2_conv3(const MetroConvDesc& d, const void* in, const void* w2, const float* bias2, const void* w3, const float* bias3,
+                       int c3, const void* residual, int res_stride, int res_offset, int res_h, int res_w, void* out,
+                       hipStream_t stream);
 bool conv_gemm4w_shape_ok(const MetroConvDesc& d, const ConvSplit* split);
 bool conv_gemm4w_supported(const MetroConvDesc& d, const ConvSplit* split);
 int launch_conv_gemm4w(const MetroConvDesc& d, const void* in, const void* w, const float* bias, const void* pro_scale,
diff --git a/metro_pose3d_amd/csrc/plan.h b/metro_pose3d_amd/csrc/plan.h
--- a/metro_pose3d_amd/csrc/plan.h
+++ b/metro_pose3d_amd/csrc/plan.h
@@ -35,6 +35,7 @@
     int psc_slot = S_NONE, reb_slot = S_NONE;
     int out_mode = 0, sub_slot = S_NONE, sub_off = 0, sub_side = 0;
     int head_c_in = 0;
+    int group_len = 1;
 };
 
 struct GraphEntry {
@@ -54,6 +55,7 @@
     std::vector<metro::GraphEntry> graphs;
     hipStream_t cap_stream = nullptr;
     int graph_max_batch = 0;
+    bool launch_groups = true;
     MetroSpec spec;
     int max_batch;
     bool fast;
diff --git a/metro_pose3d_amd/csrc/planner.cpp b/metro_pose3d_amd/csrc/planner.cpp
--- a/metro_pose3d_amd/csrc/planner.cpp
+++ b/metro_pose3d_amd/csrc/planner.cpp
@@ -333,6 +333,13 @@
         if (f.carries_next_conv1) fuse_next_conv1(L3, *next_unit);
         p->layers.push_back(L3);
         prev3 = (int)p->layers.size() - 1;
+        if (p->fast && g.stride == 2 && L2.form == LayerForm::Plain && L3.form == LayerForm::Plain && L3.out_mode == 0 &&
+            (f.shortcut == ShortcutFrom::Identity || f.shortcut == ShortcutFrom::Compact)) {
+            MetroConvDesc d2 = L2.cd;
+            d2.n = 1;
+            if (conv2_conv3_supported(d2, L3.cd.c_out, L3.cd.res_stride, L3.cd.res_offset, L3.cd.res_h, L3.cd.res_w))
+                p->layers[prev3 - 1].group_len = 2;
+        }
         *x_slot = out;
         return METRO_OK;
     }
diff --git a/metro_pose3d_amd/engine.py b/metro_pose3d_amd/engine.py
--- a/metro_pose3d_amd/engine.py
+++ b/metro_pose3d_amd/engine.py
@@ -105,6 +105,19 @@
             check(self.lib.metro_plan_layer_kernel(self._plan, i, int(n), buf, len(buf)), 'metro_plan_layer_kernel')
             out.append(buf.value.decode())
         return out
+
+    def launches(self, n: int) -> List[tuple]:
+        out = []
+        buf = C.create_string_buffer(1024)
+        first, count = C.c_int32(), C.c_int32()
+        for i in range(self.lib.metro_plan_num_launches(self._plan, int(n))):
+            check(self.lib.metro_plan_launch_info(self._plan, int(n), i, C.byref(first), C.byref(count), buf, len(buf)),
+                  'metro_plan_launch_info')
+            out.append((first.value, count.value, buf.value.decode()))
+        return out
+
+    def set_launch_groups(self, on: bool) -> None:
+        check(self.lib.metro_plan_set_launch_groups(self._plan, int(bool(on))), 'metro_plan_set_launch_groups')
 
     @property
     def flops_per_image(self) -> float:
```

Result: no change. 48330, median of 2 (+0.7%).
